# fgcallari/skeres

Hardware: AMD Instinct MI355X
Metric: LM iterations/sec (higher is better)
Workload: dtype f64

## Files before the change

include/skeres_amd.h:

```cpp
#ifndef SKERES_AMD_H
#define SKERES_AMD_H

#include <stddef.h>

#ifdef __cplusplus
extern "C" {
#endif

typedef enum sk_status {
  SK_OK = 0,
  SK_ERR_INVALID_ARGUMENT = 1,
  SK_ERR_NO_DEVICE = 2,
  SK_ERR_HIP = 3,
  SK_ERR_UNSUPPORTED = 4,
  SK_ERR_EVALUATION_FAILED = 5,
  SK_ERR_COMM = 6
} sk_status;

typedef enum sk_linear_solver_type {
  SK_DENSE_NORMAL_CHOLESKY = 0,
  SK_DENSE_QR = 1,
  SK_SPARSE_NORMAL_CHOLESKY = 2,
  SK_DENSE_SCHUR = 3,
  SK_SPARSE_SCHUR = 4,
// ... 237 lines not shown
int sk_options_set_cholesky_envelope(sk_options* o, int on);
enum { SK_DISSECTION_AUTO = 0, SK_DISSECTION_ON = 1, SK_DISSECTION_OFF = 2 };
int sk_options_set_cholesky_dissection(sk_options* o, int mode);
int sk_options_set_resident_kernels(sk_options* o, int on);
int sk_options_set_graph_replay(sk_options* o, int on);
int sk_options_set_max_segments(sk_options* o, int n);
int sk_options_set_trust_region_strategy_type(sk_options* o, int type);
int sk_options_set_dogleg_type(sk_options* o, int type);
int sk_options_get_trust_region_strategy_type(const sk_options* o);
int sk_options_get_dogleg_type(const sk_options* o);
enum { SK_BORDER_AUTO = 0, SK_BORDER_ON = 1, SK_BORDER_OFF = 2 };
int sk_options_set_cholesky_border(sk_options* o, int mode);
enum { SK_RETAINED_AUTO = 0, SK_RETAINED_ON = 1, SK_RETAINED_OFF = 2 };
int sk_options_set_retained_points(sk_options* o, int mode, int max_points);
typedef int (*sk_allreduce_fn)(void* user, double* device_buffer, size_t count, void* hip_stream);
int sk_options_set_distributed(sk_options* o, int rank, int world, sk_allreduce_fn allreduce,
                               void* user);
typedef struct sk_rccl sk_rccl;
int sk_rccl_unique_id(void* id128);
sk_rccl* sk_allreduce_rccl_init(int rank, int world, const void* id128);
sk_rccl* sk_allreduce_rccl_create(void* nccl_comm);
void sk_allreduce_rccl_free(sk_rccl* h);
long sk_allreduce_rccl_calls(const sk_rccl* h);
sk_allreduce_fn sk_allreduce_rccl_fn(void);
enum { SK_DISTRIBUTION_AUTO = 0, SK_DISTRIBUTION_SHARDED = 1, SK_DISTRIBUTION_REPLICATED = 2, SK_DISTRIBUTION_SEGMENTED = 3 };
int sk_options_set_distribution_mode(sk_options* o, int mode);
int sk_options_set_reduce_buffer(sk_options* o, void* device_ptr, size_t bytes);
size_t sk_reduce_buffer_bytes(const sk_options* o, const sk_problem* p);

sk_summary* sk_summary_new(void);
void sk_summary_free(sk_summary* s);
double sk_summary_initial_cost(const sk_summary* s);
double sk_summary_final_cost(const sk_summary* s);
int sk_summary_num_iterations(const sk_summary* s);
int sk_summary_num_successful_steps(const sk_summary* s);
int sk_summary_num_unsuccessful_steps(const sk_summary* s);
int sk_summary_termination_type(const sk_summary* s);
const char* sk_summary_message(const sk_summary* s);
const char* sk_summary_brief_report(const sk_summary* s);
const char* sk_summary_full_report(const sk_summary* s);
int sk_summary_num_logged_iterations(const sk_summary* s);
double sk_summary_iteration_field(const sk_summary* s, int iteration, int field);
double sk_summary_phase_seconds(const sk_summary* s, int phase);
int sk_summary_linear_solver_type_used(const sk_summary* s);
int sk_summary_linear_solver_type_given(const sk_summary* s);

int sk_solve(const sk_options* options, sk_problem* problem, sk_summary* summary);

sk_solver* sk_solver_create(const sk_options* options, sk_problem* problem);
int sk_last_status(void);
void sk_solver_free(sk_solver* s);
int sk_solver_step(sk_solver* s, int* done);
int sk_solver_finish(sk_solver* s, sk_summary* summary);
int sk_solver_set_kernel_timing(sk_solver* s, int on);
double sk_solver_kernel_seconds(const sk_solver* s, const char* name, int* launches);
double sk_solver_syrk_flops_per_solve(const sk_solver* s);
double sk_solver_syrk_c_bytes_per_solve(const sk_solver* s);
int sk_solver_distribution(const sk_solver* s, double* allreduce_seconds, double* saved_seconds);
int sk_solver_stat(const sk_solver* s, const char* name, double* value);
int sk_solver_inner_iteration_blocks(sk_solver* s, int* iterations, int* status);

int sk_problem_point_partition(const sk_problem* p, int world, int* cuts, int* num_cameras,
                               int* num_points, int* point_of_block);
int sk_problem_segment_plan(const sk_problem* p, int max_segments, int forced, int* num_segments, int* camera_part_of_block,
                            int* point_owner_of_block);
int sk_problem_border_plan(const sk_problem* p, int mode, int* num_border_cameras, int* camera_position_of_block, int* gap,
                           double* model_us, double* model_us_plain, double* envelope_fill);
int sk_problem_retained_plan(const sk_problem* p, int mode, int max_points, int border_mode, int* num_retained, int* retained_of_block,
                             double* model_us, double* model_us_without);

int sk_synth_dense_targets(double seed, int m, int n, const double* x_star, double* y_out);

int sk_cholesky_solve(int n, const double* A, const double* b, double* x, double* L, int group);
int sk_cholesky_solve_ex(int n, const double* A, const double* b, double* x, double* L, int group, const int* last,
                         int automatic_plan);
int sk_cholesky_solve_bordered(int n, const double* A, const double* b, double* x, double* L, int group,
                               int border_begin_row, int automatic_plan);

int sk_cholesky_solve_dissected(int n, const double* A, const double* b, double* x, int head, int tail_begin, int group,
                                int automatic_plan);

int sk_cholesky_solve_segments(int n, const double* A, const double* b, double* x, int num_segments, const int* cuts, int group,
                               int automatic_plan);

#ifdef __cplusplus
}
#endif
#endif
```

skeres_amd/api.py:

```python
import ctypes as C
import os

import numpy as np

_HERE = os.path.dirname(os.path.abspath(__file__))
_LIB_PATH = os.path.join(_HERE, "libskeres_amd.so")


class SkeresError(RuntimeError):
    pass


_dp = C.POINTER(C.c_double)
_dpp = C.POINTER(_dp)
_ip = C.POINTER(C.c_int)
EVALUATE_FN = C.CFUNCTYPE(C.c_int, C.c_void_p, _dpp, _dp, _dpp)
ALLREDUCE_FN = C.CFUNCTYPE(C.c_int, C.c_void_p, C.c_void_p, C.c_size_t, C.c_void_p)

_lib = None

_SIGS = {
    "sk_version": (C.c_char_p, []),
    "sk_last_error": (C.c_char_p, []),
    "sk_init_logging": (None, [C.c_char_p]),
# ... 57 lines not shown
    "sk_cost_function_new_tape": (C.c_void_p, [C.c_int, _ip, C.c_int, _ip, C.c_int, _dp, C.c_int, C.c_int, _ip, _dp, C.c_int]),
    "sk_problem_add_dense_rows": (C.c_int, [C.c_void_p, C.c_int, C.c_int, _dp, C.c_void_p, _dp, C.c_int]),
    "sk_problem_num_residual_blocks": (C.c_int, [C.c_void_p]),
    "sk_problem_num_parameter_blocks": (C.c_int, [C.c_void_p]),
    "sk_problem_parameter_block_index": (C.c_int, [C.c_void_p, _dp]),
    "sk_problem_num_parameters": (C.c_int, [C.c_void_p]),
    "sk_problem_num_residuals": (C.c_int, [C.c_void_p]),
    "sk_options_new": (C.c_void_p, []),
    "sk_options_free": (None, [C.c_void_p]),
    "sk_options_set_linear_solver_type": (C.c_int, [C.c_void_p, C.c_int]),
    "sk_options_set_minimizer_type": (C.c_int, [C.c_void_p, C.c_int]),
    "sk_options_set_trust_region_strategy_type": (C.c_int, [C.c_void_p, C.c_int]),
    "sk_options_set_dogleg_type": (C.c_int, [C.c_void_p, C.c_int]),
    "sk_options_get_trust_region_strategy_type": (C.c_int, [C.c_void_p]),
    "sk_options_get_dogleg_type": (C.c_int, [C.c_void_p]),
    "sk_options_set_max_num_iterations": (C.c_int, [C.c_void_p, C.c_int]),
    "sk_options_set_minimizer_progress_to_stdout": (C.c_int, [C.c_void_p, C.c_int]),
    "sk_options_set_function_tolerance": (C.c_int, [C.c_void_p, C.c_double]),
    "sk_options_set_gradient_tolerance": (C.c_int, [C.c_void_p, C.c_double]),
    "sk_options_set_parameter_tolerance": (C.c_int, [C.c_void_p, C.c_double]),
    "sk_options_set_initial_trust_region_radius": (C.c_int, [C.c_void_p, C.c_double]),
    "sk_options_set_max_trust_region_radius": (C.c_int, [C.c_void_p, C.c_double]),
    "sk_options_set_min_trust_region_radius": (C.c_int, [C.c_void_p, C.c_double]),
    "sk_options_set_min_relative_decrease": (C.c_int, [C.c_void_p, C.c_double]),
    "sk_options_set_min_lm_diagonal": (C.c_int, [C.c_void_p, C.c_double]),
    "sk_options_set_max_lm_diagonal": (C.c_int, [C.c_void_p, C.c_double]),
    "sk_options_set_jacobi_scaling": (C.c_int, [C.c_void_p, C.c_int]),
    "sk_options_set_max_num_consecutive_invalid_steps": (C.c_int, [C.c_void_p, C.c_int]),
    "sk_options_set_device": (C.c_int, [C.c_void_p, C.c_int]),
    "sk_options_set_preconditioner_type": (C.c_int, [C.c_void_p, C.c_int]),
    "sk_options_set_eta": (C.c_int, [C.c_void_p, C.c_double]),
    "sk_options_set_max_linear_solver_iterations": (C.c_int, [C.c_void_p, C.c_int]),
    "sk_options_set_min_linear_solver_iterations": (C.c_int, [C.c_void_p, C.c_int]),
    "sk_options_set_cholesky_tuning": (C.c_int, [C.c_void_p, C.c_int, C.c_int]),
    "sk_options_set_schur_elimination": (C.c_int, [C.c_void_p, C.c_int]),
    "sk_cgnr_elimination_plan": (C.c_int, [C.c_void_p, _ip, _ip, _ip, _ip, _ip]),
    "sk_options_set_use_inner_iterations": (C.c_int, [C.c_void_p, C.c_int]),
    "sk_options_get_use_inner_iterations": (C.c_int, [C.c_void_p]),
    "sk_options_set_inner_iteration_tolerance": (C.c_int, [C.c_void_p, C.c_double]),
    "sk_options_get_inner_iteration_tolerance": (C.c_double, [C.c_void_p]),
    "sk_options_set_inner_iteration_ordering": (C.c_int, [C.c_void_p, C.POINTER(_dp), _ip, C.c_int]),
    "sk_inner_iteration_plan": (C.c_int, [C.c_void_p, C.c_void_p, _ip, _ip]),
    "sk_solver_inner_iteration_blocks": (C.c_int, [C.c_void_p, _ip, _ip]),
    "sk_options_set_stream": (C.c_int, [C.c_void_p, C.c_void_p]),
    "sk_options_set_distributed": (C.c_int, [C.c_void_p, C.c_int, C.c_int, ALLREDUCE_FN, C.c_void_p]),
    "sk_options_set_reduce_buffer": (C.c_int, [C.c_void_p, C.c_void_p, C.c_size_t]),
    "sk_reduce_buffer_bytes": (C.c_size_t, [C.c_void_p, C.c_void_p]),
    "sk_summary_new": (C.c_void_p, []),
    "sk_summary_free": (None, [C.c_void_p]),
    "sk_summary_initial_cost": (C.c_double, [C.c_void_p]),
    "sk_summary_final_cost": (C.c_double, [C.c_void_p]),
    "sk_summary_num_iterations": (C.c_int, [C.c_void_p]),
    "sk_summary_num_successful_steps": (C.c_int, [C.c_void_p]),
    "sk_summary_num_unsuccessful_steps": (C.c_int, [C.c_void_p]),
    "sk_summary_termination_type": (C.c_int, [C.c_void_p]),
    "sk_summary_message": (C.c_char_p, [C.c_void_p]),
    "sk_summary_brief_report": (C.c_char_p, [C.c_void_p]),
    "sk_summary_full_report": (C.c_char_p, [C.c_void_p]),
    "sk_summary_num_logged_iterations": (C.c_int, [C.c_void_p]),
    "sk_summary_iteration_field": (C.c_double, [C.c_void_p, C.c_int, C.c_int]),
    "sk_summary_phase_seconds": (C.c_double, [C.c_void_p, C.c_int]),
    "sk_summary_linear_solver_type_used": (C.c_int, [C.c_void_p]),
    "sk_summary_linear_solver_type_given": (C.c_int, [C.c_void_p]),
    "sk_solve": (C.c_int, [C.c_void_p, C.c_void_p, C.c_void_p]),
    "sk_solver_create": (C.c_void_p, [C.c_void_p, C.c_void_p]),
    "sk_solver_free": (None, [C.c_void_p]),
    "sk_solver_step": (C.c_int, [C.c_void_p, _ip]),
    "sk_solver_finish": (C.c_int, [C.c_void_p, C.c_void_p]),
    "sk_solver_set_kernel_timing": (C.c_int, [C.c_void_p, C.c_int]),
    "sk_solver_kernel_seconds": (C.c_double, [C.c_void_p, C.c_char_p, _ip]),
    "sk_solver_syrk_flops_per_solve": (C.c_double, [C.c_void_p]),
    "sk_solver_syrk_c_bytes_per_solve": (C.c_double, [C.c_void_p]),
    "sk_solver_distribution": (C.c_int, [C.c_void_p, _dp, _dp]),
    "sk_solver_stat": (C.c_int, [C.c_void_p, C.c_char_p, _dp]),
    "sk_last_status": (C.c_int, []),
    "sk_cholesky_solve_dissected": (C.c_int, [C.c_int, _dp, _dp, _dp, C.c_int, C.c_int, C.c_int, C.c_int]),
    "sk_rccl_unique_id": (C.c_int, [C.c_void_p]),
    "sk_allreduce_rccl_init": (C.c_void_p, [C.c_int, C.c_int, C.c_void_p]),
    "sk_allreduce_rccl_create": (C.c_void_p, [C.c_void_p]),
    "sk_allreduce_rccl_free": (None, [C.c_void_p]),
    "sk_allreduce_rccl_calls": (C.c_long, [C.c_void_p]),
    "sk_allreduce_rccl_fn": (C.c_void_p, []),
    "sk_cholesky_solve_segments": (C.c_int, [C.c_int, _dp, _dp, _dp, C.c_int, _ip, C.c_int, C.c_int]),
    "sk_cholesky_solve_ex": (C.c_int, [C.c_int, _dp, _dp, _dp, _dp, C.c_int, _ip, C.c_int]),
    "sk_problem_border_plan": (C.c_int, [C.c_void_p, C.c_int, C.POINTER(C.c_int), _ip, C.POINTER(C.c_int), C.POINTER(C.c_double), C.POINTER(C.c_double), C.POINTER(C.c_double)]),
    "sk_cholesky_solve_bordered": (C.c_int, [C.c_int, _dp, _dp, _dp, _dp, C.c_int, C.c_int, C.c_int]),
    "sk_options_set_distribution_mode": (C.c_int, [C.c_void_p, C.c_int]),
    "sk_options_set_cholesky_envelope": (C.c_int, [C.c_void_p, C.c_int]),
    "sk_options_set_cholesky_dissection": (C.c_int, [C.c_void_p, C.c_int]),
    "sk_options_set_cholesky_border": (C.c_int, [C.c_void_p, C.c_int]),
    "sk_options_set_retained_points": (C.c_int, [C.c_void_p, C.c_int, C.c_int]),
    "sk_problem_retained_plan": (C.c_int, [C.c_void_p, C.c_int, C.c_int, C.c_int, C.POINTER(C.c_int), _ip, C.POINTER(C.c_double), C.POINTER(C.c_double)]),
    "sk_options_set_resident_kernels": (C.c_int, [C.c_void_p, C.c_int]),
    "sk_options_set_graph_replay": (C.c_int, [C.c_void_p, C.c_int]),
    "sk_options_set_max_segments": (C.c_int, [C.c_void_p, C.c_int]),
    "sk_cholesky_solve": (C.c_int, [C.c_int, _dp, _dp, _dp, _dp, C.c_int]),
    "sk_synth_dense_targets": (C.c_int, [C.c_double, C.c_int, C.c_int, _dp, _dp]),
    "sk_problem_point_partition": (C.c_int, [C.c_void_p, C.c_int, _ip, _ip, _ip, _ip]),
    "sk_problem_segment_plan": (C.c_int, [C.c_void_p, C.c_int, C.c_int, _ip, _ip, _ip]),
    "sk_evaluate_options_new": (C.c_void_p, []),
    "sk_evaluate_options_free": (None, [C.c_void_p]),
    "sk_evaluate_options_set_apply_loss_function": (C.c_int, [C.c_void_p, C.c_int]),
    "sk_evaluate_options_set_residual_blocks": (C.c_int, [C.c_void_p, _ip, C.c_int]),
    "sk_evaluate_options_set_parameter_blocks": (C.c_int, [C.c_void_p, _dpp, C.c_int]),
    "sk_evaluate_options_set_device": (C.c_int, [C.c_void_p, C.c_int]),
    "sk_evaluate_options_set_launch_timing": (C.c_int, [C.c_void_p, C.c_int]),
    "sk_evaluate_options_launch_seconds": (C.c_double, [C.c_void_p, C.c_int]),
    "sk_problem_evaluate_sizes": (C.c_int, [C.c_void_p, C.c_void_p, _ip, _ip, C.POINTER(C.c_longlong)]),
    "sk_problem_evaluate_structure": (C.c_int, [C.c_void_p, C.c_void_p, _ip, _ip]),
    "sk_problem_evaluate": (C.c_int, [C.c_void_p, C.c_void_p, _dp, _dp, _dp, _dp]),
    "sk_covariance_options_new": (C.c_void_p, []),
    "sk_covariance_options_free": (None, [C.c_void_p]),
    "sk_covariance_options_set_apply_loss_function": (C.c_int, [C.c_void_p, C.c_int]),
    "sk_covariance_options_set_min_reciprocal_condition_number": (C.c_int, [C.c_void_p, C.c_double]),
    "sk_covariance_options_set_device": (C.c_int, [C.c_void_p, C.c_int]),
    "sk_covariance_options_set_schur_elimination": (C.c_int, [C.c_void_p, C.c_int]),
    "sk_covariance_elimination_plan": (C.c_int, [C.c_void_p, _ip, _ip, _ip, C.POINTER(C.c_longlong)]),
    "sk_covariance_new": (C.c_void_p, [C.c_void_p]),
    "sk_covariance_free": (None, [C.c_void_p]),
    "sk_covariance_compute": (C.c_int, [C.c_void_p, C.c_void_p, _dpp, _dpp, C.c_int]),
    "sk_covariance_compute_blocks": (C.c_int, [C.c_void_p, C.c_void_p, _dpp, C.c_int]),
    "sk_covariance_get_block": (C.c_int, [C.c_void_p, _dp, _dp, _dp]),
    "sk_covariance_get_block_in_tangent_space": (C.c_int, [C.c_void_p, _dp, _dp, _dp]),
    "sk_covariance_get_matrix": (C.c_int, [C.c_void_p, _dpp, C.c_int, _dp]),
    "sk_covariance_get_matrix_in_tangent_space": (C.c_int, [C.c_void_p, _dpp, C.c_int, _dp]),
    "sk_covariance_stat": (C.c_int, [C.c_void_p, C.c_char_p, _dp]),
    "sk_covariance_block_sizes": (C.c_int, [C.c_void_p, _dp, _ip, _ip]),
}


def exported_symbols():
    return sorted(_SIGS)


def lib():
    global _lib
    if _lib is None:
        global _LIB_PATH
        _LIB_PATH = os.environ.get("SKERES_AMD_LIBRARY", _LIB_PATH)
        if not os.path.exists(_LIB_PATH):
            raise SkeresError("%s is missing: build it with `python -c 'import __graft_entry__ as g; g.build()'` "
                              "(make -C skeres_amd/csrc). There is no CPU fallback." % _LIB_PATH)
        L = C.CDLL(_LIB_PATH)
        for name, (res, args) in _SIGS.items():
            fn = getattr(L, name)
            fn.restype = res
            fn.argtypes = args
        _lib = L
    return _lib


def _check(rc):
    if rc != 0:
        raise SkeresError("status %d: %s" % (rc, lib().sk_last_error().decode()))


def _check_arg(rc):
    if rc == 1:
        raise ValueError(lib().sk_last_error().decode())
    _check(rc)


def device_count():
    return lib().sk_device_count()


# ... 1273 lines not shown
        mode = lib().sk_solver_distribution(self._h, C.byref(a), C.byref(b))
        return {1: "sharded", 2: "replicated", 3: "segmented"}.get(mode, "sharded"), a.value, b.value


def cholesky_solve(A, b, want_L=False, group=0, last=None, automatic_plan=False):
    A = np.ascontiguousarray(A, dtype=np.float64)
    b = np.ascontiguousarray(b, dtype=np.float64)
    n = A.shape[0]
    x = np.empty(n)
    L = np.empty((n, n)) if want_L else None
    lp = _ip()
    if last is not None:
        last = np.ascontiguousarray(last, dtype=np.int32)
        if last.shape[0] != (n + 1 + 127) // 128:
            raise ValueError("last needs one entry per 128-block column of the padded matrix")
        lp = last.ctypes.data_as(_ip)
    _check(lib().sk_cholesky_solve_ex(n, A.ctypes.data_as(_dp), b.ctypes.data_as(_dp), x.ctypes.data_as(_dp),
                                      L.ctypes.data_as(_dp) if want_L else _dp(), int(group), lp, int(bool(automatic_plan))))
    return (x, L) if want_L else x


def cholesky_solve_bordered(A, b, border_begin, want_L=False, group=0, automatic_plan=False):
    A = np.ascontiguousarray(A, dtype=np.float64)
    b = np.ascontiguousarray(b, dtype=np.float64)
    n = A.shape[0]
    x = np.empty(n)
    L = np.empty((n, n)) if want_L else None
    _check(lib().sk_cholesky_solve_bordered(n, A.ctypes.data_as(_dp), b.ctypes.data_as(_dp), x.ctypes.data_as(_dp),
                                            L.ctypes.data_as(_dp) if want_L else _dp(), int(group), int(border_begin), int(bool(automatic_plan))))
    return (x, L) if want_L else x


def cholesky_solve_dissected(A, b, head, tail_begin, group=0, automatic_plan=False):
    A = np.ascontiguousarray(A, dtype=np.float64)
    b = np.ascontiguousarray(b, dtype=np.float64)
    n = A.shape[0]
    x = np.empty(n)
    _check(lib().sk_cholesky_solve_dissected(n, A.ctypes.data_as(_dp), b.ctypes.data_as(_dp), x.ctypes.data_as(_dp), int(head), int(tail_begin),
                                             int(group), int(bool(automatic_plan))))
    return x


class RcclAllReduce:

    @staticmethod
    def unique_id():
        buf = C.create_string_buffer(128)
        _check(lib().sk_rccl_unique_id(buf))
        return buf.raw

    def __init__(self, rank, world, unique_id):
        self._id = C.create_string_buffer(bytes(unique_id), 128)
        self._h = lib().sk_allreduce_rccl_init(int(rank), int(world), self._id)
        if not self._h:
            raise SkeresError("status 6: %s" % lib().sk_last_error().decode())

    @property
    def calls(self):
        return int(lib().sk_allreduce_rccl_calls(self._h))

    def close(self):
        if self._h:
            lib().sk_allreduce_rccl_free(self._h)
            self._h = None

    def __del__(self):
        try:
            self.close()
        except Exception:
            pass


def cholesky_solve_segments(A, b, cuts, group=0, automatic_plan=False):
    A = np.ascontiguousarray(A, dtype=np.float64)
    b = np.ascontiguousarray(b, dtype=np.float64)
    n = A.shape[0]
    x = np.empty(n)
    c = np.ascontiguousarray(np.asarray(cuts, dtype=np.int32).reshape(-1))
    _check(lib().sk_cholesky_solve_segments(n, A.ctypes.data_as(_dp), b.ctypes.data_as(_dp), x.ctypes.data_as(_dp), len(cuts) + 1,
                                            c.ctypes.data_as(_ip), int(group), int(bool(automatic_plan))))
    return x


def synth_dense_targets(seed, m, n, x_star):
    xs = np.ascontiguousarray(x_star, dtype=np.float64)
    y = np.empty(int(m))
    _check(lib().sk_synth_dense_targets(float(seed), int(m), int(n), xs.ctypes.data_as(_dp), y.ctypes.data_as(_dp)))
    return y
```

skeres_amd/csrc/capi.hip:

```cpp
#include <cmath>
#include <cstdlib>
#include <new>

#include "bal_kernels.hpp"
#include "chol_solve.hpp"
#include "dense_kernels.hpp"
#include "dense_rows_kernels.hpp"
#include "evaluate_kernels.hpp"
#include "cgnr_plan.hpp"
#include "inner_plan.hpp"
#include "covariance.hpp"
#include "covariance_plan.hpp"
#include "evaluate_plan.hpp"
#include "solver.hpp"

using namespace sk;

struct sk_ptrvec { std::vector<double*> v; };
struct sk_loss_function { LossFunction l; };
struct sk_cost_function { CostFunction c; };
struct sk_problem { Problem p; };
struct sk_local_parameterization { LocalParameterization p; };
struct sk_options { Options o; };
struct sk_summary { Summary s; };
// ... 1041 lines not shown
  std::vector<int> part, owner;
  *num_segments = bal_segment_plan(p->p, max_segments, forced != 0, &part, &owner);
  for (size_t b = 0; b < part.size(); ++b) {
    if (camera_part_of_block) camera_part_of_block[b] = part[b];
    if (point_owner_of_block) point_owner_of_block[b] = owner[b];
  }
  return SK_OK;
  SK_GUARD_END(SK_ERR_INVALID_ARGUMENT)
}

int sk_problem_border_plan(const sk_problem* p, int mode, int* num_border_cameras, int* camera_position_of_block, int* gap, double* model_us, double* model_us_plain,
                           double* envelope_fill) {
  SK_GUARD_BEGIN
  if (!p || !num_border_cameras) { set_error("invalid argument"); return SK_ERR_INVALID_ARGUMENT; }
  if (mode != SK_BORDER_AUTO && mode != SK_BORDER_ON && mode != SK_BORDER_OFF) { set_error("invalid border mode %d", mode); return SK_ERR_INVALID_ARGUMENT; }
  std::string why;
  if (!problem_is_bal_shaped(p->p, &why)) { set_error("%s", why.c_str()); return SK_ERR_UNSUPPORTED; }
  std::vector<int> pos;
  *num_border_cameras = bal_border_plan(p->p, mode, &pos, gap, model_us, model_us_plain, envelope_fill);
  if (camera_position_of_block) for (size_t b = 0; b < pos.size(); ++b) camera_position_of_block[b] = pos[b];
  return SK_OK;
  SK_GUARD_END(SK_ERR_INVALID_ARGUMENT)
}

int sk_problem_retained_plan(const sk_problem* p, int mode, int max_points, int border_mode, int* num_retained, int* retained_of_block, double* model_us,
                             double* model_us_without) {
  SK_GUARD_BEGIN
  if (!p || !num_retained) { set_error("invalid argument"); return SK_ERR_INVALID_ARGUMENT; }
  if (mode != SK_RETAINED_AUTO && mode != SK_RETAINED_ON && mode != SK_RETAINED_OFF) { set_error("invalid retained-points mode %d", mode); return SK_ERR_INVALID_ARGUMENT; }
  if (border_mode != SK_BORDER_AUTO && border_mode != SK_BORDER_ON && border_mode != SK_BORDER_OFF) { set_error("invalid border mode %d", border_mode); return SK_ERR_INVALID_ARGUMENT; }
  std::string why;
  if (!problem_is_bal_shaped(p->p, &why)) { set_error("%s", why.c_str()); return SK_ERR_UNSUPPORTED; }
  std::vector<int> flag;
  *num_retained = bal_retained_plan(p->p, mode, max_points, border_mode, &flag, model_us, model_us_without);
  if (retained_of_block) for (size_t b = 0; b < flag.size(); ++b) retained_of_block[b] = flag[b];
  return SK_OK;
  SK_GUARD_END(SK_ERR_INVALID_ARGUMENT)
}

int sk_synth_dense_targets(double seed, int m, int n, const double* x_star, double* y_out) {
  SK_GUARD_BEGIN
  if (m <= 0 || n <= 0 || !x_star || !y_out) { set_error("invalid argument"); return SK_ERR_INVALID_ARGUMENT; }
  if (sk_device_count() <= 0) { set_error("no HIP device available: libskeres_amd has no CPU fallback"); return SK_ERR_NO_DEVICE; }
  std::vector<double> consts(3 * (size_t)m);
  for (int i = 0; i < m; ++i) { consts[3 * (size_t)i] = seed; consts[3 * (size_t)i + 1] = (double)i; consts[3 * (size_t)i + 2] = 0.0; }
  std::vector<double> xs(x_star, x_star + n);
  DevBuf<double> dc, dx, dr;
  hipStream_t s = nullptr;
  SK_HIP_TRY(dc.upload(consts, s)); SK_HIP_TRY(dx.upload(xs, s)); SK_HIP_TRY(dr.alloc(m));
  DenseRowsArgs a{}; a.loss_root = -1; a.m = m; a.n = n; a.m_pad = m; a.consts = dc.p; a.inv_sqrt_n = 1.0 / std::sqrt((double)n);
  launch_rows_residual(a, dx.p, dr.p, nullptr, false, s);
  SK_HIP_TRY(hipMemcpy(y_out, dr.p, (size_t)m * sizeof(double), hipMemcpyDeviceToHost));
  return SK_OK;
  SK_GUARD_END(SK_ERR_INVALID_ARGUMENT)
}

int sk_cholesky_solve(int n, const double* A, const double* b, double* x, double* L, int group) {
  return sk_cholesky_solve_ex(n, A, b, x, L, group, nullptr, 0);
}
int sk_cholesky_solve_ex(int n, const double* A, const double* b, double* x, double* L, int group, const int* last, int automatic_plan) {
  SK_GUARD_BEGIN
  if (n <= 0 || !A || !b || !x) { set_error("invalid argument"); return SK_ERR_INVALID_ARGUMENT; }
  return cholesky_solve_single(n, A, b, x, L, group, last, automatic_plan, -1);
  SK_GUARD_END(SK_ERR_INVALID_ARGUMENT)
}
int sk_cholesky_solve_bordered(int n, const double* A, const double* b, double* x, double* L, int group, int border_begin_row, int automatic_plan) {
  SK_GUARD_BEGIN
  if (n <= 0 || !A || !b || !x || border_begin_row < 0 || border_begin_row > n) { set_error("invalid argument"); return SK_ERR_INVALID_ARGUMENT; }
  return cholesky_solve_single(n, A, b, x, L, group, nullptr, automatic_plan, border_begin_row);
  SK_GUARD_END(SK_ERR_INVALID_ARGUMENT)
}
int sk_cholesky_solve_dissected(int n, const double* A, const double* b, double* x, int head, int tail_begin, int group, int automatic_plan) {
  SK_GUARD_BEGIN
  if (n <= 0 || !A || !b || !x || head < 0 || tail_begin < head || tail_begin > n) { set_error("invalid argument"); return SK_ERR_INVALID_ARGUMENT; }
  return cholesky_solve_two_way(n, A, b, x, head, tail_begin, group, automatic_plan);
  SK_GUARD_END(SK_ERR_INVALID_ARGUMENT)
}
int sk_cholesky_solve_segments(int n, const double* A, const double* b, double* x, int num_segments, const int* cuts, int group, int automatic_plan) {
  SK_GUARD_BEGIN
  if (n <= 0 || !A || !b || !x || num_segments < 2 || !cuts) { set_error("invalid argument"); return SK_ERR_INVALID_ARGUMENT; }
  return cholesky_solve_multi_way(n, A, b, x, num_segments, cuts, group, automatic_plan);
  SK_GUARD_END(SK_ERR_INVALID_ARGUMENT)
}

}
```

skeres_amd/csrc/chol_fronts.cpp:

```cpp
#include "chol_fronts.hpp"

#include <cstdio>
#include <cstring>

namespace sk {

std::vector<int> host_block_first_cols(const std::vector<double>& M, size_t ld, int nblk) {
  std::vector<int> first_col(nblk);
  for (int i = 0; i < nblk; ++i) {
    first_col[i] = i;
    for (int j = 0; j < i && first_col[i] == i; ++j) {
      bool nz = false;
      for (int r = 0; r < 128 && !nz; ++r) {
        const double* row = &M[((size_t)i * 128 + r) * ld + (size_t)j * 128];
        for (int c = 0; c < 128; ++c) if (row[c] != 0.0) { nz = true; break; }
      }
      if (nz) first_col[i] = j;
    }
  }
  return first_col;
}
std::vector<int> host_block_envelope(const std::vector<double>& M, size_t ld, int nblk, int tail_rows) {
  return cholesky_envelope_last(host_block_first_cols(M, ld, nblk), tail_rows);
}
// ... 85 lines not shown
std::string segment_cuts(int n, const double* A, int R, const int* cuts, SegmentCuts* out) {
  SegmentCuts& c = *out;
  c.R = R; c.n = n;
  c.sb.assign(R + 1, 0); c.se.assign(R + 1, 0);
  std::vector<int>& sb = c.sb; std::vector<int>& se = c.se;
  sb[R] = n;
  for (int k = 1; k < R; ++k) { sb[k] = cuts[2 * (k - 1)]; se[k] = cuts[2 * (k - 1) + 1]; }
  for (int k = 1; k <= R; ++k)
    if (sb[k] < se[k - 1] || (k < R && (se[k] < sb[k] || se[k] > n))) return "invalid cuts";
  for (int k = 1; k < R; ++k)
    for (int i = se[k]; i < n; ++i)
      for (int j = 0; j < sb[k]; ++j)
        if (A[(size_t)i * n + j] != 0.0) return format("rows behind separator %d couple with rows before it at (%d, %d): not a separator", k, i, j);
  c.sep_off.assign(R, 0);
  for (int k = 1; k < R; ++k) c.sep_off[k] = c.sep_off[k - 1] + (se[k] - sb[k]);
  c.nroot = c.sep_off[R - 1];
  return std::string();
}

static inline double sym(const double* A, int n, int i, int j) { return i >= j ? A[(size_t)i * n + j] : A[(size_t)j * n + i]; }

HostFront segments_root(const SegmentCuts& c, const double* A, const double* b) {
  HostFront r;
  const int R = c.R, nroot = c.nroot, E = (nroot + 1 + 127) / 128;
  const size_t dR = (size_t)E * 128;
  r.dim = dR; r.nblk = E; r.ncols = E; r.rhs_row = nroot;
  std::vector<double>& FR = r.F;
  FR.assign(dR * dR, 0.0);
  for (int k = 1; k < R; ++k)
    for (int i = c.sb[k]; i < c.se[k]; ++i) {
      const int ri = c.root_index(i);
      for (int k2 = 1; k2 <= k; ++k2)
        for (int j = c.sb[k2]; j < c.se[k2] && j <= i; ++j) FR[(size_t)ri * dR + c.root_index(j)] = sym(A, c.n, i, j);
      FR[(size_t)nroot * dR + ri] = b[i];
    }
  FR[(size_t)nroot * dR + nroot] = 1e300;
  for (size_t j = (size_t)nroot + 1; j < dR; ++j) FR[j * dR + j] = 1.0;
  r.last = root_envelope(c.sep_off);
  return r;
}

LeafFront segment_leaf(const SegmentCuts& c, const double* A, const double* b, int k) {
  LeafFront f;
  const int R = c.R;
  const std::vector<int>& sb = c.sb; const std::vector<int>& se = c.se;
  const int lo = se[k], hi = sb[k + 1], ni = hi - lo;
  const int left_n = k > 0 ? se[k] - sb[k] : 0, right_n = k + 1 < R ? se[k + 1] - sb[k + 1] : 0;
  f.L = segment_layout(ni, left_n, right_n);
  f.interior_n = ni;
  const SegmentLayout& L = f.L;
  f.dim = (size_t)L.nblk * 128;
  const size_t d = f.dim;
  f.order.assign(d, -1);
  for (int t = 0; t < ni; ++t) f.order[t] = L.reversed ? hi - 1 - t : lo + t;
  const int bo = L.ncols * 128;
  if (L.right_off >= 0) for (int t = 0; t < right_n; ++t) f.order[bo + L.right_off + t] = sb[k + 1] + t;
  if (L.left_off >= 0) for (int t = 0; t < left_n; ++t) f.order[bo + L.left_off + t] = L.reversed ? se[k] - 1 - t : sb[k] + t;
  std::vector<double>& F = f.F;
  F.assign(d * d, 0.0);
  for (size_t i = 0; i < d; ++i) {
    const int gi = f.order[i];
    if (gi < 0) continue;
    for (size_t j = 0; j <= i && j < (size_t)ni; ++j) F[i * d + j] = sym(A, c.n, gi, f.order[j]);
  }
  for (int t = 0; t < ni; ++t) F[(size_t)L.rhs_row * d + t] = b[f.order[t]];
  for (int i = ni; i < bo; ++i) F[(size_t)i * d + i] = 1.0;
  f.last = host_block_envelope(F, d, L.nblk, L.tail_rows);
  f.map.assign(d - bo, -1);
  for (size_t i = bo; i < d; ++i) if (f.order[i] >= 0) f.map[i - bo] = c.root_index(f.order[i]);
  f.map[L.rhs_row - bo] = c.nroot;
  f.gmap = f.map;
  f.gmap[L.rhs_row - bo] = -1;
  return f;
}

void segments_scatter_root(const SegmentCuts& c, const double* yR, double* x) {
  for (int k = 1; k < c.R; ++k) for (int i = c.sb[k]; i < c.se[k]; ++i) x[i] = yR[c.root_index(i)];
}

void segments_scatter_leaf(const LeafFront& f, const double* y, double* x) {
  for (int t = 0; t < f.L.ncols * 128; ++t) if (f.order[t] >= 0) x[f.order[t]] = y[t];
}

}
```

skeres_amd/csrc/chol_fronts.hpp:

```cpp
#pragma once
#include <cstddef>
#include <string>
#include <vector>

#include "chol_envelope.hpp"

namespace sk {

std::vector<int> host_block_first_cols(const std::vector<double>& M, size_t ld, int nblk);
std::vector<int> host_block_envelope(const std::vector<double>& M, size_t ld, int nblk, int tail_rows = 1);

struct HostFront {
  size_t dim = 0;
  int nblk = 0, ncols = 0, rhs_row = 0;
  std::vector<double> F;
  std::vector<int> last;
};

struct SingleFront {
  int n = 0, npad = 0, nblk = 0, rhs_row = 0;
  std::vector<double> S;
  std::vector<int> last, tail;
};
inline int single_front_blocks(int n) { return (n + 1 + 127) / 128; }
int invalid_envelope_column(int n, const int* last);
SingleFront single_front(int n, const double* A, const double* b, int border_begin_row);
void single_front_solution(const SingleFront& f, const std::vector<double>& y, double* x);
void single_front_factor(const SingleFront& f, const std::vector<double>& S, double* L);

struct TwoWayFronts {
  int n = 0, head = 0, tail_n = 0, sep_n = 0, border_blocks = 0;
  HostFront A, B, R;
  std::vector<int> mapB;
};
std::string two_way_check(int n, const double* A, int head, int tail_begin);
TwoWayFronts two_way_fronts(int n, const double* A, const double* b, int head, int tail_begin);
void two_way_scatter(const TwoWayFronts& f, const double* y, double* x);

struct SegmentCuts {
  int R = 0, n = 0, nroot = 0;
  std::vector<int> sb, se;
  std::vector<int> sep_off;
  int root_index(int row) const;
};
std::string segment_cuts(int n, const double* A, int R, const int* cuts, SegmentCuts* out);
HostFront segments_root(const SegmentCuts& c, const double* A, const double* b);
struct LeafFront {
  SegmentLayout L;
  size_t dim = 0;
  int interior_n = 0;
  std::vector<int> order;
  std::vector<int> map;
  std::vector<int> gmap;
  std::vector<int> last;
  std::vector<double> F;
};
LeafFront segment_leaf(const SegmentCuts& c, const double* A, const double* b, int k);
void segments_scatter_root(const SegmentCuts& c, const double* yR, double* x);
void segments_scatter_leaf(const LeafFront& f, const double* y, double* x);

}
```

skeres_amd/csrc/chol_kernels.hip:

```cpp
#include <hip/hip_runtime.h>
#include <algorithm>
#include <atomic>
#include <chrono>
#include <hip/hip_ext.h>
#include <math.h>
#include <stdlib.h>
#include <string.h>
#include <memory>
#include "chol_kernels.hpp"
#include "device_table.hpp"

namespace sk {

typedef double d4 __attribute__((ext_vector_type(4)));

constexpr int gemm_lds_doubles(int kBKT, int kTM, int kTN) { return 2 * (kTM + kTN) * (kBKT + 2); }
#define SK_GEMM_LDS(kBKT, kTM, kTN) __shared__ __attribute__((aligned(16))) double sh[gemm_lds_doubles(kBKT, kTM, kTN)];
template <int kMode, int kShape, int kBKT, int kPF, int kTM, int kTN>
__device__ __forceinline__ void gemm_nt_f64_body(double* shp, double* C, long ldc, const double* A, long lda, const double* B, long ldb, int K,
                                                 int tiles_m, int skip, int main_t = 0x7fffffff, int jump_t = 0, int main_n = 0x7fffffff,
                                                 int jump_n = 0, int block_id = -1, int* first_column_done = nullptr, int count_cols = 1,
                                                 int* diag_done = nullptr) {
  constexpr int mode = kMode;
  constexpr int kLdT = kBKT + 2;
// ... 75 lines not shown
  _Pragma("unroll") for (int i = 0; i < kChB; ++i) {                                                       \
    const double2 v_ = *reinterpret_cast<const double2*>(Bg + (long)(i * kRowStep + srow) * ldb + (kbase) + sc); rb##set[2 * i] = v_.x; rb##set[2 * i + 1] = v_.y; \
  }
#define SK_STORE_STAGE(set, buf)                                                                   \
  _Pragma("unroll") for (int i = 0; i < kChA; ++i)                                                  \
    *reinterpret_cast<double2*>(&shp[(buf) * kShBuf + (i * kRowStep + srow) * kLdT + sc]) = make_double2(ra##set[2 * i], ra##set[2 * i + 1]); \
  _Pragma("unroll") for (int i = 0; i < kChB; ++i)                                                  \
    *reinterpret_cast<double2*>(&shp[(buf) * kShBuf + (kTM + i * kRowStep + srow) * kLdT + sc]) = make_double2(rb##set[2 * i], rb##set[2 * i + 1]);
  const int nk = K / kBKT;
  SK_LOAD_STAGE(0, 0)
  if (kPF == 2) { SK_LOAD_STAGE(1, (nk > 1 ? 1 : 0) * kBKT) }
  SK_STORE_STAGE(0, 0)
  __syncthreads();
#define SK_LOAD_STAGE_X(set, kbase) SK_LOAD_STAGE(set, kbase)
#define SK_STORE_STAGE_X(set, buf) SK_STORE_STAGE(set, buf)
#define SK_KSTEP(kt, SETL, SETS)                                                                   \
  {                                                                                                \
    const int buf = (kt) & 1;                                                                      \
    const int knext = ((kt) + kPF < nk ? (kt) + kPF : nk - 1) * kBKT;                              \
    SK_LOAD_STAGE_X(SETL, knext)                                                                   \
    const double* sa = &shp[buf * kShBuf + (wr * (kTM / 2) + l15) * kLdT + l4];                               \
    const double* sb = &shp[buf * kShBuf + (kTM + wc * (kTN / 2) + l15) * kLdT + l4];                         \
    _Pragma("unroll") for (int kk = 0; kk < kBKT / 4; ++kk) {                                      \
      double a[kMT], b[kNT];                                                                       \
      _Pragma("unroll") for (int m = 0; m < kMT; ++m) a[m] = sa[m * 16 * kLdT + kk * 4];           \
      _Pragma("unroll") for (int m = 0; m < kNT; ++m) b[m] = sb[m * 16 * kLdT + kk * 4];           \
      _Pragma("unroll") for (int mt = 0; mt < kMT; ++mt)                                           \
        _Pragma("unroll") for (int nt = 0; nt < kNT; ++nt)                                         \
          acc[mt][nt] = __builtin_amdgcn_mfma_f64_16x16x4f64(a[mt], b[nt], acc[mt][nt], 0, 0, 0);  \
    }                                                                                              \
    SK_STORE_STAGE_X(SETS, buf ^ 1)                                                                \
    __syncthreads();                                                                               \
  }
  if (kPF == 1) {
    for (int kt = 0; kt < nk; ++kt) SK_KSTEP(kt, 0, 0)
  } else {
    for (int kt = 0; kt < nk; kt += 2) {
      SK_KSTEP(kt, 0, 1)
      SK_KSTEP(kt + 1, 1, 0)
    }
  }
#undef SK_KSTEP
#undef SK_LOAD_STAGE_X
#undef SK_STORE_STAGE_X
  (void)ra1; (void)rb1;
#undef SK_LOAD_STAGE
#undef SK_STORE_STAGE
  const double sgn = mode == 0 ? -1.0 : 1.0;
  if (kShape == 2 && first_column_done && first_column) {
#pragma unroll
    for (int mt = 0; mt < kMT; ++mt)
#pragma unroll
      for (int nt = 0; nt < kNT; ++nt)
#pragma unroll
        for (int i = 0; i < 4; ++i)
          __hip_atomic_store(&Cg[(long)(crow + mt * 16 + 4 * i) * ldc + ccol + nt * 16], sgn * acc[mt][nt][i], __ATOMIC_RELAXED, __HIP_MEMORY_SCOPE_AGENT);
    asm volatile("s_waitcnt vmcnt(0) lgkmcnt(0)" ::: "memory");
    __syncthreads();
    if (threadIdx.x == 0) {
      __hip_atomic_fetch_add(first_column_done, 1, __ATOMIC_RELAXED, __HIP_MEMORY_SCOPE_AGENT);
      if (diag_done && diag_tile) __hip_atomic_fetch_add(diag_done, 16 / (128 / kTM), __ATOMIC_RELAXED, __HIP_MEMORY_SCOPE_AGENT);
    }
    return;
  }
#pragma unroll
  for (int mt = 0; mt < kMT; ++mt)
#pragma unroll
    for (int nt = 0; nt < kNT; ++nt)
#pragma unroll
      for (int i = 0; i < 4; ++i)
        Cg[(long)(crow + mt * 16 + 4 * i) * ldc + ccol + nt * 16] = sgn * acc[mt][nt][i];
}

__global__ __launch_bounds__(256, 2) void syrk_trailing_f64_kernel(double* C, long ldc, const double* A, long lda, int K, int tile_off, int main_t,
                                                                   int jump_t) {
  SK_GEMM_LDS(16, 128, 128)
  gemm_nt_f64_body<0, 1, 16, 1, 128, 128>(sh, C, ldc, A, lda, A, lda, K, 0, tile_off, main_t, jump_t);
}
__global__ __launch_bounds__(256, 2) void syrk_trailing_thin_f64_kernel(double* C, long ldc, const double* A, long lda, int K, int tiles_m, int main_t,
                                                                        int jump_t, int main_n, int jump_n, int* first_column_done, int count_cols, int* diag_done) {
  SK_GEMM_LDS(16, 32, 128)
  gemm_nt_f64_body<0, 2, 16, 2, 32, 128>(sh, C, ldc, A, lda, A, lda, K, tiles_m, 0, main_t, jump_t, main_n, jump_n, -1, first_column_done, count_cols, diag_done);
}
struct ThinSyrkArgs { double* C; long ldc; const double* A; long lda; int K, tiles_m, main_t, jump_t, main_n, jump_n; int* first_column_done; int grid; };
struct ThinSyrkPair { ThinSyrkArgs f[2]; };
__global__ __launch_bounds__(256, 2) void syrk_trailing_thin_pair_f64_kernel(ThinSyrkPair pair) {
  const ThinSyrkArgs& p = pair.f[blockIdx.y];
  if ((int)blockIdx.x >= p.grid) return;
  SK_GEMM_LDS(16, 32, 128)
  gemm_nt_f64_body<0, 2, 16, 2, 32, 128>(sh, p.C, p.ldc, p.A, p.lda, p.A, p.lda, p.K, p.tiles_m, 0, p.main_t, p.jump_t, p.main_n, p.jump_n, -1, p.first_column_done, 1, nullptr);
}
__global__ __launch_bounds__(256, 2) void syrk_gram_f64_kernel(double* C, long ldc, size_t slab_stride, const double* A, long lda, int K) {
  SK_GEMM_LDS(16, 128, 128)
  gemm_nt_f64_body<1, 1, 16, 1, 128, 128>(sh, C + (size_t)blockIdx.y * slab_stride, ldc, A + (size_t)blockIdx.y * K, lda, A + (size_t)blockIdx.y * K, lda, K, 0, 0);
}
__global__ __launch_bounds__(256) void gram_reduce_kernel(double* __restrict__ H, const double* __restrict__ slabs, size_t slab_stride, long ld,
                                                          int nslabs) {
  const int b = blockIdx.x;
  int r = (int)((sqrt(8.0 * (double)b + 1.0) - 1.0) * 0.5);
  while ((r + 1) * (r + 2) / 2 <= b) ++r;
  while (r * (r + 1) / 2 > b) --r;
  const int ti = r, tj = b - r * (r + 1) / 2;
  for (int e = threadIdx.x; e < 128 * 128; e += 256) {
    const size_t off = (size_t)(ti * 128 + (e >> 7)) * ld + tj * 128 + (e & 127);
    double s = 0.0;
    for (int c = 0; c < nslabs; ++c) s += slabs[(size_t)c * slab_stride + off];
    H[off] = s;
  }
}
__global__ __launch_bounds__(256, 2) void gemm_update_f64_kernel(double* C, long ldc, const double* A, long lda, const double* B,
                                                                 long ldb, int K, int tiles_m, int skip, int main_t, int jump_t) {
  __builtin_amdgcn_s_setprio(2);
  SK_GEMM_LDS(16, 64, 128)
  gemm_nt_f64_body<0, 0, 16, 2, 64, 128>(sh, C, ldc, A, lda, B, ldb, K, tiles_m, skip, main_t, jump_t);
}
__global__ __launch_bounds__(256, 2) void gemm_update_thin_f64_kernel(double* C, long ldc, const double* A, long lda, const double* B,
                                                                      long ldb, int K, int tiles_m, int skip, int main_t, int jump_t) {
  __builtin_amdgcn_s_setprio(2);
  SK_GEMM_LDS(16, 32, 128)
  gemm_nt_f64_body<0, 0, 16, 2, 32, 128>(sh, C, ldc, A, lda, B, ldb, K, tiles_m, skip, main_t, jump_t);
}
__global__ __launch_bounds__(256, 2) void trsm_gemm_thin_f64_kernel(double* C, long ldc, const double* A, long lda, const double* Linv,
                                                                    int tiles_m, int main_t, int jump_t) {
  __builtin_amdgcn_s_setprio(2);
  SK_GEMM_LDS(16, 32, 128)
  gemm_nt_f64_body<1, 0, 16, 2, 32, 128>(sh, C, ldc, A, lda, Linv, 128, 128, tiles_m, 0, main_t, jump_t);
}
__global__ __launch_bounds__(256, 1) void gemm_diag_f64_kernel(double* C, long ldc, const double* A, long lda, int K) {
  __builtin_amdgcn_s_setprio(3);
  SK_GEMM_LDS(32, 64, 64)
  gemm_nt_f64_body<0, 0, 32, 2, 64, 64>(sh, C, ldc, A, lda, A, lda, K, 2, 4);
}
__global__ __launch_bounds__(256, 2) void trsm_gemm_f64_kernel(double* C, long ldc, const double* A, long lda, const double* Linv,
                                                               int tiles_m, int main_t, int jump_t) {
  __builtin_amdgcn_s_setprio(2);
  SK_GEMM_LDS(16, 64, 128)
  gemm_nt_f64_body<1, 0, 16, 2, 64, 128>(sh, C, ldc, A, lda, Linv, 128, 128, tiles_m, 0, main_t, jump_t);
}

static constexpr int kB = 32, kBs = 33;
static constexpr int kBlk = kB * kBs;
__device__ __forceinline__ int blk_off(int bi, int bj) { return (bi * (bi + 1) / 2 + bj) * kBlk; }
__device__ __forceinline__ int inv_off(int bi, int bj) { return (10 + bi * (bi - 1) / 2 + bj) * kBlk; }

__device__ __forceinline__ double fast_rsqrt(double x) {
  double y = __builtin_amdgcn_rsq(x);
  double h = 0.5 * x;
  y = y * (1.5 - h * y * y);
  y = y * (1.5 - h * y * y);
  return y;
}
__device__ __forceinline__ double fast_rcp(double x) {
  const double y = __builtin_amdgcn_rcp(x);
  const double e = __builtin_fma(-x, y, 1.0);
  const double q = __builtin_fma(e, e, e);
  return __builtin_fma(y, q, y);
}
__device__ __forceinline__ double lane_bcast(double x, int src) {
  const int lo = __builtin_amdgcn_readlane(__double2loint(x), src);
  const int hi = __builtin_amdgcn_readlane(__double2hiint(x), src);
  return __hiloint2double(hi, lo);
}

__device__ __forceinline__ bool wave_potrf32(const double* D, double* colbuf, double (&a)[32], int lane) {
  const int row = lane & 31;
  const bool unit = lane >= 32;
#pragma unroll
  for (int c = 0; c < 32; ++c) {
    const double d = D[row * kBs + c];
// ... 506 lines not shown
      }
      if (sync_load(abort_flag) != 0) return false;
      if (wall_clock64() - t0 > kChainTimeoutTicks) { __hip_atomic_store(abort_flag, 1, __ATOMIC_RELAXED, __HIP_MEMORY_SCOPE_AGENT); return false; }
    }
    __builtin_amdgcn_s_sleep(2);
  }
}

struct ChainRanges { int n; int begin[8], end[8]; };

__device__ __forceinline__ void chain_end_signal(int* counter) {
  __syncthreads();
  if (threadIdx.x == 0) {
    __builtin_amdgcn_fence(__ATOMIC_RELEASE, "agent");
    __hip_atomic_fetch_add(counter, 1, __ATOMIC_RELAXED, __HIP_MEMORY_SCOPE_AGENT);
  }
}
__global__ void chain_end_marker_kernel(int* counter) { chain_end_signal(counter); }
__global__ void chain_gate_kernel(const int* counter, int expected, int* info) {
  if (threadIdx.x != 0) return;
  if (sync_load(counter) < expected) {
    const long long t0 = wall_clock64();
    int spins = 0;
    do {
      __builtin_amdgcn_s_sleep(4);
      if ((++spins & 63) == 0 && wall_clock64() - t0 > 4 * kChainTimeoutTicks) { info_raise(info, 2); break; }
    } while (sync_load(counter) < expected);
  }
  __builtin_amdgcn_fence(__ATOMIC_ACQUIRE, "agent");
}
__global__ void chain_start_gate_kernel(const int* p, int value, int* info) {
  if (threadIdx.x != 0) return;
  if (!chain_wait_start(p, value)) info_raise(info, 2);
}
__device__ __forceinline__ void potrf_server_body(double* lds, double* S, long ld, const ChainRanges& ranges, double* Linv, int* info, int* sync, int maxblk, int local, int start) {
  __shared__ int ok_s;
  const int stamp_front = gridDim.x == 2 ? (int)blockIdx.x : 0;
  int done = 0;
  if (start != 0) {
    if (threadIdx.x == 0) ok_s = chain_wait_start(sync + kSyncStart, start) ? 1 : 0;
    __syncthreads();
    if (!ok_s) {
      if (threadIdx.x == 0) info_raise(info, 2);
      return;
    }
    SK_CHAIN_ACQUIRE_ALL
    __syncthreads();
  }
  if (local && threadIdx.x == 0) __hip_atomic_store(sync + kSyncServerXcc, 1 + xcc_id(), __ATOMIC_RELAXED, __HIP_MEMORY_SCOPE_AGENT);
  for (int r = 0; r < ranges.n; ++r)
    for (int j = ranges.begin[r]; j < ranges.end[r]; ++j) {
      if (j > 0) {
        if (threadIdx.x == 0) ok_s = server_wait_diag(sync, j, local) ? 1 : 0;
        __syncthreads();
        if (!ok_s) {
          if (threadIdx.x == 0) info_raise(info, 2);
          return;
        }
        SK_CHAIN_ACQUIRE_ALL
      }
      SK_CHAIN_STAMP(j, 0)
      potrf128_body(lds, S + (long)j * 128 * ld + (long)j * 128, ld, Linv + (long)j * 128 * 128, info);
      if (local) {
        asm volatile("s_waitcnt vmcnt(0) lgkmcnt(0)" ::: "memory");
        __syncthreads();
        if (threadIdx.x == 0) {
          store_l2(sync + kSyncPotrfFast, j + 1);
          SK_CHAIN_STAMP(j, 1)
          __builtin_amdgcn_fence(__ATOMIC_RELEASE, "agent");
          __hip_atomic_fetch_add(sync + kSyncPotrfDone, j + 1 - done, __ATOMIC_RELAXED, __HIP_MEMORY_SCOPE_AGENT);
        }
      } else {
        chain_publish(sync + kSyncPotrfDone, j + 1 - done);
        SK_CHAIN_STAMP(j, 1)
      }
      done = j + 1;
    }
}
__global__ __launch_bounds__(256, 1) void potrf_server_kernel(double* S, long ld, ChainRanges ranges, double* Linv, int* info, int* sync, int maxblk, int local, int start) {
  extern __shared__ __attribute__((aligned(16))) double lds[];
  potrf_server_body(lds, S, ld, ranges, Linv, info, sync, maxblk, local, start);
  if (start != 0) chain_end_signal(sync + kSyncEnd);
}
__global__ __launch_bounds__(256) void chain_start_kernel(int* sync_a, int n_a, int* sync_b, int n_b, int value) {
  for (int i = threadIdx.x; i < n_a; i += 256) sync_a[i] = 0;
  if (sync_b) for (int i = threadIdx.x; i < n_b; i += 256) sync_b[i] = 0;
  __syncthreads();
  if (threadIdx.x != 0) return;
  __builtin_amdgcn_fence(__ATOMIC_RELEASE, "agent");
  __hip_atomic_store(sync_a + kSyncStart, value, __ATOMIC_RELAXED, __HIP_MEMORY_SCOPE_AGENT);
  if (sync_b) __hip_atomic_store(sync_b + kSyncStart, value, __ATOMIC_RELAXED, __HIP_MEMORY_SCOPE_AGENT);
}
struct ServerArgs { double* S; long ld; ChainRanges ranges; double* Linv; int* sync; int maxblk; };
struct ServerPair { ServerArgs f[2]; };
__global__ __launch_bounds__(256, 1) void potrf_server_pair_kernel(ServerPair pair, int* info, int local, int start) {
  extern __shared__ __attribute__((aligned(16))) double lds[];
  const ServerArgs& p = pair.f[blockIdx.x];
  potrf_server_body(lds, p.S, p.ld, p.ranges, p.Linv, info, p.sync, p.maxblk, local, start);
  if (start != 0) chain_end_signal(pair.f[0].sync + kSyncEnd);
}

constexpr int kCritLd = 130;
__device__ __forceinline__ void crit_tile_load(double* shp, const double* A, long lda, const double* B, long ldb) {
  const int t = threadIdx.x, row = t >> 3, c0 = (t & 7) * 16;
  double2 va[8], vb[8];
#pragma unroll
  for (int i = 0; i < 8; ++i) va[i] = *reinterpret_cast<const double2*>(A + (long)row * lda + c0 + 2 * i);
#pragma unroll
  for (int i = 0; i < 8; ++i) vb[i] = *reinterpret_cast<const double2*>(B + (long)row * ldb + c0 + 2 * i);
#pragma unroll
  for (int i = 0; i < 8; ++i) *reinterpret_cast<double2*>(shp + row * kCritLd + c0 + 2 * i) = va[i];
#pragma unroll
  for (int i = 0; i < 8; ++i) *reinterpret_cast<double2*>(shp + (32 + row) * kCritLd + c0 + 2 * i) = vb[i];
}
__device__ __forceinline__ d4 crit_tile_mma(const double* shp, d4 acc) {
  const int lane = threadIdx.x & 63, wave = threadIdx.x >> 6;
  const int l15 = lane & 15, l4 = lane >> 4;
  const double* sa = shp + ((wave >> 1) * 16 + l15) * kCritLd + l4;
  const double* sb = shp + (32 + (wave & 1) * 16 + l15) * kCritLd + l4;
  d4 acc1 = {0.0, 0.0, 0.0, 0.0};
#pragma unroll
  for (int kk = 0; kk < 32; kk += 2) {
    acc = __builtin_amdgcn_mfma_f64_16x16x4f64(sa[kk * 4], sb[kk * 4], acc, 0, 0, 0);
    acc1 = __builtin_amdgcn_mfma_f64_16x16x4f64(sa[kk * 4 + 4], sb[kk * 4 + 4], acc1, 0, 0, 0);
  }
  return acc + acc1;
}
__device__ __forceinline__ long crit_tile_off(long ldc, int i) {
  const int lane = threadIdx.x & 63, wave = threadIdx.x >> 6;
  return (long)((wave >> 1) * 16 + (lane >> 4) + 4 * i) * ldc + (wave & 1) * 16 + (lane & 15);
}

__device__ __forceinline__ void chain_column_body(int b, double* S, long ld, int j, const double* Linv_j, int tiles_m, int main_t, int jump_t,
                                                  int ncrit, double* Xs, int* sync, int maxblk, int syrk_need, int column_need, int* info, int do_next, int wait_first,
                                                  int ncand) {
  __shared__ __attribute__((aligned(16))) double sh[2 * 32 * kCritLd];
  static_assert(2 * 32 * kCritLd >= gemm_lds_doubles(16, 32, 128), "LDS of the thin tiles");
  __shared__ int ok_s;
  const int stamp_front = gridDim.y == 2 ? (int)blockIdx.y : 0;
  __builtin_amdgcn_s_setprio(2);
  double* A21 = S + (long)(j + 1) * 128 * ld + (long)j * 128;
  int* x_ready = sync + kSyncHeader + maxblk + j;
  int* diag_ready = sync + kSyncHeader + j + 1;
  int* abort_flag = sync + kSyncAbort;
  const bool local = ncand > ncrit;
  bool crit = b < ncand;
  if (crit && local) {
    if (threadIdx.x == 0) {
      int t = -1;
      if (chain_wait(sync + kSyncServerXcc, 1, abort_flag) && sync_load(sync + kSyncServerXcc) == 1 + xcc_id())
        t = __hip_atomic_fetch_add(sync + kSyncHeader + 2 * maxblk + j, 1, __ATOMIC_RELAXED, __HIP_MEMORY_SCOPE_AGENT);
      ok_s = t >= 0 && t < 16 ? t : -1;
    }
    __syncthreads();
    const int tile = ok_s;
    __syncthreads();
    if (tile < 0) return;
    b = tile;
  }
  const int ri = b >> 2, q = b & 3;
  const int thin_id = 4 + (b - ncand);
  const int thin_bid = ncrit ? thin_id : b;
  const bool stamp = b == 0 && crit == (ncrit > 0);
  if (stamp) SK_CHAIN_STAMP(j, 2)
  if (crit && local) {
    double* Xj = Xs + (size_t)j * 128 * 128;
    const bool lower = q <= ri;
    double* Ct = A21 + 128 + (long)(ri * 32) * ld + q * 32;
    {
      const int t = threadIdx.x, row = t >> 3, c0 = (t & 7) * 16;
      double2 va[8];
#pragma unroll
      for (int i = 0; i < 8; ++i) va[i] = *reinterpret_cast<const double2*>(A21 + (long)(ri * 32 + row) * ld + c0 + 2 * i);
#pragma unroll
      for (int i = 0; i < 8; ++i) *reinterpret_cast<double2*>(sh + row * kCritLd + c0 + 2 * i) = va[i];
    }
    if (threadIdx.x == 0) ok_s = chain_wait_l2(sync + kSyncPotrfFast, j + 1, abort_flag) ? 1 : 0;
    __syncthreads();
// ... 52 lines not shown
      if (b == 1 && threadIdx.x == 0) {
        __builtin_amdgcn_fence(__ATOMIC_RELEASE, "agent");
        __hip_atomic_fetch_add(x_ready, 16, __ATOMIC_RELAXED, __HIP_MEMORY_SCOPE_AGENT);
      }
      asm volatile("s_waitcnt vmcnt(0) lgkmcnt(0)" ::: "memory");
      if (lower) {
#pragma unroll
        for (int i = 0; i < 8; ++i) *reinterpret_cast<double2*>(sh + row * kCritLd + c0 + 2 * i) = va[i];
#pragma unroll
        for (int i = 0; i < 8; ++i) *reinterpret_cast<double2*>(sh + (32 + row) * kCritLd + c0 + 2 * i) = vb[i];
      }
    }
    __syncthreads();
    if (lower) {
      cacc = crit_tile_mma(sh, cacc);
#pragma unroll
      for (int i = 0; i < 4; ++i) Ct[crit_tile_off(ld, i)] = -cacc[i];
    }
    asm volatile("s_waitcnt vmcnt(0) lgkmcnt(0)" ::: "memory");
    __syncthreads();
    if (threadIdx.x == 0) store_l2(sync + kSyncDSlot + b, j + 1);
    if (stamp) SK_CHAIN_STAMP(j, 6)
    return;
  }
  if (threadIdx.x == 0)
    ok_s = (chain_wait(sync + kSyncPotrfDone, j + 1, abort_flag) &&
            (!wait_first || (chain_wait(sync + kSyncSyrkSeq, syrk_need, abort_flag) && chain_wait(sync + kSyncSyrkColumn, column_need, abort_flag)))) ? 1 : 0;
  __syncthreads();
  if (!ok_s) { if (threadIdx.x == 0) info_raise(info, 2); return; }
  SK_CHAIN_ACQUIRE_ALL
  if (stamp) SK_CHAIN_STAMP(j, 3)
  d4 xacc = {0.0, 0.0, 0.0, 0.0};
  if (crit) {
    crit_tile_load(sh, A21 + (long)ri * 32 * ld, ld, Linv_j + (long)q * 32 * 128, 128);
    __syncthreads();
    xacc = crit_tile_mma(sh, xacc);
#pragma unroll
    for (int i = 0; i < 4; ++i) store_through(Xs + (long)(ri * 32) * 128 + q * 32 + crit_tile_off(128, i), xacc[i]);
    chain_publish_through(x_ready, 1);
  } else {
    gemm_nt_f64_body<1, 0, 16, 2, 32, 128>(sh, A21, ld, A21, ld, Linv_j, 128, 128, tiles_m, 0, main_t, jump_t, 0x7fffffff, 0, thin_bid);
    asm volatile("s_waitcnt vmcnt(0) lgkmcnt(0)" ::: "memory");
    __syncthreads();
  }
  if (stamp) SK_CHAIN_STAMP(j, 4)
  if (!do_next && !crit) return;
  if (threadIdx.x == 0)
    ok_s = (chain_wait(x_ready, ncrit, abort_flag) && (!do_next || (chain_wait(sync + kSyncSyrkSeq, syrk_need, abort_flag) &&
            chain_wait(sync + kSyncSyrkColumn, column_need, abort_flag)))) ? 1 : 0;
  __syncthreads();
  if (!ok_s) { if (threadIdx.x == 0) info_raise(info, 2); return; }
  SK_CHAIN_ACQUIRE_ALL
  if (stamp) SK_CHAIN_STAMP(j, 5)
  const double* Xsrc = local ? (const double*)(Xs + (size_t)j * 128 * 128) : (const double*)Xs;
  if (crit) {
#pragma unroll
    for (int i = 0; i < 4; ++i) A21[(long)(ri * 32) * ld + q * 32 + crit_tile_off(ld, i)] = xacc[i];
    if (!do_next) return;
    if (q <= ri) {
      double* Ct = A21 + 128 + (long)(ri * 32) * ld + q * 32;
      d4 acc;
#pragma unroll
      for (int i = 0; i < 4; ++i) acc[i] = -Ct[crit_tile_off(ld, i)];
      crit_tile_load(sh, Xs + (long)ri * 32 * 128, 128, Xs + (long)q * 32 * 128, 128);
      __syncthreads();
      acc = crit_tile_mma(sh, acc);
#pragma unroll
      for (int i = 0; i < 4; ++i) store_through(Ct + crit_tile_off(ld, i), -acc[i]);
    }
    chain_publish_through(diag_ready, 1);
  } else {
    const double* Bx = ncrit ? Xsrc : (const double*)A21;
    gemm_nt_f64_body<0, 0, 16, 2, 32, 128>(sh, A21 + 128, ld, A21, ld, Bx, ncrit ? 128 : ld, 128, tiles_m, 1, main_t, jump_t, 0x7fffffff, 0, thin_bid);
    if (ncrit == 0 && b == 0) chain_publish(diag_ready, 16);
  }
  if (stamp) SK_CHAIN_STAMP(j, 6)
}
__global__ __launch_bounds__(256, 2) void chain_column_kernel(double* S, long ld, int j, const double* Linv_j, int tiles_m, int main_t, int jump_t,
                                                              int ncrit, double* Xs, int* sync, int maxblk, int syrk_need, int column_need, int* info, int do_next, int wait_first,
                                                              int ncand) {
  chain_column_body((int)blockIdx.x, S, ld, j, Linv_j, tiles_m, main_t, jump_t, ncrit, Xs, sync, maxblk, syrk_need, column_need, info, do_next, wait_first, ncand);
}
struct ColumnArgs { double* S; long ld; int j; const double* Linv_j; int tiles_m, main_t, jump_t, ncrit; double* Xs; int* sync; int maxblk, syrk_need, column_need, grid, ncand; };
struct ColumnPair { ColumnArgs f[2]; };
__global__ __launch_bounds__(256, 2) void chain_column_pair_kernel(ColumnPair pair, int* info) {
  const ColumnArgs& p = pair.f[blockIdx.y];
  if ((int)blockIdx.x >= p.grid) return;
  chain_column_body((int)blockIdx.x, p.S, p.ld, p.j, p.Linv_j, p.tiles_m, p.main_t, p.jump_t, p.ncrit, p.Xs, p.sync, p.maxblk, p.syrk_need, p.column_need, info, 1, 0, p.ncand);
}

__global__ void chain_marker_kernel(int* flag, int seq) {
  __hip_atomic_store(flag, seq, __ATOMIC_RELAXED, __HIP_MEMORY_SCOPE_AGENT);
}

__global__ __launch_bounds__(1024) void bs_step_kernel(const double* __restrict__ Linv, const double* __restrict__ Lrow, long ld,
                                                        double* __restrict__ w, double* __restrict__ yout, int kb, int col0, int ncols) {
  __shared__ double wk[128], ykb[128], part[8][128];
  const int t = threadIdx.x;
  const int c = t & 127, g = t >> 7;
  const int cl = t & 63, rg = t >> 6;
  const int col = col0 + blockIdx.x * 64 + cl;
  double wv = 0.0, li[16], lr[8];
  if (t < 128) wv = w[kb * 128 + t];
#pragma unroll
  for (int i = 0; i < 16; ++i) li[i] = Linv[(long)(g * 16 + i) * 128 + c];
  if (col < ncols) {
    const double* p = Lrow + (long)(rg * 8) * ld + col;
#pragma unroll
    for (int i = 0; i < 8; ++i) lr[i] = p[(long)i * ld];
  } else {
#pragma unroll
    for (int i = 0; i < 8; ++i) lr[i] = 0.0;
  }
  if (t < 128) wk[t] = wv;
  __syncthreads();
  {
    double s = 0.0;
#pragma unroll
    for (int i = 0; i < 16; ++i) s += li[i] * wk[g * 16 + i];
    part[g][c] = s;
  }
  __syncthreads();
  if (t < 128) {
    double s = 0.0;
#pragma unroll
    for (int q = 0; q < 8; ++q) s += part[q][t];
    ykb[t] = s;
    if (blockIdx.x == 0) yout[kb * 128 + t] = s;
  }
  __syncthreads();
  double s = 0.0;
#pragma unroll
  for (int i = 0; i < 8; ++i) s += lr[i] * ykb[rg * 8 + i];
  double* red = &part[0][0];
  red[rg * 64 + cl] = s;
  __syncthreads();
  if (t < 64 && col < ncols) {
    double u = 0.0;
#pragma unroll
    for (int g = 0; g < 16; ++g) u += red[g * 64 + t];
    w[col] -= u;
  }
}

#ifdef SK_TESTING
__device__ int g_bs_test_janitor_giveup;
#endif
__device__ long long g_bs_stamps[1024][4];
__device__ int g_bs_stamps_on;
constexpr int kBsMaxBlocks = 960;
struct BsTop { unsigned short top[kBsMaxBlocks]; unsigned short tail[kBsMaxBlocks]; };
constexpr unsigned long long kBsSentinel = ~0ull;
struct BsArgs {
  const double* Linv; double* S; long ld; const double* rhs; int n; double* y; int nblk; int* info; int nown; const double* yb;
  int janitors;
  const int* yb_map;
  int jan_parts;
  int l2_poll;
};
__device__ __forceinline__ unsigned long long load_sc0_u64(const unsigned long long* p) {
  unsigned long long v;
  asm volatile("global_load_dwordx2 %0, %1, off sc0\n\ts_waitcnt vmcnt(0)" : "=v"(v) : "v"(p) : "memory");
  return v;
}
template <typename Env>
__device__ __forceinline__ void bs_resident_body(const BsArgs& a, const Env& env, const int block) {
  const double* __restrict__ Linv = a.Linv; double* S = a.S; const long ld = a.ld; const double* rhs = a.rhs; const int n = a.n; double* y = a.y;
  const int nblk = a.nblk; int* info = a.info; const int nown = a.nown; const double* __restrict__ yb = a.yb; const int zero_after = a.janitors;
// ... 76 lines not shown
          } else {
            v = __hip_atomic_load(src, __ATOMIC_RELAXED, __HIP_MEMORY_SCOPE_AGENT);
          }
          if (v == kBsSentinel && wall_clock64() - t0 > kChainTimeoutTicks) { abort_s = 1; v = 0ull; }
        } while (v == kBsSentinel);
      }
      ysh[t] = __longlong_as_double((long long)v);
    }
    __syncthreads();
    if (g_bs_stamps_on && t == 0 && cur == kb + 1) g_bs_stamps[kb][1] = wall_clock64();
#pragma unroll
    for (int g = 0; g < 2; ++g) {
      double sacc = 0.0;
#pragma unroll
      for (int i = 0; i < 8; ++i) sacc += lr[g * 8 + i] * ysh[rg * 16 + g * 8 + i];
      part[rg * 2 + g][c] = sacc;
    }
    const int nxt = (cur > top && cur - 1 < tlo) ? top : cur - 1;
    if (nxt > kb) {
      const double* p = Lcol + (long)nxt * 128 * ld;
#pragma unroll
      for (int i = 0; i < 16; ++i) lr[i] = p[(long)i * ld];
    }

    __syncthreads();
    if (t < 128) {
      double u = 0.0;
#pragma unroll
      for (int g = 0; g < 16; ++g) u += part[g][t];
      wsh[t] -= u;
    }
    cur = nxt;
  }
  __syncthreads();
  {
    double sacc = 0.0;
#pragma unroll
    for (int i = 0; i < 16; ++i) sacc += li[i] * wsh[rg * 16 + i];
    part[rg][c] = sacc;
  }
  __syncthreads();
  if (t < 128) {
    double sacc = 0.0;
#pragma unroll
    for (int q = 0; q < 8; ++q) sacc += part[q][t];
    unsigned long long bits = (unsigned long long)__double_as_longlong(sacc);
    if (bits == kBsSentinel) bits ^= 1ull;
    if (a.l2_poll) *reinterpret_cast<volatile unsigned long long*>(y + (long)kb * 128 + t) = bits;
    __hip_atomic_store(reinterpret_cast<unsigned long long*>(y + (long)kb * 128 + t), bits, __ATOMIC_RELAXED, __HIP_MEMORY_SCOPE_AGENT);
    if (g_bs_stamps_on && t == 0) { asm volatile("s_waitcnt vmcnt(0)" ::: "memory"); g_bs_stamps[kb][2] = wall_clock64(); }
  }
  if (t == 0 && abort_s && info) info_raise(info, 2);
}

__global__ __launch_bounds__(1024, 1) void bs_resident_kernel(const double* __restrict__ Linv, double* S, long ld, const double* rhs,
                                                               int n, double* y, int nblk, BsTop env, int* info, int nown, const double* __restrict__ yb, int zero_after ,
                                                               const int* __restrict__ yb_map) {
  const int spread = zero_after < 0 ? 1 : 0;
  const BsArgs a{Linv, S, ld, rhs, n, y, nblk, info, nown, yb, spread ? 7 * nown : zero_after, yb_map, spread ? 7 : 0, spread};
  const int b = (int)blockIdx.x;
  bs_resident_body(a, env, spread ? ((b & 7) == 0 ? b >> 3 : nown + (b >> 3) * 7 + (b & 7) - 1) : b);
}
constexpr int kBsPairMaxBlocks = 448;
struct BsTopHalf { unsigned short top[kBsPairMaxBlocks]; unsigned short tail[kBsPairMaxBlocks]; };
struct BsPair { BsArgs f[2]; BsTopHalf env[2]; };
__global__ __launch_bounds__(1024, 1) void bs_resident_pair_kernel(BsPair p) {
  const int b = (int)blockIdx.x, nA = p.f[0].nown, nB = p.f[1].nown, own = nA + nB;
  int front, blk;
  if (p.f[0].jan_parts > 0) {
    const int g = b >> 3, slot = b & 7;
    front = slot >> 2;
    const int nown = front ? nB : nA;
    if (g >= nown) return;
    blk = (slot & 3) == 0 ? g : nown + g * 3 + (slot & 3) - 1;
    bs_resident_body(p.f[front], p.env[front], blk);
    return;
  }
  if (b < own) {
    const int m = nA < nB ? nA : nB;
    if (b < 2 * m) { front = b & 1; blk = b >> 1; } else { front = nA > nB ? 0 : 1; blk = b - m; }
  } else {
    const int j = b - own;
    if (j < p.f[0].janitors) { front = 0; blk = nA + j; } else { front = 1; blk = nB + (j - p.f[0].janitors); }
  }
  bs_resident_body(p.f[front], p.env[front], blk);
}

__global__ void copy_row_kernel(const double* __restrict__ src, double* __restrict__ dst, int n, int npad) {
  const int j = blockIdx.x * blockDim.x + threadIdx.x;
  if (j < npad) dst[j] = j < n ? src[j] : 0.0;
}

static const size_t g_potrf_lds = (size_t)(18 * kBlk + 192 + 4) * sizeof(double);
size_t potrf128_lds_bytes() { return g_potrf_lds; }

static std::vector<hipStream_t> g_orphan_streams;
constexpr int g_early_column = 1;
constexpr int g_thin_grid = 512;
constexpr int g_ext_events = 1;
constexpr unsigned g_event_flags = hipEventDisableTiming | hipEventDisableSystemFence;
static int g_chain_server = 1;
constexpr int g_chain_max_trailing = 24, g_chain_prefix_group = 2;
static int g_pair_max_trailing = 0;
constexpr int g_thin_syrk_tiles = 48;
constexpr int g_tail_tiles = 48, g_tail_group = 1;
static int g_chain_local = 0;
static std::atomic<int> g_bs_resident{1};
#ifdef SK_TESTING
static std::atomic<int> g_test_withhold{-1};
static std::atomic<int> g_test_janitor_giveup{0};
#endif
hipError_t cholesky_init() {
  static std::once_flag once;
  std::call_once(once, [] {
#ifdef SK_TESTING
    if (const char* e = getenv("SK_CHAIN_TEST_WITHHOLD_MARKER")) g_test_withhold.store(atoi(e));
    if (const char* e = getenv("SK_BS_TEST_JANITOR_GIVEUP")) g_test_janitor_giveup.store(atoi(e) > 0 ? 1 : 0);
#endif
    const DevKnobs& k = dev_knobs();
    g_bs_resident.store(k.bs_resident);
    g_chain_server = k.chain_server;
    g_pair_max_trailing = k.pair_max_trailing;
    g_chain_local = k.chain_xcd_local;
  });
  hipError_t rc = hipFuncSetAttribute(reinterpret_cast<const void*>(potrf_server_kernel), hipFuncAttributeMaxDynamicSharedMemorySize, (int)g_potrf_lds);
  if (rc != hipSuccess) return rc;
  rc = hipFuncSetAttribute(reinterpret_cast<const void*>(potrf_server_pair_kernel), hipFuncAttributeMaxDynamicSharedMemorySize, (int)g_potrf_lds);
  if (rc != hipSuccess) return rc;
  return hipFuncSetAttribute(reinterpret_cast<const void*>(potrf128_kernel), hipFuncAttributeMaxDynamicSharedMemorySize, 160 * 1024);
}

CholeskyContext::~CholeskyContext() {
  for (hipEvent_t e : events) (void)hipEventDestroy(e);
  if (fork_ev) (void)hipEventDestroy(fork_ev);
  if (join_ev) (void)hipEventDestroy(join_ev);
  if (sync) (void)hipFree(sync);
  if (xs) (void)hipFree(xs);
}

int* CholeskyContext::sync_for(int nblk) {
  if (nblk > sync_blk) {
    if (sync) (void)hipFree(sync);
    if (xs) (void)hipFree(xs);
    sync = nullptr; xs = nullptr;
    sync_blk = 0;
    const int cap = (nblk + 63) / 64 * 64;
    if (hipMalloc(reinterpret_cast<void**>(&xs), sizeof(double) * 128 * 128 * (size_t)cap) != hipSuccess) { (void)hipGetLastError(); xs = nullptr; return nullptr; }
    if (hipMalloc(reinterpret_cast<void**>(&sync), sizeof(int) * (size_t)(kSyncHeader + kSyncArrays * cap)) != hipSuccess) { (void)hipGetLastError(); sync = nullptr; return nullptr; }
    sync_blk = cap;
  }
  return sync;
}

constexpr int kBulkCand = 2, kPanelCand = 4, kServerCand = 3;
struct DeviceQueues {
  int device = -1;
  hipStream_t panel = nullptr, bulk = nullptr, bulk_early = nullptr, server = nullptr;
  int reserved_cus = 0, early_tiles = 0;
  hipStream_t bulk_candidates[kBulkCand] = {}, bulk_early_candidates[kBulkCand] = {}, panel_candidates[kPanelCand] = {},
              server_candidates[kServerCand] = {};
  std::vector<hipStream_t> all_streams;
  int queue_choice = -1;
  std::atomic<bool> tuning{false};
  std::atomic<int> chain_server{1};
  std::atomic<int> pair_users{0};
  hipStream_t fork = nullptr;
  hipStream_t plain[2] = {nullptr, nullptr};
  std::mutex enqueue_mutex[2];
};
static PerDeviceTable<DeviceQueues> g_device_queues;

static hipError_t create_bulk_stream(hipStream_t* out, int per_xcd, int ncu, int* reserved) {
  *reserved = 0;
  if (per_xcd > 0 && ncu >= 64 && ncu % 8 == 0 && per_xcd < ncu / 8) {
    std::vector<uint32_t> mask((size_t)(ncu + 31) / 32, 0u);
    for (int i = per_xcd * 8; i < ncu; ++i) mask[(size_t)i / 32] |= 1u << (i % 32);
    if (hipExtStreamCreateWithCUMask(out, (uint32_t)mask.size(), mask.data()) == hipSuccess) { *reserved = per_xcd * 8; return hipSuccess; }
    (void)hipGetLastError();
  }
  return hipStreamCreateWithFlags(out, hipStreamNonBlocking);
}

static DeviceQueues* create_device_queues(int dev) {
  std::unique_ptr<DeviceQueues> q(new DeviceQueues());
  q->device = dev;
  q->chain_server.store(g_chain_server);
  int ncu = 0, reserved = 0, reserved_early = 0;
  (void)hipDeviceGetAttribute(&ncu, hipDeviceAttributeMultiprocessorCount, dev);
  const int per_xcd = dev_knobs().bulk_reserve >= 0 ? dev_knobs().bulk_reserve : 4, per_xcd_early = dev_knobs().bulk_reserve_early >= 0 ? dev_knobs().bulk_reserve_early : 2, early_tiles = 72;
  if (dev_knobs().queue_shift > 0) {
    std::vector<uint32_t> all((size_t)(ncu + 31) / 32, 0xffffffffu);
    for (int k = 0; k < dev_knobs().queue_shift; ++k) {
      hipStream_t d = nullptr;
      if (hipExtStreamCreateWithCUMask(&d, (uint32_t)all.size(), all.data()) != hipSuccess) (void)hipGetLastError();
      else q->all_streams.push_back(d);
    }
  }
  auto fail = [&]() -> DeviceQueues* {
    for (hipStream_t st : q->all_streams) g_orphan_streams.push_back(st);
    return nullptr;
  };
  hipStream_t b = nullptr, be = nullptr;
  if (create_bulk_stream(&b, per_xcd, ncu, &reserved) != hipSuccess) { (void)hipGetLastError(); return fail(); }
  q->all_streams.push_back(b);
  if (create_bulk_stream(&be, per_xcd_early, ncu, &reserved_early) != hipSuccess) { (void)hipGetLastError(); return fail(); }
  q->all_streams.push_back(be);
  q->bulk_candidates[0] = b; q->bulk_early_candidates[0] = be;
  hipStream_t p = nullptr, sv = nullptr;
  if (reserved > 0) {
    const size_t words = (size_t)(ncu + 31) / 32;
    std::vector<uint32_t> cu0(words, 0u), rest(words, 0u);
    cu0[0] = 0xffu;
    for (int i = 8; i < ncu; ++i) rest[(size_t)i / 32] |= 1u << (i % 32);
    bool ok = true;
    auto masked = [&](hipStream_t* out, const std::vector<uint32_t>& m) {
      if (!ok) return;
      if (hipExtStreamCreateWithCUMask(out, (uint32_t)words, m.data()) != hipSuccess) { (void)hipGetLastError(); *out = nullptr; ok = false; return; }
      q->all_streams.push_back(*out);
    };
    for (int k = 1; k < kBulkCand && ok; ++k) {
      int r = 0;
      if (create_bulk_stream(&q->bulk_candidates[k], per_xcd, ncu, &r) != hipSuccess || create_bulk_stream(&q->bulk_early_candidates[k], per_xcd_early, ncu, &r) != hipSuccess) {
        (void)hipGetLastError();
        ok = false;
      }
      if (q->bulk_candidates[k]) q->all_streams.push_back(q->bulk_candidates[k]);
      if (q->bulk_early_candidates[k]) q->all_streams.push_back(q->bulk_early_candidates[k]);
    }
    for (int k = 0; k < kPanelCand; ++k) masked(&q->panel_candidates[k], rest);
    for (int k = 0; k < kServerCand; ++k) masked(&q->server_candidates[k], cu0);
    p = q->panel_candidates[0];
    sv = p ? q->server_candidates[0] : nullptr;
    if (!ok) q->queue_choice = 0;
    if (dev_knobs().chain_queues >= 0) q->queue_choice = dev_knobs().chain_queues % (kBulkCand * kPanelCand * kServerCand);
    if (ok && q->queue_choice >= 0) {
      b = q->bulk_candidates[q->queue_choice / (kPanelCand * kServerCand)];
      be = q->bulk_early_candidates[q->queue_choice / (kPanelCand * kServerCand)];
      p = q->panel_candidates[q->queue_choice / kServerCand % kPanelCand];
      sv = q->server_candidates[q->queue_choice % kServerCand];
    }
  }
  if (!p) {
    if (hipStreamCreateWithFlags(&p, hipStreamNonBlocking) != hipSuccess) { (void)hipGetLastError(); return fail(); }
    q->all_streams.push_back(p);
  }
  q->server = sv; q->panel = p; q->bulk = b; q->bulk_early = be; q->reserved_cus = reserved; q->early_tiles = early_tiles;
  static bool registered = false;
  if (!registered) {
// ... 218 lines not shown
  }
  if (serialised) {
    q.tuning = false;
    ctx->in_trial = false;
    q.chain_server = 0;
    std::fprintf(stderr, "[skeres_amd] the resident panel chain timed out in its trial run (are kernels being serialised, e.g. by counter "
                         "collection?): block columns are factored launch by launch in this process\n");
    select(0);
    q.queue_choice = 0;
    (void)hipFree(A); (void)hipFree(Linv); (void)hipFree(info);
    return;
  }
  double best = ms[0];
  for (int c = 1; c < ncomb; ++c) best = std::min(best, ms[c]);
  if (best > 8.0) {
    q.chain_server = 0;
    std::fprintf(stderr, "[skeres_amd] the resident panel chain ran %.0f times slower than it should in its trial run (is the device shared with "
                         "another process?): block columns are factored launch by launch in this process\n", best / 1.1);
  }
  std::vector<double> ms2((size_t)ncomb, 1e30);
  double best2 = 1e30;
  for (int c = 0; c < ncomb; ++c) {
    if (ms[c] > 1.08 * best) continue;
    select(c);
    ctx->early_tiles = 0;
    double sum = 0.0;
    for (int rep = 0; rep < 4; ++rep) {
      (void)hipStreamSynchronize(s);
      const auto t0 = std::chrono::steady_clock::now();
      cholesky_factor(A, n, n, Linv, info, 2, s, ctx, nullptr, nullptr, false);
      (void)hipStreamSynchronize(s);
      if (rep > 0) sum += std::chrono::duration<double, std::milli>(std::chrono::steady_clock::now() - t0).count();
    }
    ms2[c] = sum / 3.0;
    best2 = std::min(best2, ms2[c]);
  }
  for (int c = ncomb - 1; c >= 0; --c) if (ms2[c] <= 1.04 * best2) q.queue_choice = c;
  if (dev_knobs().debug_queues) {
    std::fprintf(stderr, "[skeres_amd] synthetic factorisations (ms: banded under the resident chain / dense on the early-group queue) per (bulk, panel, server) queue candidates:");
    for (int c = 0; c < ncomb; ++c) {
      std::fprintf(stderr, "%s%.2f", c % kServerCand == 0 ? "  " : " ", ms[c]);
      if (ms2[c] < 1e29) std::fprintf(stderr, "/%.2f", ms2[c]);
    }
    std::fprintf(stderr, ": combination %d (device %d)\n", q.queue_choice, q.device);
  }
  q.tuning = false;
  ctx->in_trial = false;
  select(q.queue_choice);
  (void)hipFree(A);
  (void)hipFree(Linv);
  (void)hipFree(info);
}

bool cholesky_note_info(CholeskyContext* ctx, int info) {
  if (info == 2) g_bs_resident.store(0);
  if (info == 2 && ctx && ctx->sync && dev_knobs().debug_chain_abort) {
    std::vector<int> h((size_t)kSyncHeader + kSyncArrays * ctx->sync_blk);
    (void)hipMemcpy(h.data(), ctx->sync, h.size() * sizeof(int), hipMemcpyDeviceToHost);
    std::fprintf(stderr, "[skeres_amd] chain abort: potrf_done %d abort %d syrk_seq %d syrk_column %d | diag_ready:", h[kSyncPotrfDone], h[kSyncAbort], h[kSyncSyrkSeq], h[kSyncSyrkColumn]);
    for (int j = 0; j < 40 && j < ctx->sync_blk; ++j) std::fprintf(stderr, " %d", h[kSyncHeader + j]);
    std::fprintf(stderr, " | x_ready:");
    for (int j = 0; j < 40 && j < ctx->sync_blk; ++j) std::fprintf(stderr, " %d", h[kSyncHeader + ctx->sync_blk + j]);
    std::fprintf(stderr, "\n");
  }
  if (info != 2) return false;
  if (!ctx || !ctx->dq) {
    std::fprintf(stderr, "[skeres_amd] the resident back-substitution timed out: one launch per block step from now on\n");
    return true;
  }
  std::lock_guard<std::mutex> lock(g_device_queues.operation_mutex());
  if (ctx->dq->chain_server) {
    ctx->dq->chain_server = 0;
    std::fprintf(stderr, "[skeres_amd] the resident panel chain timed out on device %d (is the device shared with another process, or are "
                         "kernels being serialised?): block columns are factored launch by launch on it from now on\n", ctx->dq->device);
  }
  return true;
}
void cholesky_disable_chain(CholeskyContext* ctx) {
  if (!ctx || !ctx->dq) return;
  std::lock_guard<std::mutex> lock(g_device_queues.operation_mutex());
  ctx->dq->chain_server = 0;
}
bool cholesky_chain_enabled(const CholeskyContext* ctx) { return ctx && ctx->dq && ctx->server && ctx->resident && ctx->dq->chain_server; }
bool cholesky_claim_pair_servers(CholeskyContext* ctx) {
  if (!ctx || !ctx->dq) return false;
  if (ctx->dq->pair_users.fetch_add(1) < 4) return true;
  ctx->dq->pair_users.fetch_sub(1);
  return false;
}
void cholesky_release_pair_servers(CholeskyContext* ctx) { if (ctx && ctx->dq) ctx->dq->pair_users.fetch_sub(1); }

void cholesky_prepare(CholeskyContext* ctx, hipStream_t s) {
  if (!ctx || !ctx->dq || !ctx->server || ctx->prepared) return;
  std::lock_guard<std::mutex> lock(g_device_queues.operation_mutex());
  DeviceQueues& q = *ctx->dq;
  if (!q.chain_server || !ctx->resident) { if (q.queue_choice >= 0) { ctx->use(&q); ctx->prepared = true; } return; }
  if (q.queue_choice < 0) tune_chain_queues(ctx, s);
  ctx->use(&q);
  ctx->prepared = q.queue_choice >= 0;
}

void cholesky_factor(double* S, long ld, int npad, double* Linv, int* info, int group, hipStream_t s, CholeskyContext* ctx,
                     KernelTimer* kt, const int* last, bool allow_chain, int ncols, int tail_rows, const CholeskyPartner* partner, const int* tail) {
  const int nblk = npad / 128;
  if (ncols < 0 || ncols > nblk) ncols = nblk;
  if (tail_rows < 1 || ncols > nblk - tail_rows) tail_rows = 1;
  const int tail_uniform = nblk - tail_rows;
  auto tail0_of = [&](int c) { return tail ? tail[c < nblk ? c : nblk - 1] : tail_uniform; };
  if (ctx && ctx->dq && !ctx->prepared && !(ctx->dq->tuning && ctx->in_trial)) cholesky_prepare(ctx, s);
  const bool la = ctx != nullptr && ctx->panel != nullptr && ctx->bulk != nullptr;
  std::unique_lock<std::mutex> enqueue_lock;
  const auto t_wait0 = std::chrono::steady_clock::now();
  if (la && ctx->dq) enqueue_lock = std::unique_lock<std::mutex>(ctx->dq->enqueue_mutex[ctx->fork ? 1 : 0]);
  struct EnqueueClock {
    std::chrono::steady_clock::time_point t0, t1 = std::chrono::steady_clock::now();
    ~EnqueueClock() {
      const bool on = dev_knobs().debug_chain_abort;
      const double held = std::chrono::duration<double, std::milli>(std::chrono::steady_clock::now() - t1).count();
      const double waited = std::chrono::duration<double, std::milli>(t1 - t0).count();
      if (on && (held > 50.0 || waited > 500.0)) std::fprintf(stderr, "[skeres_amd] cholesky_factor: waited %.1f ms for the device's enqueue lock, enqueued for %.1f ms\n", waited, held);
    }
  } enqueue_clock;
  enqueue_clock.t0 = t_wait0;
  hipStream_t sp = la ? ctx->panel : s;
  hipStream_t sb = la ? ctx->bulk : s;
  hipStream_t sb_prev = sb;
  size_t ev = 0;
  auto order = [&](hipStream_t from, hipStream_t to) {
    if (from == to) return;
    hipEvent_t e = ctx->event(ev++);
    (void)hipEventRecord(e, from);
    (void)hipStreamWaitEvent(to, e, 0);
  };
  auto last_main = [&](int c) { return last ? (last[c] < nblk - 1 ? last[c] : nblk - 1) : nblk - 1; };
  struct Rows { int main, extra, jump; };
  auto rows_from = [&](int first_row, int col) {
    Rows r;
    const int last_row = last_main(col);
    r.main = last_row >= first_row ? last_row - first_row + 1 : 0;
    const int t0 = std::max(tail0_of(col), first_row + r.main);
    r.extra = std::max(0, nblk - t0);
    r.jump = r.extra ? t0 - (first_row + r.main) : 0;
    return r;
  };
  auto update = [&](hipStream_t st, const char* name, double* C, const double* A, const double* B, int K, Rows r, int tiles_n, int flags) {
    const int tiles_m = r.main + r.extra;
    if (tiles_m <= 0 || tiles_n <= 0) return;
    if (kt) kt->begin(name, st);
    if (4 * tiles_m * tiles_n <= g_thin_grid)
      hipLaunchKernelGGL(gemm_update_thin_f64_kernel, dim3(4 * tiles_m * tiles_n), dim3(256), 0, st, C, ld, A, ld, B, ld, K, 4 * tiles_m, flags, 4 * r.main,
                         4 * r.jump);
    else
      hipLaunchKernelGGL(gemm_update_f64_kernel, dim3(2 * tiles_m * tiles_n), dim3(256), 0, st, C, ld, A, ld, B, ld, K, 2 * tiles_m, flags, 2 * r.main,
                         2 * r.jump);
    if (kt) kt->end(name, st);
  };
  auto update_diag = [&](hipStream_t st, const char* name, double* C, const double* A, int K) {
    if (kt) kt->begin(name, st);
    hipLaunchKernelGGL(gemm_diag_f64_kernel, dim3(4), dim3(256), 0, st, C, ld, A, ld, K);
    if (kt) kt->end(name, st);
  };
  hipEvent_t panel_done = nullptr;
  auto panel = [&](int k0, int k1) {
    panel_done = nullptr;
    for (int kb = k0; kb < k1; ++kb) {
      double* Akk = S + (long)kb * 128 * ld + (long)kb * 128;
      const Rows below = rows_from(kb + 1, kb);
      const double* P = S + (long)kb * 128 * ld + (long)k0 * 128;
      const int K = (kb - k0) * 128;
      if (kb > k0) update_diag(sp, "gemm_diag_update", Akk, P, K);
      if (kt) kt->begin("potrf128", sp);
      hipLaunchKernelGGL(potrf128_kernel, dim3(1), dim3(256), potrf128_lds_bytes(), sp, Akk, ld, Linv + (long)kb * 128 * 128, info);
      if (kt) kt->end("potrf128", sp);
      if (below.main + below.extra > 0) {
        double* A21 = Akk + 128 * ld;
        if (kb > k0) update(sp, "gemm_panel_update", A21, P + 128 * ld, P, K, below, 1, 0);
        hipEvent_t stop = nullptr;
        if (la && g_ext_events && kb == k1 - 1) stop = panel_done = ctx->event(ev++);
        if (kt) kt->begin("gemm_trsm", sp);
        if (4 * (below.main + below.extra) <= g_thin_grid)
          hipExtLaunchKernelGGL(trsm_gemm_thin_f64_kernel, dim3(4 * (below.main + below.extra)), dim3(256), 0, sp, nullptr, stop, 0, A21, ld,
                                (const double*)A21, ld, (const double*)(Linv + (long)kb * 128 * 128), 4 * (below.main + below.extra), 4 * below.main,
                                4 * below.jump);
        else
          hipExtLaunchKernelGGL(trsm_gemm_f64_kernel, dim3(2 * (below.main + below.extra)), dim3(256), 0, sp, nullptr, stop, 0, A21, ld,
                                (const double*)A21, ld, (const double*)(Linv + (long)kb * 128 * 128), 2 * (below.main + below.extra), 2 * below.main,
                                2 * below.jump);
        if (kt) kt->end("gemm_trsm", sp);
      }
    }
  };
  const CholeskyPlan plan = cholesky_plan(nblk, group, last, la && allow_chain && ctx->server != nullptr, ncols, tail_rows, tail);
  const std::vector<int>& gb = plan.bounds;
  const int ngroups = (int)gb.size() - 1;
  ChainRanges ranges;
  ranges.n = 0;
  for (int j = 0; j < nblk; ++j)
    if (plan.resident[j] && (j == 0 || !plan.resident[j - 1])) {
      if (ranges.n == 8) { ranges.n = 0; break; }
      int e = j;
      while (e < nblk && plan.resident[e]) ++e;
      ranges.begin[ranges.n] = j; ranges.end[ranges.n] = e; ++ranges.n;
    }
  bool chain = ranges.n > 0 && ctx->dq && ctx->dq->chain_server && ctx->resident && !(kt && kt->times_all());
  int* sync = chain ? ctx->sync_for(nblk) : nullptr;
  if (!sync) chain = false;
  auto is_resident = [&](int k) { return chain && k < nblk && plan.resident[k]; };
  const int local = chain && (g_chain_local == 1 || (g_chain_local == 2 && !(partner && partner->ncols > 0))) ? 1 : 0;
  auto column_grid = [&](int ncrit, int T, int ncand) { return ncrit ? ncand + 4 * T - 4 : 4 * T; };
  const int maxblk = chain ? ctx->sync_blk : 0;
  const char* stamps_file = chain ? dev_knobs().chain_stamps : nullptr;
  hipStream_t srv = nullptr;
  hipEvent_t start_ev = nullptr;
  int start_value = 0;
  struct PartnerState {
    bool on = false; CholeskyPlan plan; int nblk = 0, ncols = 0, tail0 = 0, start_at = 0, maxblk = 0; const int* last = nullptr; const int* tail = nullptr;
    double* S = nullptr; long ld = 0; double* Linv = nullptr; int* sync = nullptr; double* xs = nullptr;
    int next = 0, seq = 0, col_seq = 0;
  } pb;
  struct PartnerStep { ColumnArgs col; ThinSyrkArgs syrk; int Tb; bool next_resident, by_column; };
  auto partner_step = [&](int kB) {
    PartnerStep st;
    auto lm = [&](int c) { return pb.last ? (pb.last[c] < pb.nblk - 1 ? pb.last[c] : pb.nblk - 1) : pb.nblk - 1; };
    auto rf = [&](int first_row, int last_row) {
      Rows r;
      r.main = last_row >= first_row ? last_row - first_row + 1 : 0;
      const int t0 = std::max(pb.tail ? pb.tail[kB] : pb.tail0, first_row + r.main);
      r.extra = std::max(0, pb.nblk - t0);
      r.jump = r.extra ? t0 - (first_row + r.main) : 0;
      return r;
    };
    const int k1 = kB + 1, Lg = lm(kB);
    const Rows rn = rf(k1, Lg), rs = rf(k1 + 1, Lg);
    const int T = rn.main + rn.extra, ncrit = (rn.main > 0 || rn.jump == 0) ? 16 : 0;
    st.Tb = rs.main + rs.extra;
    st.next_resident = k1 < pb.ncols;
    st.by_column = st.next_resident && g_early_column;
    const int ncand = ncrit && local ? kCritCandidates : ncrit;
    st.col = ColumnArgs{pb.S, pb.ld, kB, pb.Linv + (long)kB * 128 * 128, 4 * T, 4 * rn.main, 4 * rn.jump, ncrit, pb.xs, pb.sync, pb.maxblk, pb.seq, pb.col_seq,
                        column_grid(ncrit, T, ncand), ncand};
    st.syrk = ThinSyrkArgs{pb.S + (long)(k1 + 1) * 128 * pb.ld + (long)(k1 + 1) * 128, pb.ld, pb.S + (long)(k1 + 1) * 128 * pb.ld + (long)kB * 128, pb.ld, 128, 4 * st.Tb,
                           4 * rs.main, 4 * rs.jump, rs.main, rs.jump, st.by_column ? pb.sync + kSyncSyrkColumn : (int*)nullptr, st.Tb > 0 ? 2 * st.Tb * (st.Tb + 1) : 0};
    return st;
  };
  auto partner_advance = [&](const PartnerStep& st, hipStream_t bulk_stream) {
    if (st.Tb > 0) {
      if (st.by_column) pb.col_seq += 4 * st.Tb;
      else if (st.next_resident) { ++pb.seq; hipLaunchKernelGGL(chain_marker_kernel, dim3(1), dim3(1), 0, bulk_stream, pb.sync + kSyncSyrkSeq, pb.seq); }
    }
    ++pb.next;
  };
  if (chain) {
    const int stamps_on = stamps_file ? 1 : 0;
    static int stamps_state = 0;
    if (stamps_on != stamps_state) { (void)hipMemcpyToSymbol(HIP_SYMBOL(g_chain_stamps_on), &stamps_on, sizeof(int)); stamps_state = stamps_on; }
    srv = ctx->server;
    hipStreamCaptureStatus capturing = hipStreamCaptureStatusNone;
    if (hipStreamIsCapturing(s, &capturing) != hipSuccess) { (void)hipGetLastError(); capturing = hipStreamCaptureStatusActive; }
    const bool early = dev_knobs().chain_early_server != 0 && capturing == hipStreamCaptureStatusNone;
    if (!early) (void)hipMemsetAsync(sync, 0, sizeof(int) * (size_t)(kSyncHeader + kSyncArrays * maxblk), s);
    if (partner && partner->ncols > 0 && partner->ctx && !(kt && kt->times_all())) {
      pb.plan = cholesky_plan(partner->nblk, group, partner->last, true, partner->ncols, partner->tail_rows, partner->tail);
      bool all = (int)pb.plan.resident.size() >= partner->ncols;
      for (int j = 0; all && j < partner->ncols; ++j) all = pb.plan.resident[j] && !pb.plan.paired[j];
      int start = 0;
      while (start < ncols && !(plan.resident[start] && !plan.paired[start])) ++start;
      int* sb_sync = all && start < ncols ? partner->ctx->sync_for(partner->nblk) : nullptr;
      if (sb_sync && partner->ctx->xs) {
        pb.on = true; pb.start_at = start; pb.sync = sb_sync; pb.maxblk = partner->ctx->sync_blk; pb.xs = partner->ctx->xs;
        pb.nblk = partner->nblk; pb.ncols = partner->ncols; pb.tail0 = partner->nblk - std::max(1, std::min(partner->tail_rows, partner->nblk - partner->ncols));
        pb.last = partner->last; pb.tail = partner->tail; pb.S = partner->S; pb.ld = partner->ld; pb.Linv = partner->Linv;
        if (!early) (void)hipMemsetAsync(pb.sync, 0, sizeof(int) * (size_t)(kSyncHeader + kSyncArrays * pb.maxblk), s);
        partner->taken = true;
      }
    }
    start_ev = ctx->event(ev++);
    (void)hipEventRecord(start_ev, s);
    if (early) {
      static std::atomic<int> epoch{0};
      start_value = 1 + (epoch.fetch_add(1) & 0x3fffffff);
      hipLaunchKernelGGL(chain_start_kernel, dim3(1), dim3(256), 0, s, sync, kSyncHeader + kSyncArrays * maxblk, pb.on ? pb.sync : (int*)nullptr,
                         pb.on ? kSyncHeader + kSyncArrays * pb.maxblk : 0, start_value);
    } else {
      (void)hipStreamWaitEvent(srv, start_ev, 0);
    }
    if (pb.on) {
      ServerPair sp2;
      sp2.f[0] = ServerArgs{S, ld, ranges, Linv, sync, maxblk};
      ChainRanges rb; rb.n = 1; rb.begin[0] = 0; rb.end[0] = pb.ncols;
      sp2.f[1] = ServerArgs{pb.S, pb.ld, rb, pb.Linv, pb.sync, pb.maxblk};
      hipLaunchKernelGGL(potrf_server_pair_kernel, dim3(2), dim3(256), potrf128_lds_bytes(), srv, sp2, info, local, start_value);
    } else {
      hipLaunchKernelGGL(potrf_server_kernel, dim3(1), dim3(256), potrf128_lds_bytes(), srv, S, ld, ranges, Linv, info, sync, maxblk, local, start_value);
    }
  }
  if (la && chain && start_value != 0 && sp != s) {
    hipLaunchKernelGGL(chain_start_gate_kernel, dim3(1), dim3(64), 0, sp, (const int*)(sync + kSyncStart), start_value, info);
  } else if (la) {
    if (!start_ev) { start_ev = ctx->event(ev++); (void)hipEventRecord(start_ev, s); }
    for (hipStream_t q : {sp, ctx->bulk, ctx->bulk_early}) if (q != s) (void)hipStreamWaitEvent(q, start_ev, 0);
  }
  if (!is_resident(0) && ncols > 0) panel(gb[0], gb[1]);
  bool used_bulk_early = false;
  hipEvent_t syrk_done = nullptr;
  hipEvent_t syrk_any = nullptr, syrk_done2 = nullptr;
  int seq = 0;
  int col_seq = 0;
  for (int g = 0; g + 1 < ngroups; ++g) {
    const int k0 = gb[g], k1 = gb[g + 1];
    if (k0 >= ncols) break;
    const int K = (k1 - k0) * 128;
    bool with_partner = false;
    PartnerStep pst{};
    const bool resident = is_resident(k0);
    const bool next_resident = is_resident(k1);
    const bool pair = plan.paired[k0] == 1 && k1 - k0 == 2;
    const bool after_pair = k0 > 0 && plan.paired[k0 - 1] == 2 && is_resident(k0 - 1);
    const int na = pair ? 0 : (resident ? 1 : gb[g + 2] - k1);
    const Rows rn = rows_from(k1, k1 - 1);
    const Rows rs = rows_from(k1 + na, k1 - 1);
    double* A22 = S + (long)k1 * 128 * ld + (long)k1 * 128;
    const double* P = S + (long)k1 * 128 * ld + (long)k0 * 128;
    const int Tb = rs.main + rs.extra;
    if (la) sb = Tb >= ctx->early_tiles ? ctx->bulk_early : ctx->bulk;
    if (la && Tb > 0 && sb == ctx->bulk_early) used_bulk_early = true;
    if (sb != sb_prev && syrk_done) (void)hipStreamWaitEvent(sb, syrk_done, 0);
    sb_prev = sb;
    if (resident && pair) {
      if (syrk_done2) (void)hipStreamWaitEvent(sp, syrk_done2, 0);
      hipEvent_t col_done = ctx->event(ev++);
      for (int c = 0; c < 2; ++c) {
        const Rows rc = rows_from(k0 + c + 1, k0 + c);
        const int T = rc.main + rc.extra;
        const int ncrit = (rc.main > 0 || rc.jump == 0) ? 16 : 0;
        hipExtLaunchKernelGGL(chain_column_kernel, dim3(ncrit ? 16 + 4 * T - 4 : 4 * T), dim3(256), 0, sp, nullptr, c == 1 ? col_done : (hipEvent_t) nullptr, 0, S, ld,
                              k0 + c, (const double*)(Linv + (long)(k0 + c) * 128 * 128), 4 * T, 4 * rc.main, 4 * rc.jump, ncrit, ctx->xs, sync, maxblk, seq, col_seq, info,
                              c == 0 ? 1 : 0, c == 0 && after_pair ? 1 : 0, ncrit);
      }
      (void)hipStreamWaitEvent(sb, col_done, 0);
    } else if (resident) {
      const int T = rn.main + rn.extra;
      const int ncrit = (rn.main > 0 || rn.jump == 0) ? 16 : 0;
      const int ncand = ncrit && local && !after_pair ? kCritCandidates : ncrit;
      with_partner = pb.on && k0 >= pb.start_at && pb.next < pb.ncols && !after_pair && Tb <= g_thin_syrk_tiles && ctx->early_tiles > g_thin_syrk_tiles;
      if (with_partner) pst = partner_step(pb.next);
      hipEvent_t col_done = (Tb > 0 || (with_partner && pst.Tb > 0)) ? ctx->event(ev++) : nullptr;
      if (with_partner) {
        ColumnPair cp;
        cp.f[0] = ColumnArgs{S, ld, k0, Linv + (long)k0 * 128 * 128, 4 * T, 4 * rn.main, 4 * rn.jump, ncrit, ctx->xs, sync, maxblk, seq, col_seq, column_grid(ncrit, T, ncand), ncand};
        cp.f[1] = pst.col;
        hipExtLaunchKernelGGL(chain_column_pair_kernel, dim3(std::max(cp.f[0].grid, cp.f[1].grid), 2), dim3(256), 0, sp, nullptr, col_done, 0, cp, info);
      } else {
        hipExtLaunchKernelGGL(chain_column_kernel, dim3(column_grid(ncrit, T, ncand)), dim3(256), 0, sp, nullptr, col_done, 0, S, ld, k0,
                              (const double*)(Linv + (long)k0 * 128 * 128), 4 * T, 4 * rn.main, 4 * rn.jump, ncrit, ctx->xs, sync, maxblk, seq, col_seq, info, 1, after_pair ? 1 : 0, ncand);
      }
      if (col_done) (void)hipStreamWaitEvent(sb, col_done, 0);
    } else {
      if (panel_done) (void)hipStreamWaitEvent(sb, panel_done, 0);
      else order(sp, sb);
      if (la && syrk_done) (void)hipStreamWaitEvent(sp, syrk_done, 0);
      update(sp, "gemm_syrk_next", A22, P, P, K, rn, na, 1);
    }
    syrk_done = nullptr;
    if (with_partner) {
      const bool by_col = next_resident && g_early_column;
      bool withheld = false;
#ifdef SK_TESTING
      if (next_resident && Tb > 0 && !ctx->dq->tuning) { int want = k1; withheld = want >= 0 && g_test_withhold.compare_exchange_strong(want, -1); }
#endif
      ThinSyrkPair tp;
      tp.f[0] = ThinSyrkArgs{S + (long)(k1 + 1) * 128 * ld + (long)(k1 + 1) * 128, ld, S + (long)(k1 + 1) * 128 * ld + (long)k0 * 128, ld, 128, 4 * Tb, 4 * rs.main, 4 * rs.jump,
                             rs.main, rs.jump, by_col && !withheld ? sync + kSyncSyrkColumn : (int*)nullptr, Tb > 0 ? 2 * Tb * (Tb + 1) : 0};
      tp.f[1] = pst.syrk;
      const int gx = std::max(tp.f[0].grid, tp.f[1].grid);
      hipEvent_t t_start = nullptr, t_stop = nullptr;
      if (kt && gx > 0) kt->pair("gemm_syrk", &t_start, &t_stop);
      hipEvent_t stop_ev = t_stop ? t_stop : ctx->event(ev++);
      if (gx > 0) hipExtLaunchKernelGGL(syrk_trailing_thin_pair_f64_kernel, dim3(gx, 2), dim3(256), 0, sb, t_start, stop_ev, 0, tp);
      if (Tb > 0) {
        if (by_col) col_seq += 4 * Tb;
        else if (next_resident) { ++seq; if (!withheld) hipLaunchKernelGGL(chain_marker_kernel, dim3(1), dim3(1), 0, sb, sync + kSyncSyrkSeq, seq); }
      }
      partner_advance(pst, sb);
      if (gx > 0 && !next_resident) syrk_done = stop_ev;
      syrk_done2 = syrk_any;
      syrk_any = gx > 0 ? stop_ev : nullptr;
    } else if (Tb > 0) {
      double* Cb = S + (long)(k1 + na) * 128 * ld + (long)(k1 + na) * 128;
      const double* Pb = S + (long)(k1 + na) * 128 * ld + (long)k0 * 128;
      bool record = la && (!next_resident || (pair && !resident));
      if (la && !record && g + 3 < (int)gb.size()) {
        const int k2 = gb[g + 2], na1 = (plan.paired[k1] == 1 && k2 - k1 == 2) ? 0 : (is_resident(k1) ? 1 : gb[g + 3] - k2);
        const Rows rs1 = rows_from(k2 + na1, k2 - 1);
        record = (rs1.main + rs1.extra >= ctx->early_tiles) != (sb == ctx->bulk_early);
      }
      hipEvent_t t_start = nullptr, t_stop = nullptr;
      if (kt) kt->pair("gemm_syrk", &t_start, &t_stop);
      hipEvent_t stop_ev = t_stop ? t_stop : ((record || (la && chain)) ? ctx->event(ev++) : nullptr);
      bool withheld = false;
#ifdef SK_TESTING
      if (next_resident && !ctx->dq->tuning) { int want = k1; withheld = want >= 0 && g_test_withhold.compare_exchange_strong(want, -1); }
#endif
      const bool pair_chain = pair && resident;
      const bool thin = Tb <= g_thin_syrk_tiles || pair_chain, by_column = next_resident && thin && (g_early_column || pair_chain);
      const int count_cols = pair_chain ? 2 : 1;
      if (thin)
        hipExtLaunchKernelGGL(syrk_trailing_thin_f64_kernel, dim3(2 * Tb * (Tb + 1)), dim3(256), 0, sb, t_start, stop_ev, 0, Cb, ld, Pb, ld, K, 4 * Tb, 4 * rs.main,
                              4 * rs.jump, rs.main, rs.jump, by_column && !withheld ? sync + kSyncSyrkColumn : (int*)nullptr, count_cols,
                              pair_chain && next_resident && !withheld ? sync + kSyncHeader + k1 : (int*)nullptr);
      else
        hipExtLaunchKernelGGL(syrk_trailing_f64_kernel, dim3(Tb * (Tb + 1) / 2), dim3(256), 0, sb, t_start, stop_ev, 0, Cb, ld, Pb, ld, K, 0, rs.main, rs.jump);
      if (by_column) {
        col_seq += 4 * Tb + (count_cols > 1 && Tb > 1 ? 4 * (Tb - 1) : 0);
      } else if (next_resident) {
        ++seq;
        if (!withheld) hipLaunchKernelGGL(chain_marker_kernel, dim3(1), dim3(1), 0, sb, sync + kSyncSyrkSeq, seq);
      }
      if (record) syrk_done = stop_ev;
      syrk_done2 = syrk_any;
      syrk_any = stop_ev;
    } else {
      syrk_done2 = syrk_any;
      syrk_any = nullptr;
    }
    if (next_resident) {
      if (!resident) hipLaunchKernelGGL(chain_marker_kernel, dim3(1), dim3(1), 0, sp, sync + kSyncHeader + k1, 16);
    } else {
      const int k2 = gb[g + 2];
      if (k1 < ncols) {
        if ((pair || (resident && k2 - k1 > 1)) && la && syrk_done) (void)hipStreamWaitEvent(sp, syrk_done, 0);
        panel(k1, k2);
      }
    }
  }
  while (pb.on && pb.next < pb.ncols) {
    const PartnerStep st = partner_step(pb.next);
    hipEvent_t col_done = st.Tb > 0 ? ctx->event(ev++) : nullptr;
    ColumnPair cp;
    cp.f[0] = st.col; cp.f[1] = st.col; cp.f[1].grid = 0;
    hipExtLaunchKernelGGL(chain_column_pair_kernel, dim3(st.col.grid, 1), dim3(256), 0, sp, nullptr, col_done, 0, cp, info);
    if (st.Tb > 0) {
      (void)hipStreamWaitEvent(ctx->bulk, col_done, 0);
      ThinSyrkPair tp;
      tp.f[0] = st.syrk; tp.f[1] = st.syrk; tp.f[1].grid = 0;
      hipEvent_t t_start = nullptr, t_stop = nullptr;
      if (kt) kt->pair("gemm_syrk", &t_start, &t_stop);
      hipExtLaunchKernelGGL(syrk_trailing_thin_pair_f64_kernel, dim3(st.syrk.grid, 1), dim3(256), 0, ctx->bulk, t_start, t_stop, 0, tp);
    }
    partner_advance(st, ctx->bulk);
  }
  if (chain && start_value != 0) {
    int expected = pb.on ? 2 : 1;
    for (hipStream_t q : {sp, ctx->bulk, used_bulk_early ? ctx->bulk_early : (hipStream_t) nullptr})
      if (q && q != s) { hipLaunchKernelGGL(chain_end_marker_kernel, dim3(1), dim3(64), 0, q, sync + kSyncEnd); ++expected; }
    hipLaunchKernelGGL(chain_gate_kernel, dim3(1), dim3(64), 0, s, (const int*)(sync + kSyncEnd), expected, info);
  } else {
  order(sp, s);
  if (la) { order(ctx->bulk, s); if (used_bulk_early) order(ctx->bulk_early, s); }
  if (chain) order(srv, s);
  }
  if (stamps_file) {
    (void)hipStreamSynchronize(s);
    std::vector<long long> st((size_t)1024 * 8);
    (void)hipMemcpyFromSymbol(st.data(), HIP_SYMBOL(g_chain_stamps), st.size() * sizeof(long long));
    const std::string stamps_name = std::string(stamps_file) + (partner && partner->ncols > 0 ? ".pair" : "");
    if (FILE* f = fopen(stamps_name.c_str(), "w")) {
      for (int j = 0; j < nblk && j < 512; ++j) {
        if (!plan.resident[j]) continue;
        fprintf(f, "%d ", j);
        for (int i = 0; i < 7; ++i) fprintf(f, "%lld ", st[(size_t)j * 8 + i]);
        const Rows rs = rows_from(j + 2, j);
        fprintf(f, "%d\n", rs.main + rs.extra);
      }
      for (int j = 0; partner && j < partner->ncols && j < 512; ++j) {
        fprintf(f, "%d ", 512 + j);
        for (int i = 0; i < 7; ++i) fprintf(f, "%lld ", st[(size_t)(512 + j) * 8 + i]);
        fprintf(f, "0\n");
      }
      fclose(f);
    }
  }
}

bool cholesky_backsolve_resident(int nblk) { return g_bs_resident.load() != 0 && nblk <= kBsMaxBlocks; }
static int bs_janitors(int owners) { return std::max(1, std::min(owners, 96)); }
void cholesky_backsolve(double* S, long ld, int n, int npad, int rhs_row, const double* Linv, double* w, double* y,
                        hipStream_t s, KernelTimer* kt, const int* last, int* info, const int* tail, bool zero_after, int resident, bool prefilled) {
  const int nblk = npad / 128;
  if (info && (resident < 0 ? g_bs_resident.load() != 0 : resident != 0) && nblk <= kBsMaxBlocks) {
    BsTop env;
    for (int c = 0; c < nblk; ++c) {
      env.top[c] = (unsigned short)(last ? std::min(std::max(last[c], c), nblk - 1) : nblk - 1);
      env.tail[c] = (unsigned short)(tail ? std::min(std::max(tail[c], 0), nblk - 1) : nblk - 1);
    }
    if (kt) kt->begin("backsolve", s);
    if (!prefilled) (void)hipMemsetAsync(y, 0xff, sizeof(double) * (size_t)npad, s);
    const char* bs_stamps = dev_knobs().bs_stamps;
    if (bs_stamps) { static bool on = false; if (!on) { const int one = 1; (void)hipMemcpyToSymbol(HIP_SYMBOL(g_bs_stamps_on), &one, sizeof(int)); on = true; } }
    const bool spread = zero_after && dev_knobs().bs_spread != 0;
    const int janitors = zero_after ? bs_janitors(nblk) : 0;
#ifdef SK_TESTING
    if (janitors > 0) { int want = 1; if (g_test_janitor_giveup.compare_exchange_strong(want, 0)) { const int one = 1; (void)hipMemcpyToSymbolAsync(HIP_SYMBOL(g_bs_test_janitor_giveup), &one, sizeof(int), 0, hipMemcpyHostToDevice, s); (void)hipStreamSynchronize(s); } }
#endif
    hipLaunchKernelGGL(bs_resident_kernel, dim3(spread ? 8 * nblk : nblk + janitors), dim3(1024), 0, s, Linv, S, ld, (const double*)(S + (long)rhs_row * ld), n, y, nblk, env, info, nblk,
                       (const double*)nullptr, spread ? -1 : janitors, (const int*)nullptr);
    if (kt) kt->end("backsolve", s);
    if (bs_stamps) {
      (void)hipStreamSynchronize(s);
      std::vector<long long> st((size_t)1024 * 4);
      (void)hipMemcpyFromSymbol(st.data(), HIP_SYMBOL(g_bs_stamps), st.size() * sizeof(long long));
      if (FILE* f = fopen(bs_stamps, "w")) {
        for (int kb = nblk - 1; kb >= 0; --kb) fprintf(f, "%d %lld %lld %lld\n", kb, st[(size_t)kb * 4], st[(size_t)kb * 4 + 1], st[(size_t)kb * 4 + 2]);
        fclose(f);
      }
    }
    return;
  }
  hipLaunchKernelGGL(copy_row_kernel, dim3((npad + 255) / 256), dim3(256), 0, s, S + (long)rhs_row * ld, w, n, npad);
  if (kt) kt->begin("backsolve", s);
  const std::vector<int> first = cholesky_row_first_cols(nblk, last, tail);
  for (int kb = nblk - 1; kb >= 0; --kb) {
    const int ncols = kb * 128, col0 = first[kb] * 128;
    const int grid = ncols > col0 ? (ncols - col0 + 63) / 64 : 1;
    hipLaunchKernelGGL(bs_step_kernel, dim3(grid), dim3(1024), 0, s, Linv + (long)kb * 128 * 128, S + (long)kb * 128 * ld, ld, w, y, kb, col0, ncols);
  }
  if (kt) kt->end("backsolve", s);
}

__global__ __launch_bounds__(256) void border_add_kernel(double* __restrict__ root, long ld_r, const double* __restrict__ border, long ld_f, int m,
                                                         const int* __restrict__ map) {
  const long e = (long)blockIdx.x * 256 + threadIdx.x;
  if (e >= (long)m * m) return;
  const int i = (int)(e / m), j = (int)(e % m);
  if (j > i) return;
  int ri = i, rj = j;
  if (map) { ri = map[i]; rj = map[j]; }
  if (ri < 0 || rj < 0) return;
  const double v = border[(long)i * ld_f + j];
  if (v == 0.0) return;
  if (ri >= rj) root[(long)ri * ld_r + rj] += v;
  else root[(long)rj * ld_r + ri] += v;
}

__global__ __launch_bounds__(1024) void bs_border_kernel(const double* __restrict__ Lb, long ld, int m, const double* __restrict__ yb, double* __restrict__ w,
                                                          int col0, int ncols) {
  __shared__ double red[16 * 64];
  const int t = threadIdx.x, cl = t & 63, rg = t >> 6;
  const int col = col0 + blockIdx.x * 64 + cl;
  double acc = 0.0;
  if (col < ncols)
    for (int r = rg; r < m; r += 16) acc += Lb[(long)r * ld + col] * yb[r];
  red[rg * 64 + cl] = acc;
  __syncthreads();
  if (t < 64 && col < ncols) {
    double u = 0.0;
#pragma unroll
    for (int g = 0; g < 16; ++g) u += red[g * 64 + t];
    w[col] -= u;
  }
}

__global__ void gather_map_kernel(const double* __restrict__ src, const int* __restrict__ map, double* __restrict__ dst, int m) {
  const int i = blockIdx.x * blockDim.x + threadIdx.x;
  if (i < m) dst[i] = map ? (map[i] >= 0 ? src[map[i]] : 0.0) : src[i];
}

__global__ __launch_bounds__(256) void border_add2_kernel(double* __restrict__ root, long ld_r, const double* __restrict__ a, long ld_a, const double* __restrict__ b, long ld_b,
                                                          int m, const int* __restrict__ map) {
  const long e = (long)blockIdx.x * 256 + threadIdx.x;
  if (e >= (long)m * m) return;
  const int i = (int)(e / m), j = (int)(e % m);
  if (j > i) return;
  double v = root[(long)i * ld_r + j];
  bool touched = false;
  const double va = a[(long)i * ld_a + j];
  if (va != 0.0) { v += va; touched = true; }
  const int bi = map[i], bj = map[j];
  if (bi >= 0 && bj >= 0) {
    const double vb = bi >= bj ? b[(long)bi * ld_b + bj] : b[(long)bj * ld_b + bi];
    if (vb != 0.0) { v += vb; touched = true; }
  }
  if (touched) root[(long)i * ld_r + j] = v;
}
void cholesky_border_add(double* root, long ld_r, const double* front, long ld_f, int ncols, int border_blocks, const int* map, hipStream_t s) {
  const int m = border_blocks * 128;
  const long total = (long)m * m;
  hipLaunchKernelGGL(border_add_kernel, dim3((unsigned)((total + 255) / 256)), dim3(256), 0, s, root, ld_r, front + (long)ncols * 128 * ld_f + (long)ncols * 128, ld_f, m, map);
}

void cholesky_backsolve_front(double* S, long ld, int nblk, int ncols, int rhs_row, const double* Linv, const double* yb, double* w, double* y,
                              hipStream_t s, const int* last, bool spike, int tail_rows, int* info, bool zero_after, const int* tail, const int* yb_map, int resident,
                              bool prefilled) {
  const int ni = ncols * 128, m = (nblk - ncols) * 128;
  if (ncols <= 0) return;
  const bool res = info && (resident < 0 ? g_bs_resident.load() != 0 : resident != 0) && nblk <= kBsMaxBlocks;
  if (yb_map && !res) {
    std::fprintf(stderr, "[skeres_amd] internal: cholesky_backsolve_front got a border map without the resident launch\n");
    if (info) (void)hipMemsetAsync(info, 0x7f, sizeof(int), s);
    return;
  }
  if (res) {
    if (tail_rows < 1 || tail_rows > nblk - ncols) tail_rows = 1;
    BsTop env;
    for (int c = 0; c < nblk; ++c) {
      env.top[c] = (unsigned short)(last ? std::min(std::max(last[c], c), nblk - 1) : nblk - 1);
      env.tail[c] = (unsigned short)(tail ? std::min(std::max(tail[c], 0), nblk - 1) : nblk - tail_rows);
    }
    if (!prefilled) (void)hipMemsetAsync(y, 0xff, sizeof(double) * (size_t)ni, s);
    const bool spread = zero_after && dev_knobs().bs_spread != 0;
    const int janitors = zero_after ? bs_janitors(ncols) : 0;
    hipLaunchKernelGGL(bs_resident_kernel, dim3(spread ? 8 * ncols : ncols + janitors), dim3(1024), 0, s, Linv, S, ld, (const double*)(S + (long)rhs_row * ld), ni, y, nblk, env, info, ncols, yb,
                       spread ? -1 : janitors, yb_map);
    return;
  }
  hipLaunchKernelGGL(copy_row_kernel, dim3((ni + 255) / 256), dim3(256), 0, s, S + (long)rhs_row * ld, w, ni, ni);
  std::vector<int> first(nblk, 0);
  int c0 = 0;
  if (last)
    for (int kb = 0; kb < nblk - 1; ++kb) {
      while (c0 < kb && last[c0] < kb) ++c0;
      first[kb] = c0;
    }
  const int bfirst = first[ncols < nblk - 1 ? ncols : nblk - 1];
  const int bcol0 = (spike || tail) ? 0 : std::min(bfirst, ncols) * 128;
  if (ni > bcol0)
    hipLaunchKernelGGL(bs_border_kernel, dim3((ni - bcol0 + 63) / 64), dim3(1024), 0, s, S + (long)ncols * 128 * ld, ld, m, yb, w, bcol0, ni);
  for (int kb = ncols - 1; kb >= 0; --kb) {
    const int nc = kb * 128, col0 = first[kb] * 128;
    const int grid = nc > col0 ? (nc - col0 + 63) / 64 : 1;
    hipLaunchKernelGGL(bs_step_kernel, dim3(grid), dim3(1024), 0, s, Linv + (long)kb * 128 * 128, S + (long)kb * 128 * ld, ld, w, y, kb, col0, nc);
  }
}

static void fork_join_events(CholeskyContext* c) {
  if (!c->fork_ev) (void)hipEventCreateWithFlags(&c->fork_ev, g_event_flags);
  if (!c->join_ev) (void)hipEventCreateWithFlags(&c->join_ev, g_event_flags);
}

void cholesky_dissected_factor(const DissectedSystem& d, int* info, int group, hipStream_t s, CholeskyContext* ctxA, CholeskyContext* ctxB,
                               KernelTimer* kt, KernelTimer* ktB, bool allow_chain) {
  if (d.A.ncols > 0 && d.B.ncols > 0 && ctxA && ctxB && allow_chain) {
    CholeskyPartner pt{d.B.S, d.B.ld, d.B.nblk, d.B.ncols, 1, d.B.last, d.B.Linv, ctxB, d.B.tail};
    cholesky_factor(d.A.S, d.A.ld, d.A.nblk * 128, d.A.Linv, info, group, s, ctxA, kt, d.A.last, allow_chain, d.A.ncols, 1, &pt, d.A.tail);
    if (!pt.taken)
      cholesky_factor(d.B.S, d.B.ld, d.B.nblk * 128, d.B.Linv, info, group, s, ctxA, kt, d.B.last, allow_chain, d.B.ncols, 1, nullptr, d.B.tail);
    cholesky_border_add(d.R.S, d.R.ld, d.A.S, d.A.ld, d.A.ncols, d.border_blocks, nullptr, s);
    cholesky_border_add(d.R.S, d.R.ld, d.B.S, d.B.ld, d.B.ncols, d.border_blocks, d.mapB, s);
    cholesky_factor(d.R.S, d.R.ld, d.R.nblk * 128, d.R.Linv, info, group, s, ctxA, kt, d.R.last, allow_chain);
    return;
  }
  const bool side = d.B.ncols > 0 && ctxB && ctxB->fork;
  if (d.B.ncols > 0 && !side) {
    cholesky_factor(d.B.S, d.B.ld, d.B.nblk * 128, d.B.Linv, info, group, s, ctxA, kt, d.B.last, allow_chain && ctxB && ctxB->server, d.B.ncols, 1, nullptr, d.B.tail);
  } else if (side) {
    fork_join_events(ctxB);
    hipStream_t sB = ctxB->fork;
    (void)hipEventRecord(ctxB->fork_ev, s);
    (void)hipStreamWaitEvent(sB, ctxB->fork_ev, 0);
    const bool chainB = allow_chain && ctxB->server != nullptr;
    if (!ctxB->runner) ctxB->runner.reset(new AsyncRunner(ctxB->device));
    ctxB->runner->run([&d, info, group, ctxB, ktB, sB, chainB] {
      cholesky_factor(d.B.S, d.B.ld, d.B.nblk * 128, d.B.Linv, info, group, sB, ctxB, ktB, d.B.last, chainB, d.B.ncols, 1, nullptr, d.B.tail);
      (void)hipEventRecord(ctxB->join_ev, sB);
    });
  }
  if (d.A.ncols > 0) cholesky_factor(d.A.S, d.A.ld, d.A.nblk * 128, d.A.Linv, info, group, s, ctxA, kt, d.A.last, allow_chain, d.A.ncols, 1, nullptr, d.A.tail);
  if (side) {
    ctxB->runner->wait();
    (void)hipStreamWaitEvent(s, ctxB->join_ev, 0);
  }
  if (d.A.ncols > 0 && d.B.ncols > 0 && d.mapB && d.mapB_involution) {
    const int m = d.border_blocks * 128;
    hipLaunchKernelGGL(border_add2_kernel, dim3((unsigned)(((long)m * m + 255) / 256)), dim3(256), 0, s, d.R.S, d.R.ld,
                       (const double*)(d.A.S + (long)d.A.ncols * 128 * d.A.ld + (long)d.A.ncols * 128), d.A.ld,
                       (const double*)(d.B.S + (long)d.B.ncols * 128 * d.B.ld + (long)d.B.ncols * 128), d.B.ld, m, d.mapB);
  } else {
    if (d.A.ncols > 0) cholesky_border_add(d.R.S, d.R.ld, d.A.S, d.A.ld, d.A.ncols, d.border_blocks, nullptr, s);
    if (d.B.ncols > 0) cholesky_border_add(d.R.S, d.R.ld, d.B.S, d.B.ld, d.B.ncols, d.border_blocks, d.mapB, s);
  }
  cholesky_factor(d.R.S, d.R.ld, d.R.nblk * 128, d.R.Linv, info, group, s, ctxA, kt, d.R.last, allow_chain);
}

void cholesky_dissected_backsolve(const DissectedSystem& d, int n_root, double* wR, double* yR, double* wA, double* yA, double* wB, double* yB, double* ybB,
                                  hipStream_t s, CholeskyContext* ctxB, KernelTimer* kt, int* info, bool zero_after, int resident, bool prefilled) {
  if (resident < 0) resident = g_bs_resident.load() != 0 ? 1 : 0;
  cholesky_backsolve(d.R.S, d.R.ld, n_root, d.R.nblk * 128, d.R.rhs_row, d.R.Linv, wR, yR, s, nullptr, d.R.last, info, nullptr, zero_after, resident, prefilled);
  if (kt) kt->begin("backsolve", s);
  const int m = d.border_blocks * 128;
  const bool paired = dev_knobs().bs_pair != 0 && d.A.ncols > 0 && d.B.ncols > 0 && info && resident != 0 && d.A.nblk <= kBsPairMaxBlocks && d.B.nblk <= kBsPairMaxBlocks;
  const bool side = !paired && d.B.ncols > 0 && d.A.ncols > 0 && ctxB && ctxB->fork;
  hipStream_t sB = s;
  if (paired) {
    BsPair p;
    const bool spread = zero_after && dev_knobs().bs_spread != 0;
    const FrontView* fv[2] = {&d.A, &d.B};
    double* ys[2] = {yA, yB};
    int grid = 0, jan = 0;
    for (int f = 0; f < 2; ++f) {
      const FrontView& F = *fv[f];
      for (int c = 0; c < F.nblk; ++c) {
        p.env[f].top[c] = (unsigned short)(F.last ? std::min(std::max(F.last[c], c), F.nblk - 1) : F.nblk - 1);
        p.env[f].tail[c] = (unsigned short)(F.tail ? std::min(std::max(F.tail[c], 0), F.nblk - 1) : F.nblk - 1);
      }
      const int janitors = spread ? 3 * F.ncols : (zero_after ? bs_janitors(F.ncols) : 0);
      p.f[f] = BsArgs{F.Linv, F.S, F.ld, (const double*)(F.S + (long)F.rhs_row * F.ld), F.ncols * 128, ys[f], F.nblk, info, F.ncols, yR, janitors, f == 1 ? d.mapB : nullptr,
                      spread ? 3 : 0, spread ? 1 : 0};
      grid += F.ncols; jan += janitors;
    }
    if (spread) { grid = 8 * std::max(d.A.ncols, d.B.ncols); jan = 0; }
    const size_t nA = (size_t)d.A.ncols * 128, nB = (size_t)d.B.ncols * 128;
    if (prefilled) {}
    else if (yB >= yA + nA && (size_t)(yB - yA) <= nA + 4096) (void)hipMemsetAsync(yA, 0xff, sizeof(double) * ((size_t)(yB - yA) + nB), s);
    else { (void)hipMemsetAsync(yA, 0xff, sizeof(double) * nA, s); (void)hipMemsetAsync(yB, 0xff, sizeof(double) * nB, s); }
    hipLaunchKernelGGL(bs_resident_pair_kernel, dim3(grid + jan), dim3(1024), 0, s, p);
  } else {
  if (d.B.ncols > 0) {
    if (side) {
      fork_join_events(ctxB);
      (void)hipEventRecord(ctxB->fork_ev, s);
      (void)hipStreamWaitEvent(ctxB->fork, ctxB->fork_ev, 0);
      sB = ctxB->fork;
    }
    const bool mapped = info && resident != 0 && d.B.nblk <= kBsMaxBlocks;
    if (!mapped) cholesky_gather_map(yR, d.mapB, ybB, m, sB);
    cholesky_backsolve_front(d.B.S, d.B.ld, d.B.nblk, d.B.ncols, d.B.rhs_row, d.B.Linv, mapped ? yR : ybB, wB, yB, sB, d.B.last, false, 1, info, zero_after, d.B.tail,
                             mapped ? d.mapB : nullptr, resident, prefilled);
  }
  }
  if (!paired && d.A.ncols > 0) cholesky_backsolve_front(d.A.S, d.A.ld, d.A.nblk, d.A.ncols, d.A.rhs_row, d.A.Linv, yR, wA, yA, s, d.A.last, false, 1, info, zero_after, d.A.tail, nullptr, resident, prefilled);
  if (side) {
    (void)hipEventRecord(ctxB->join_ev, ctxB->fork);
    (void)hipStreamWaitEvent(s, ctxB->join_ev, 0);
  }
  if (kt) kt->end("backsolve", s);
}

void cholesky_gather_map(const double* src, const int* map, double* dst, int m, hipStream_t s) {
  hipLaunchKernelGGL(gather_map_kernel, dim3((m + 255) / 256), dim3(256), 0, s, src, map, dst, m);
}

void launch_syrk_gram(double* H, long ldh, const double* A, long lda, int Kc, int nslabs, double* slabs, int tiles, hipStream_t s,
                      KernelTimer* kt) {
  if (tiles <= 0) return;
  const size_t slab_stride = (size_t)tiles * 128 * ldh;
  if (kt) kt->begin("syrk_gram", s);
  hipLaunchKernelGGL(syrk_gram_f64_kernel, dim3(tiles * (tiles + 1) / 2, nslabs), dim3(256), 0, s, nslabs > 1 ? slabs : H, ldh, slab_stride, A, lda, Kc);
  if (kt) kt->end("syrk_gram", s);
  if (nslabs > 1) hipLaunchKernelGGL(gram_reduce_kernel, dim3(tiles * (tiles + 1) / 2), dim3(256), 0, s, H, slabs, slab_stride, ldh, nslabs);
}

double cholesky_syrk_flops(int npad, int group, const int* last, bool chain, double* c_tiles, int ncols, int tail_rows, const int* tail) {
  const int nblk = npad / 128;
  const BlockEnvelope env(nblk, last, tail, ncols, tail_rows);
  ncols = env.ncols;
  const CholeskyPlan plan = cholesky_plan(nblk, group, last, chain, ncols, env.tail_rows, tail);
  const std::vector<int>& gb = plan.bounds;
  double f = 0.0, tiles = 0.0;
  for (size_t g = 0; g + 2 < gb.size(); ++g) {
    if (gb[g] >= ncols) break;
    const int k0 = gb[g], k1 = gb[g + 1];
    const int na = (plan.paired[k0] == 1 && k1 - k0 == 2) ? 0 : (plan.resident[k0] ? 1 : gb[g + 2] - k1);
    const int Tb = env.active_rows(k1 - 1, k1 + na);
    f += 0.5 * Tb * (Tb + 1.0) * 2.0 * 128.0 * 128.0 * (double)((k1 - k0) * 128);
    tiles += 0.5 * Tb * (Tb + 1.0);
  }
  if (c_tiles) *c_tiles = tiles;
  return f;
}

}
```

skeres_amd/csrc/chol_kernels.hpp:

```cpp
#pragma once
#include <hip/hip_runtime.h>
#include <condition_variable>
#include <cstdint>
#include <functional>
#include <map>
#include <memory>
#include <mutex>
#include <thread>
#include <string>
#include <vector>

#include "chol_envelope.hpp"
#include "dev_knobs.hpp"

namespace sk {

class KernelTimer {
 public:
  struct Stat { double seconds = 0.0; int launches = 0; };
  void enable(bool on) { enabled_ = on; }
  void only(const std::string& name) { only_ = name; }
  bool enabled() const { return enabled_; }
  bool times_all() const { return enabled_ && only_.empty(); }
  void begin(const char* name, hipStream_t s) {
// ... 56 lines not shown
  std::map<std::string, Stat> stats_;
};

class AsyncRunner {
 public:
  explicit AsyncRunner(int device) : device_(device) {}
  ~AsyncRunner() {
    { std::lock_guard<std::mutex> l(m_); stop_ = true; }
    cv_.notify_all();
    if (th_.joinable()) th_.join();
  }
  void run(std::function<void()> job) {
    wait();
    { std::lock_guard<std::mutex> l(m_); job_ = std::move(job); busy_ = true; }
    if (!th_.joinable()) th_ = std::thread([this] { loop(); });
    cv_.notify_all();
  }
  void wait() {
    std::unique_lock<std::mutex> l(m_);
    cv_.wait(l, [this] { return !busy_; });
  }

 private:
  void loop() {
    (void)hipSetDevice(device_);
    for (;;) {
      std::function<void()> job;
      {
        std::unique_lock<std::mutex> l(m_);
        cv_.wait(l, [this] { return stop_ || (busy_ && job_); });
        if (stop_) return;
        job = std::move(job_); job_ = nullptr;
      }
      job();
      { std::lock_guard<std::mutex> l(m_); busy_ = false; }
      cv_.notify_all();
    }
  }
  int device_;
  std::thread th_;
  std::mutex m_;
  std::condition_variable cv_;
  std::function<void()> job_;
  bool busy_ = false, stop_ = false;
};

struct DeviceQueues;
struct CholeskyContext {
  DeviceQueues* dq = nullptr;
  bool prepared = false;
  bool in_trial = false;
  bool resident = true;
  int device = -1;
  void use(DeviceQueues* q);
  hipStream_t panel = nullptr;
  hipStream_t bulk = nullptr;
  hipStream_t bulk_early = nullptr;
  int early_tiles = 0;
  int reserved_cus = 0;
  hipStream_t server = nullptr;
  int* sync = nullptr;
  int sync_blk = 0;
  double* xs = nullptr;
  int* sync_for(int nblk);
  std::vector<hipEvent_t> events;
  hipError_t init();
  hipError_t init_secondary(const CholeskyContext& primary);
  hipStream_t fork = nullptr;
  hipEvent_t fork_ev = nullptr, join_ev = nullptr;
  std::unique_ptr<AsyncRunner> runner;
  hipEvent_t event(size_t i);
  ~CholeskyContext();
};

hipError_t cholesky_init();
size_t potrf128_lds_bytes();
struct CholeskyPartner {
  double* S; long ld; int nblk, ncols, tail_rows; const int* last; double* Linv; CholeskyContext* ctx;
  const int* tail = nullptr;
  mutable bool taken = false;
};
void cholesky_factor(double* S, long ld, int npad, double* Linv, int* info, int group, hipStream_t s, CholeskyContext* ctx,
                     KernelTimer* kt, const int* last = nullptr, bool allow_chain = false, int ncols = -1, int tail_rows = 1,
                     const CholeskyPartner* partner = nullptr, const int* tail = nullptr);
void cholesky_prepare(CholeskyContext* ctx, hipStream_t s);
bool cholesky_note_info(CholeskyContext* ctx, int info);
bool cholesky_chain_enabled(const CholeskyContext* ctx);
bool cholesky_claim_pair_servers(CholeskyContext* ctx);
void cholesky_release_pair_servers(CholeskyContext* ctx);
void cholesky_disable_chain(CholeskyContext* ctx);
void cholesky_backsolve(double* S, long ld, int n, int npad, int rhs_row, const double* Linv, double* w, double* y,
                        hipStream_t s, KernelTimer* kt, const int* last = nullptr, int* info = nullptr, const int* tail = nullptr, bool zero_after = false, int resident = -1,
                        bool prefilled = false);
bool cholesky_backsolve_resident(int nblk);
struct FrontView {
  double* S = nullptr; long ld = 0;
  int nblk = 0, ncols = 0;
  const int* last = nullptr;
  double* Linv = nullptr;
  int rhs_row = 0;
  int tail_rows = 1;
  bool spike = false;
  const int* tail = nullptr;
};
struct DissectedSystem {
  FrontView A, B, R;
  int border_blocks = 0;
  const int* mapB = nullptr;
  bool mapB_involution = false;
};
void cholesky_dissected_factor(const DissectedSystem& d, int* info, int group, hipStream_t s, CholeskyContext* ctxA, CholeskyContext* ctxB,
                               KernelTimer* kt, KernelTimer* ktB, bool allow_chain);
void cholesky_dissected_backsolve(const DissectedSystem& d, int n_root, double* wR, double* yR, double* wA, double* yA, double* wB, double* yB, double* ybB,
                                  hipStream_t s, CholeskyContext* ctxB, KernelTimer* kt, int* info = nullptr, bool zero_after = false, int resident = -1, bool prefilled = false);
void cholesky_border_add(double* root, long ld_r, const double* front, long ld_f, int ncols, int border_blocks, const int* map, hipStream_t s);
void cholesky_backsolve_front(double* S, long ld, int nblk, int ncols, int rhs_row, const double* Linv, const double* yb, double* w, double* y,
                              hipStream_t s, const int* last, bool spike = false, int tail_rows = 1, int* info = nullptr, bool zero_after = false, const int* tail = nullptr,
                              const int* yb_map = nullptr,
                              int resident = -1, bool prefilled = false);
void cholesky_gather_map(const double* src, const int* map, double* dst, int m, hipStream_t s);
void launch_syrk_gram(double* H, long ldh, const double* A, long lda, int Kc, int nslabs, double* slabs, int tiles, hipStream_t s,
                      KernelTimer* kt);

}
```

skeres_amd/csrc/chol_solve.hip:

```cpp
#include "chol_solve.hpp"

#include <memory>

#include "chol_fronts.hpp"
#include "chol_kernels.hpp"
#include "common.hpp"

namespace sk {
namespace {

struct SolveDevice {
  CholeskyContext ctx;
  StreamGuard stream;
  bool la = false;
  int open(bool prepare) {
    if (sk_device_count() <= 0) { set_error("no HIP device available: libskeres_amd has no CPU fallback"); return SK_ERR_NO_DEVICE; }
    SK_HIP_TRY(cholesky_init());
    la = ctx.init() == hipSuccess;
    if (!la) (void)hipGetLastError();
    SK_HIP_TRY(hipStreamCreateWithFlags(&stream.s, hipStreamNonBlocking));
    if (prepare && la) cholesky_prepare(&ctx, stream.s);
    return SK_OK;
  }
  CholeskyContext* context() { return la ? &ctx : nullptr; }
  bool chain(int automatic_plan) const { return automatic_plan != 0 && la && ctx.server != nullptr; }
  int close(const int* dinfo) {
    int info = 0;
    SK_HIP_TRY(hipMemcpyAsync(&info, dinfo, sizeof(int), hipMemcpyDeviceToHost, stream.s));
    SK_HIP_TRY(hipStreamSynchronize(stream.s));
    if (info == 2) { (void)cholesky_note_info(&ctx, info); set_error("the resident panel chain timed out"); return SK_ERR_HIP; }
    if (info) { set_error("matrix is not positive definite"); return SK_ERR_EVALUATION_FAILED; }
    return SK_OK;
  }
};

int group_or_automatic(int group, int automatic_plan) { return group > 0 ? group : automatic_plan ? 1 : 3; }

hipError_t download(std::vector<double>& h, const double* d, hipStream_t s) { return hipMemcpyAsync(h.data(), d, h.size() * sizeof(double), hipMemcpyDeviceToHost, s); }

const int* envelope_of(const std::vector<int>& last) { return last.empty() ? nullptr : last.data(); }

}

int cholesky_solve_single(int n, const double* A, const double* b, double* x, double* L, int group, const int* last, int automatic_plan, int border_begin_row) {
  if (last) {
    const int c = invalid_envelope_column(n, last);
    if (c >= 0) { set_error("invalid block envelope at block column %d", c); return SK_ERR_INVALID_ARGUMENT; }
  }
  SolveDevice dev;
  if (const int rc = dev.open(false)) return rc;
  hipStream_t s = dev.stream.s;
  group = group_or_automatic(group, automatic_plan);
  SingleFront f = single_front(n, A, b, border_begin_row);
  const int npad = f.npad;
  const int* tail = nullptr;
  if (border_begin_row >= 0) { last = f.last.data(); tail = f.tail.data(); }
  DevBuf<double> dS, dLinv, dw, dy; DevBuf<int> dinfo;
  SK_HIP_TRY(dS.upload(f.S, s)); SK_HIP_TRY(dLinv.alloc((size_t)npad * 128)); SK_HIP_TRY(dLinv.zero(s));
  SK_HIP_TRY(dy.alloc(npad)); SK_HIP_TRY(dw.alloc(npad)); SK_HIP_TRY(dinfo.alloc(1)); SK_HIP_TRY(dinfo.zero(s));
  cholesky_factor(dS.p, npad, npad, dLinv.p, dinfo.p, group, s, dev.context(), nullptr, last, dev.chain(automatic_plan), -1, 1, nullptr, tail);
  cholesky_backsolve(dS.p, npad, n, npad, f.rhs_row, dLinv.p, dw.p, dy.p, s, nullptr, last, dinfo.p, tail);
  if (const int rc = dev.close(dinfo.p)) return rc;
  std::vector<double> y(npad);
  SK_HIP_TRY(download(y, dy.p, s));
  if (L) SK_HIP_TRY(download(f.S, dS.p, s));
  SK_HIP_TRY(hipStreamSynchronize(s));
  single_front_solution(f, y, x);
  if (L) single_front_factor(f, f.S, L);
  return SK_OK;
}

int cholesky_solve_two_way(int n, const double* A, const double* b, double* x, int head, int tail_begin, int group, int automatic_plan) {
  const std::string why = two_way_check(n, A, head, tail_begin);
  if (!why.empty()) { set_error("%s", why.c_str()); return SK_ERR_INVALID_ARGUMENT; }
  SolveDevice dev;
  if (const int rc = dev.open(true)) return rc;
  hipStream_t s = dev.stream.s;
  CholeskyContext ctxB;
  const bool side = dev.la && ctxB.init_secondary(dev.ctx) == hipSuccess;
  if (dev.la && !side) (void)hipGetLastError();
  group = group_or_automatic(group, automatic_plan);
  const TwoWayFronts f = two_way_fronts(n, A, b, head, tail_begin);
  const size_t dA = f.A.dim, dB = f.B.dim, dR = f.R.dim;
  DevBuf<double> dFA, dFB, dFR, dLinv, dw, dy; DevBuf<int> dinfo, dmap;
  SK_HIP_TRY(dFA.upload(f.A.F, s)); SK_HIP_TRY(dFB.upload(f.B.F, s)); SK_HIP_TRY(dFR.upload(f.R.F, s)); SK_HIP_TRY(dmap.upload(f.mapB, s));
  SK_HIP_TRY(dLinv.alloc((size_t)(f.A.ncols + f.B.ncols + f.R.ncols) * 128 * 128)); SK_HIP_TRY(dLinv.zero(s));
  SK_HIP_TRY(dw.alloc(dA + dB + 2 * dR)); SK_HIP_TRY(dy.alloc(dA + dB + dR)); SK_HIP_TRY(dy.zero(s)); SK_HIP_TRY(dinfo.alloc(1)); SK_HIP_TRY(dinfo.zero(s));
  auto view = [](const HostFront& h, double* S, double* Linv) {
    FrontView v;
    v.S = S; v.ld = (long)h.dim; v.nblk = h.nblk; v.ncols = h.ncols; v.last = envelope_of(h.last); v.Linv = Linv; v.rhs_row = h.rhs_row;
    return v;
  };
  DissectedSystem d;
  d.A = view(f.A, dFA.p, dLinv.p);
  d.B = view(f.B, dFB.p, dLinv.p + (size_t)f.A.ncols * 128 * 128);
  d.R = view(f.R, dFR.p, dLinv.p + (size_t)(f.A.ncols + f.B.ncols) * 128 * 128);
  d.border_blocks = f.border_blocks; d.mapB = dmap.p;
  cholesky_dissected_factor(d, dinfo.p, group, s, dev.context(), side ? &ctxB : nullptr, nullptr, nullptr, dev.chain(automatic_plan));
  double *wA = dw.p, *wB = dw.p + dA, *wR = dw.p + dA + dB, *ybB = dw.p + dA + dB + dR;
  double *yA = dy.p, *yB = dy.p + dA, *yR = dy.p + dA + dB;
  cholesky_dissected_backsolve(d, f.sep_n, wR, yR, wA, yA, wB, yB, ybB, s, side ? &ctxB : nullptr, nullptr, dinfo.p);
  if (const int rc = dev.close(dinfo.p)) return rc;
  std::vector<double> y(dA + dB + dR);
  SK_HIP_TRY(download(y, dy.p, s));
  SK_HIP_TRY(hipStreamSynchronize(s));
  two_way_scatter(f, y.data(), x);
  return SK_OK;
}

int cholesky_solve_multi_way(int n, const double* A, const double* b, double* x, int num_segments, const int* cuts, int group, int automatic_plan) {
  const int R = num_segments;
  SegmentCuts c;
  const std::string why = segment_cuts(n, A, R, cuts, &c);
  if (!why.empty()) { set_error("%s", why.c_str()); return SK_ERR_INVALID_ARGUMENT; }
  SolveDevice dev;
  if (const int rc = dev.open(true)) return rc;
  hipStream_t s = dev.stream.s;
  group = group_or_automatic(group, automatic_plan);
  const bool chain = dev.chain(automatic_plan);
  const HostFront root = segments_root(c, A, b);
  const size_t dR = root.dim;
  const int* lastR = envelope_of(root.last);
  DevBuf<double> dFR; DevBuf<int> dinfo;
  SK_HIP_TRY(dFR.upload(root.F, s)); SK_HIP_TRY(dinfo.alloc(1)); SK_HIP_TRY(dinfo.zero(s));
  struct Leaf { LeafFront f; std::vector<double> yh; DevBuf<double> F, Linv, w, y, yb; DevBuf<int> dmap; };
  std::vector<std::unique_ptr<Leaf>> leaves;
  for (int k = 0; k < R; ++k) {
    std::unique_ptr<Leaf> lf(new Leaf());
    lf->f = segment_leaf(c, A, b, k);
    const SegmentLayout& L = lf->f.L;
    const size_t d = lf->f.dim, border = d - (size_t)L.ncols * 128;
    SK_HIP_TRY(lf->F.upload(lf->f.F, s)); SK_HIP_TRY(lf->dmap.upload(lf->f.map, s));
    SK_HIP_TRY(lf->Linv.alloc((size_t)L.ncols * 128 * 128)); SK_HIP_TRY(lf->Linv.zero(s));
    SK_HIP_TRY(lf->w.alloc(d)); SK_HIP_TRY(lf->y.alloc(d)); SK_HIP_TRY(lf->y.zero(s)); SK_HIP_TRY(lf->yb.alloc(border));
    if (lf->f.interior_n > 0) {
      cholesky_factor(lf->F.p, (long)d, (int)d, lf->Linv.p, dinfo.p, group, s, dev.context(), nullptr, lf->f.last.data(), chain, L.ncols, L.tail_rows);
      cholesky_border_add(dFR.p, (long)dR, lf->F.p, (long)d, L.ncols, L.nblk - L.ncols, lf->dmap.p, s);
    }
    SK_HIP_TRY(hipStreamSynchronize(s));
    std::vector<double>().swap(lf->f.F);
    leaves.push_back(std::move(lf));
  }
  DevBuf<double> dLinvR, dwR, dyR;
  SK_HIP_TRY(dLinvR.alloc(dR * 128)); SK_HIP_TRY(dLinvR.zero(s)); SK_HIP_TRY(dwR.alloc(dR)); SK_HIP_TRY(dyR.alloc(dR));
  cholesky_factor(dFR.p, (long)dR, (int)dR, dLinvR.p, dinfo.p, group, s, dev.context(), nullptr, lastR, chain);
  cholesky_backsolve(dFR.p, (long)dR, c.nroot, (int)dR, c.nroot, dLinvR.p, dwR.p, dyR.p, s, nullptr, lastR, dinfo.p);
  for (auto& lf : leaves) {
    const SegmentLayout& L = lf->f.L;
    if (L.ncols == 0) continue;
    const int m = (L.nblk - L.ncols) * 128;
    DevBuf<int> dg;
    SK_HIP_TRY(dg.upload(lf->f.gmap, s));
    cholesky_gather_map(dyR.p, dg.p, lf->yb.p, m, s);
    cholesky_backsolve_front(lf->F.p, (long)lf->f.dim, L.nblk, L.ncols, L.rhs_row, lf->Linv.p, lf->yb.p, lf->w.p, lf->y.p, s, lf->f.last.data(), L.spike, L.tail_rows, dinfo.p);
    SK_HIP_TRY(hipStreamSynchronize(s));
  }
  if (const int rc = dev.close(dinfo.p)) return rc;
  std::vector<double> yR(dR);
  SK_HIP_TRY(download(yR, dyR.p, s));
  for (auto& lf : leaves) { lf->yh.resize(lf->f.dim); SK_HIP_TRY(download(lf->yh, lf->y.p, s)); }
  SK_HIP_TRY(hipStreamSynchronize(s));
  segments_scatter_root(c, yR.data(), x);
  for (auto& lf : leaves) segments_scatter_leaf(lf->f, lf->yh.data(), x);
  return SK_OK;
}

}
```

skeres_amd/csrc/chol_solve.hpp:

```cpp
#pragma once

namespace sk {

int cholesky_solve_single(int n, const double* A, const double* b, double* x, double* L, int group, const int* last, int automatic_plan, int border_begin_row);
int cholesky_solve_two_way(int n, const double* A, const double* b, double* x, int head, int tail_begin, int group, int automatic_plan);
int cholesky_solve_multi_way(int n, const double* A, const double* b, double* x, int num_segments, const int* cuts, int group, int automatic_plan);

}
```

Before: 263.6.

## Add nested-dissection tree Cholesky solve with lock-step group kernels for up to four fronts

Adds a dissection-tree Cholesky solver (two to four leaves, optional middle separators and a bordered root). Sibling fronts at each level are factored and back-solved together by widening the former pair kernels (server, column, thin syrk, chain start, resident backsolve) to groups of up to four fronts. The goal is to run independent fronts concurrently in single launches and cut per-front launch and serialization cost. It adds a new API entry point, and it is unclear whether the default LM iteration path uses it.

New measurement: 260.9. -1.0%, worse.

```diff
diff --git a/include/skeres_amd.h b/include/skeres_amd.h
--- a/include/skeres_amd.h
+++ b/include/skeres_amd.h
@@ -343,6 +343,10 @@
 
 int sk_cholesky_solve_segments(int n, const double* A, const double* b, double* x, int num_segments, const int* cuts, int group,
                                int automatic_plan);
+int sk_cholesky_solve_tree(int n, const double* A, const double* b, double* x, int num_segments, const int* cuts, int border_begin,
+                           int group, int automatic_plan, int lock_step, double* factors, long factor_doubles);
+long sk_cholesky_tree_factor_doubles(int n, int num_segments, const int* cuts, int border_begin);
+int sk_cholesky_tree_fronts_in_lock_step(void);
 
 #ifdef __cplusplus
 }
diff --git a/skeres_amd/api.py b/skeres_amd/api.py
--- a/skeres_amd/api.py
+++ b/skeres_amd/api.py
@@ -163,6 +163,9 @@
     "sk_allreduce_rccl_calls": (C.c_long, [C.c_void_p]),
     "sk_allreduce_rccl_fn": (C.c_void_p, []),
     "sk_cholesky_solve_segments": (C.c_int, [C.c_int, _dp, _dp, _dp, C.c_int, _ip, C.c_int, C.c_int]),
+    "sk_cholesky_solve_tree": (C.c_int, [C.c_int, _dp, _dp, _dp, C.c_int, _ip, C.c_int, C.c_int, C.c_int, C.c_int, _dp, C.c_long]),
+    "sk_cholesky_tree_factor_doubles": (C.c_long, [C.c_int, C.c_int, _ip, C.c_int]),
+    "sk_cholesky_tree_fronts_in_lock_step": (C.c_int, []),
     "sk_cholesky_solve_ex": (C.c_int, [C.c_int, _dp, _dp, _dp, _dp, C.c_int, _ip, C.c_int]),
     "sk_problem_border_plan": (C.c_int, [C.c_void_p, C.c_int, C.POINTER(C.c_int), _ip, C.POINTER(C.c_int), C.POINTER(C.c_double), C.POINTER(C.c_double), C.POINTER(C.c_double)]),
     "sk_cholesky_solve_bordered": (C.c_int, [C.c_int, _dp, _dp, _dp, _dp, C.c_int, C.c_int, C.c_int]),
@@ -1602,6 +1605,25 @@
     return x
 
 
+def cholesky_solve_tree(A, b, cuts, border_begin=-1, group=0, automatic_plan=True, lock_step=True, want_factors=False):
+    A = np.ascontiguousarray(A, dtype=np.float64)
+    b = np.ascontiguousarray(b, dtype=np.float64)
+    n = A.shape[0]
+    x = np.empty(n)
+    c = np.ascontiguousarray(np.asarray(cuts, dtype=np.int32).reshape(-1))
+    cp = c.ctypes.data_as(_ip)
+    factors, fp, count = None, _dp(), 0
+    if want_factors:
+        count = lib().sk_cholesky_tree_factor_doubles(n, len(cuts) + 1, cp, int(border_begin))
+        if count < 0:
+            raise ValueError(lib().sk_last_error().decode())
+        factors = np.empty(count)
+        fp = factors.ctypes.data_as(_dp)
+    _check(lib().sk_cholesky_solve_tree(n, A.ctypes.data_as(_dp), b.ctypes.data_as(_dp), x.ctypes.data_as(_dp), len(cuts) + 1, cp, int(border_begin),
+                                        int(group), int(bool(automatic_plan)), int(bool(lock_step)), fp, count))
+    return (x, factors) if want_factors else x
+
+
 def synth_dense_targets(seed, m, n, x_star):
     xs = np.ascontiguousarray(x_star, dtype=np.float64)
     y = np.empty(int(m))
diff --git a/skeres_amd/csrc/capi.hip b/skeres_amd/csrc/capi.hip
--- a/skeres_amd/csrc/capi.hip
+++ b/skeres_amd/csrc/capi.hip
@@ -1147,5 +1147,19 @@
   return cholesky_solve_multi_way(n, A, b, x, num_segments, cuts, group, automatic_plan);
   SK_GUARD_END(SK_ERR_INVALID_ARGUMENT)
 }
-
-}
+int sk_cholesky_solve_tree(int n, const double* A, const double* b, double* x, int num_segments, const int* cuts, int border_begin, int group, int automatic_plan,
+                           int lock_step, double* factors, long factor_doubles) {
+  SK_GUARD_BEGIN
+  if (n <= 0 || !A || !b || !x || num_segments < 2 || num_segments > 4 || !cuts || border_begin > n || (factors && factor_doubles <= 0)) { set_error("invalid argument"); return SK_ERR_INVALID_ARGUMENT; }
+  return cholesky_solve_tree(n, A, b, x, num_segments, cuts, border_begin, group, automatic_plan, lock_step, factors, factor_doubles);
+  SK_GUARD_END(SK_ERR_INVALID_ARGUMENT)
+}
+int sk_cholesky_tree_fronts_in_lock_step(void) { return cholesky_tree_fronts_in_lock_step(); }
+long sk_cholesky_tree_factor_doubles(int n, int num_segments, const int* cuts, int border_begin) {
+  SK_GUARD_BEGIN
+  if (n <= 0 || num_segments < 2 || num_segments > 4 || !cuts || border_begin > n) { set_error("invalid argument"); return -1; }
+  return cholesky_tree_factor_doubles(n, num_segments, cuts, border_begin);
+  SK_GUARD_END(-1)
+}
+
+}
diff --git a/skeres_amd/csrc/chol_fronts.cpp b/skeres_amd/csrc/chol_fronts.cpp
--- a/skeres_amd/csrc/chol_fronts.cpp
+++ b/skeres_amd/csrc/chol_fronts.cpp
@@ -191,4 +191,137 @@
   for (int t = 0; t < f.L.ncols * 128; ++t) if (f.order[t] >= 0) x[f.order[t]] = y[t];
 }
 
-}
+namespace {
+struct TreeShape {
+  int R = 0, n = 0, border_begin = 0;
+  std::vector<int> sb, se;
+  int root_sep() const { return R >= 3 ? 2 : 1; }
+  int nmid() const { return R >= 4 ? 2 : R == 3 ? 1 : 0; }
+  int mid_sep(int m) const { return m == 0 ? 1 : 3; }
+  int leaf_parent(int k) const { return R == 2 ? -1 : k < 2 ? 0 : R == 4 ? 1 : -1; }
+  int parent_front(int f) const { return f < 4 ? (leaf_parent(f) >= 0 ? 4 + leaf_parent(f) : 6) : f < 6 ? 6 : -1; }
+  int front_of(int row) const {
+    if (row >= border_begin) return 6;
+    for (int k = 1; k < R; ++k)
+      if (row >= sb[k] && row < se[k]) return k == root_sep() ? 6 : k == 1 ? 4 : 5;
+    for (int k = 0; k < R; ++k) if (row >= se[k] && row < sb[k + 1]) return k;
+    return -1;
+  }
+  std::vector<int> rows_of(int f) const {
+    std::vector<int> r;
+    auto range = [&r](int lo, int hi) { for (int i = lo; i < hi; ++i) r.push_back(i); };
+    if (f < 4) range(se[f], sb[f + 1]);
+    else if (f < 6) range(sb[mid_sep(f - 4)], se[mid_sep(f - 4)]);
+    else { range(sb[root_sep()], se[root_sep()]); range(border_begin, n); }
+    return r;
+  }
+};
+std::string tree_shape(int n, int R, const int* cuts, int border_begin, TreeShape* out) {
+  TreeShape& t = *out;
+  if (R < 2 || R > 4) return "a dissection tree has two to four segments";
+  t.R = R; t.n = n; t.border_begin = border_begin < 0 ? n : border_begin;
+  if (t.border_begin > n) return "invalid cuts";
+  t.sb.assign(R + 1, 0); t.se.assign(R + 1, 0);
+  t.sb[R] = t.border_begin;
+  for (int k = 1; k < R; ++k) { t.sb[k] = cuts[2 * (k - 1)]; t.se[k] = cuts[2 * (k - 1) + 1]; }
+  for (int k = 1; k <= R; ++k)
+    if (t.sb[k] < t.se[k - 1] || (k < R && (t.se[k] < t.sb[k] || t.se[k] > t.border_begin))) return "invalid cuts";
+  return std::string();
+}
+}
+
+std::string tree_check(int n, const double* A, int R, const int* cuts, int border_begin) {
+  TreeShape t;
+  const std::string why = tree_shape(n, R, cuts, border_begin, &t);
+  if (!why.empty()) return why;
+  std::vector<int> front(n);
+  for (int i = 0; i < n; ++i) front[i] = t.front_of(i);
+  auto under = [&t](int f, int g) { for (f = t.parent_front(f); f >= 0; f = t.parent_front(f)) if (f == g) return true; return false; };
+  for (int i = 0; i < n; ++i)
+    for (int j = 0; j < i; ++j) {
+      if (A[(size_t)i * n + j] == 0.0) continue;
+      const int fi = front[i], fj = front[j];
+      if (fi != fj && !under(fi, fj) && !under(fj, fi)) return format("rows %d and %d couple across the tree: not a separator", i, j);
+    }
+  return std::string();
+}
+
+TreeFronts tree_fronts(int n, const double* A, const double* b, int R, const int* cuts, int border_begin) {
+  TreeFronts out;
+  TreeShape t;
+  if (!tree_shape(n, R, cuts, border_begin, &t).empty()) return out;
+  out.n = n; out.nleaves = R; out.nmid = t.nmid();
+  auto front = [&out](int f) -> TreeFrontHost& { return f < 4 ? out.leaf[f] : f < 6 ? out.mid[f - 4] : out.root; };
+  const int sequence[7] = {6, 4, 5, 0, 1, 2, 3};
+  for (int f : sequence) {
+    if ((f < 4 && f >= R) || (f >= 4 && f < 6 && f - 4 >= out.nmid)) continue;
+    TreeFrontHost& F = front(f);
+    const std::vector<int> own = t.rows_of(f);
+    const int ni = (int)own.size();
+    F.interior_n = ni;
+    HostFront& h = F.h;
+    if (f == 6) {
+      h.nblk = h.ncols = (ni + 1 + 127) / 128; h.rhs_row = ni; F.border_n = 0;
+    } else {
+      const TreeFrontHost& P = front(t.parent_front(f));
+      F.parent = f < 4 ? t.leaf_parent(f) : -1;
+      F.border_n = P.interior_n + P.border_n;
+      h.ncols = (ni + 127) / 128;
+      F.tail_rows = (F.border_n + 1 + 127) / 128;
+      h.nblk = h.ncols + F.tail_rows;
+      h.rhs_row = h.ncols * 128 + F.border_n;
+    }
+    h.dim = (size_t)h.nblk * 128;
+    const size_t d = h.dim;
+    const int bo = f == 6 ? 0 : h.ncols * 128;
+    F.order.assign(d, -1);
+    for (int k = 0; k < ni; ++k) F.order[k] = own[k];
+    if (f != 6) {
+      const TreeFrontHost& P = front(t.parent_front(f));
+      const int pbo = &P == &out.root ? 0 : P.h.ncols * 128;
+      F.map.assign(d - bo, -1);
+      int k = 0;
+      for (int q = 0; q < P.interior_n; ++q, ++k) { F.order[bo + k] = P.order[q]; F.map[k] = q; }
+      for (int q = 0; q < P.border_n; ++q, ++k) { F.order[bo + k] = P.order[pbo + q]; F.map[k] = pbo + q; }
+      F.ymap = F.map;
+      F.map[F.border_n] = P.h.rhs_row;
+    }
+    h.F.assign(d * d, 0.0);
+    for (size_t i = 0; i < d; ++i) {
+      const int gi = F.order[i];
+      if (gi < 0) continue;
+      for (size_t j = 0; j <= i && j < (size_t)ni; ++j) h.F[i * d + j] = sym(A, n, gi, F.order[j]);
+    }
+    for (int k = 0; k < ni; ++k) h.F[(size_t)h.rhs_row * d + k] = b[own[k]];
+    if (f == 6) {
+      h.F[(size_t)ni * d + ni] = 1e300;
+      for (size_t j = (size_t)ni + 1; j < d; ++j) h.F[j * d + j] = 1.0;
+    } else {
+      for (int i = ni; i < bo; ++i) h.F[(size_t)i * d + i] = 1.0;
+      if (f < 4) h.last = host_block_envelope(h.F, d, h.nblk, F.tail_rows);
+    }
+  }
+  return out;
+}
+
+long tree_factor_doubles(int n, int R, const int* cuts, int border_begin) {
+  TreeShape t;
+  if (!tree_shape(n, R, cuts, border_begin, &t).empty()) return -1;
+  long rows[7] = {0, 0, 0, 0, 0, 0, 0}, total = 0;
+  const int sequence[7] = {6, 4, 5, 0, 1, 2, 3};
+  for (int f : sequence) {
+    if ((f < 4 && f >= R) || (f >= 4 && f < 6 && f - 4 >= t.nmid())) continue;
+    const long ni = (long)t.rows_of(f).size();
+    long dim;
+    if (f == 6) { rows[f] = ni; dim = (ni + 1 + 127) / 128 * 128; }
+    else { const long border = rows[t.parent_front(f)]; rows[f] = ni + border; dim = ((ni + 127) / 128 + (border + 1 + 127) / 128) * 128; }
+    total += dim * dim;
+  }
+  return total;
+}
+
+void tree_scatter(const TreeFrontHost& f, const double* y, double* x) {
+  for (int k = 0; k < f.interior_n; ++k) x[f.order[k]] = y[k];
+}
+
+}
diff --git a/skeres_amd/csrc/chol_fronts.hpp b/skeres_amd/csrc/chol_fronts.hpp
--- a/skeres_amd/csrc/chol_fronts.hpp
+++ b/skeres_amd/csrc/chol_fronts.hpp
@@ -59,4 +59,22 @@
 void segments_scatter_root(const SegmentCuts& c, const double* yR, double* x);
 void segments_scatter_leaf(const LeafFront& f, const double* y, double* x);
 
+struct TreeFrontHost {
+  HostFront h;
+  int tail_rows = 1;
+  int parent = -1;
+  int interior_n = 0, border_n = 0;
+  std::vector<int> order;
+  std::vector<int> map;
+  std::vector<int> ymap;
+};
+struct TreeFronts {
+  int n = 0, nleaves = 0, nmid = 0;
+  TreeFrontHost leaf[4], mid[2], root;
+};
+std::string tree_check(int n, const double* A, int R, const int* cuts, int border_begin);
+TreeFronts tree_fronts(int n, const double* A, const double* b, int R, const int* cuts, int border_begin);
+void tree_scatter(const TreeFrontHost& f, const double* y, double* x);
+long tree_factor_doubles(int n, int R, const int* cuts, int border_begin);
+
 }
diff --git a/skeres_amd/csrc/chol_kernels.hip b/skeres_amd/csrc/chol_kernels.hip
--- a/skeres_amd/csrc/chol_kernels.hip
+++ b/skeres_amd/csrc/chol_kernels.hip
@@ -181,9 +181,10 @@
   SK_GEMM_LDS(16, 32, 128)
   gemm_nt_f64_body<0, 2, 16, 2, 32, 128>(sh, C, ldc, A, lda, A, lda, K, tiles_m, 0, main_t, jump_t, main_n, jump_n, -1, first_column_done, count_cols, diag_done);
 }
+constexpr int kMaxGroupFronts = 4;
 struct ThinSyrkArgs { double* C; long ldc; const double* A; long lda; int K, tiles_m, main_t, jump_t, main_n, jump_n; int* first_column_done; int grid; };
-struct ThinSyrkPair { ThinSyrkArgs f[2]; };
-__global__ __launch_bounds__(256, 2) void syrk_trailing_thin_pair_f64_kernel(ThinSyrkPair pair) {
+struct ThinSyrkGroup { ThinSyrkArgs f[kMaxGroupFronts]; };
+__global__ __launch_bounds__(256, 2) void syrk_trailing_thin_pair_f64_kernel(ThinSyrkGroup pair) {
   const ThinSyrkArgs& p = pair.f[blockIdx.y];
   if ((int)blockIdx.x >= p.grid) return;
   SK_GEMM_LDS(16, 32, 128)
@@ -856,18 +857,19 @@
   potrf_server_body(lds, S, ld, ranges, Linv, info, sync, maxblk, local, start);
   if (start != 0) chain_end_signal(sync + kSyncEnd);
 }
-__global__ __launch_bounds__(256) void chain_start_kernel(int* sync_a, int n_a, int* sync_b, int n_b, int value) {
-  for (int i = threadIdx.x; i < n_a; i += 256) sync_a[i] = 0;
-  if (sync_b) for (int i = threadIdx.x; i < n_b; i += 256) sync_b[i] = 0;
+struct ChainStartArgs { int* sync[4]; int n[4]; };
+__global__ __launch_bounds__(256) void chain_start_kernel(ChainStartArgs a, int value) {
+  for (int f = 0; f < 4; ++f)
+    if (a.sync[f]) for (int i = threadIdx.x; i < a.n[f]; i += 256) a.sync[f][i] = 0;
   __syncthreads();
   if (threadIdx.x != 0) return;
   __builtin_amdgcn_fence(__ATOMIC_RELEASE, "agent");
-  __hip_atomic_store(sync_a + kSyncStart, value, __ATOMIC_RELAXED, __HIP_MEMORY_SCOPE_AGENT);
-  if (sync_b) __hip_atomic_store(sync_b + kSyncStart, value, __ATOMIC_RELAXED, __HIP_MEMORY_SCOPE_AGENT);
+  for (int f = 0; f < 4; ++f)
+    if (a.sync[f]) __hip_atomic_store(a.sync[f] + kSyncStart, value, __ATOMIC_RELAXED, __HIP_MEMORY_SCOPE_AGENT);
 }
 struct ServerArgs { double* S; long ld; ChainRanges ranges; double* Linv; int* sync; int maxblk; };
-struct ServerPair { ServerArgs f[2]; };
-__global__ __launch_bounds__(256, 1) void potrf_server_pair_kernel(ServerPair pair, int* info, int local, int start) {
+struct ServerGroup { ServerArgs f[kMaxGroupFronts]; };
+__global__ __launch_bounds__(256, 1) void potrf_server_pair_kernel(ServerGroup pair, int* info, int local, int start) {
   extern __shared__ __attribute__((aligned(16))) double lds[];
   const ServerArgs& p = pair.f[blockIdx.x];
   potrf_server_body(lds, p.S, p.ld, p.ranges, p.Linv, info, p.sync, p.maxblk, local, start);
@@ -1086,8 +1088,8 @@
   chain_column_body((int)blockIdx.x, S, ld, j, Linv_j, tiles_m, main_t, jump_t, ncrit, Xs, sync, maxblk, syrk_need, column_need, info, do_next, wait_first, ncand);
 }
 struct ColumnArgs { double* S; long ld; int j; const double* Linv_j; int tiles_m, main_t, jump_t, ncrit; double* Xs; int* sync; int maxblk, syrk_need, column_need, grid, ncand; };
-struct ColumnPair { ColumnArgs f[2]; };
-__global__ __launch_bounds__(256, 2) void chain_column_pair_kernel(ColumnPair pair, int* info) {
+struct ColumnGroup { ColumnArgs f[kMaxGroupFronts]; };
+__global__ __launch_bounds__(256, 2) void chain_column_pair_kernel(ColumnGroup pair, int* info) {
   const ColumnArgs& p = pair.f[blockIdx.y];
   if ((int)blockIdx.x >= p.grid) return;
   chain_column_body((int)blockIdx.x, p.S, p.ld, p.j, p.Linv_j, p.tiles_m, p.main_t, p.jump_t, p.ncrit, p.Xs, p.sync, p.maxblk, p.syrk_need, p.column_need, info, 1, 0, p.ncand);
@@ -1330,6 +1332,44 @@
   } else {
     const int j = b - own;
     if (j < p.f[0].janitors) { front = 0; blk = nA + j; } else { front = 1; blk = nB + (j - p.f[0].janitors); }
+  }
+  bs_resident_body(p.f[front], p.env[front], blk);
+}
+
+constexpr int kBsGroupMaxBlocks = 224;
+struct BsTopQuarter { unsigned short top[kBsGroupMaxBlocks]; unsigned short tail[kBsGroupMaxBlocks]; };
+struct BsGroup { BsArgs f[kMaxGroupFronts]; BsTopQuarter env[kMaxGroupFronts]; int nf; };
+static_assert(sizeof(BsGroup) <= 4096, "the kernel-argument segment");
+__global__ __launch_bounds__(1024, 1) void bs_resident_group_kernel(BsGroup p) {
+  const int b = (int)blockIdx.x;
+  if (p.f[0].jan_parts > 0) {
+    const int g = b >> 3, slot = b & 7, front = slot >> 1;
+    if (front >= p.nf) return;
+    const int nown = p.f[front].nown;
+    if (g >= nown) return;
+    bs_resident_body(p.f[front], p.env[front], (slot & 1) == 0 ? g : nown + g);
+    return;
+  }
+  int own = 0;
+  for (int f = 0; f < p.nf; ++f) own += p.f[f].nown;
+  int front = 0, blk = 0;
+  if (b < own) {
+    int rem = b;
+    for (int r = 0;; ++r) {
+      int live = 0;
+      for (int f = 0; f < p.nf; ++f) live += p.f[f].nown > r ? 1 : 0;
+      if (rem < live) {
+        for (int f = 0; f < p.nf; ++f) if (p.f[f].nown > r && rem-- == 0) { front = f; break; }
+        blk = r;
+        break;
+      }
+      rem -= live;
+    }
+  } else {
+    int j = b - own;
+    while (front < p.nf - 1 && j >= p.f[front].janitors) { j -= p.f[front].janitors; ++front; }
+    if (j >= p.f[front].janitors) return;
+    blk = p.f[front].nown + j;
   }
   bs_resident_body(p.f[front], p.env[front], blk);
 }
@@ -1411,7 +1451,7 @@
   int queue_choice = -1;
   std::atomic<bool> tuning{false};
   std::atomic<int> chain_server{1};
-  std::atomic<int> pair_users{0};
+  std::atomic<int> group_server_cus{0};
   hipStream_t fork = nullptr;
   hipStream_t plain[2] = {nullptr, nullptr};
   std::mutex enqueue_mutex[2];
@@ -1796,13 +1836,15 @@
   ctx->dq->chain_server = 0;
 }
 bool cholesky_chain_enabled(const CholeskyContext* ctx) { return ctx && ctx->dq && ctx->server && ctx->resident && ctx->dq->chain_server; }
-bool cholesky_claim_pair_servers(CholeskyContext* ctx) {
-  if (!ctx || !ctx->dq) return false;
-  if (ctx->dq->pair_users.fetch_add(1) < 4) return true;
-  ctx->dq->pair_users.fetch_sub(1);
+bool cholesky_claim_group_servers(CholeskyContext* ctx, int fronts) {
+  if (!ctx || !ctx->dq || fronts < 2 || fronts > kMaxGroupFronts) return false;
+  if (ctx->dq->group_server_cus.fetch_add(fronts) + fronts <= 8) return true;
+  ctx->dq->group_server_cus.fetch_sub(fronts);
   return false;
 }
-void cholesky_release_pair_servers(CholeskyContext* ctx) { if (ctx && ctx->dq) ctx->dq->pair_users.fetch_sub(1); }
+void cholesky_release_group_servers(CholeskyContext* ctx, int fronts) { if (ctx && ctx->dq) ctx->dq->group_server_cus.fetch_sub(fronts); }
+bool cholesky_claim_pair_servers(CholeskyContext* ctx) { return cholesky_claim_group_servers(ctx, 2); }
+void cholesky_release_pair_servers(CholeskyContext* ctx) { cholesky_release_group_servers(ctx, 2); }
 
 void cholesky_prepare(CholeskyContext* ctx, hipStream_t s) {
   if (!ctx || !ctx->dq || !ctx->server || ctx->prepared) return;
@@ -1815,7 +1857,7 @@
 }
 
 void cholesky_factor(double* S, long ld, int npad, double* Linv, int* info, int group, hipStream_t s, CholeskyContext* ctx,
-                     KernelTimer* kt, const int* last, bool allow_chain, int ncols, int tail_rows, const CholeskyPartner* partner, const int* tail) {
+                     KernelTimer* kt, const int* last, bool allow_chain, int ncols, int tail_rows, const CholeskyPartner* partner, const int* tail, int npartners) {
   const int nblk = npad / 128;
   if (ncols < 0 || ncols > nblk) ncols = nblk;
   if (tail_rows < 1 || ncols > nblk - tail_rows) tail_rows = 1;
@@ -1931,9 +1973,12 @@
     bool on = false; CholeskyPlan plan; int nblk = 0, ncols = 0, tail0 = 0, start_at = 0, maxblk = 0; const int* last = nullptr; const int* tail = nullptr;
     double* S = nullptr; long ld = 0; double* Linv = nullptr; int* sync = nullptr; double* xs = nullptr;
     int next = 0, seq = 0, col_seq = 0;
-  } pb;
+  } pbs[kMaxGroupFronts - 1];
+  int npb = 0;
+  if (!partner) npartners = 0;
+  npartners = std::max(0, std::min(npartners, kMaxGroupFronts - 1));
   struct PartnerStep { ColumnArgs col; ThinSyrkArgs syrk; int Tb; bool next_resident, by_column; };
-  auto partner_step = [&](int kB) {
+  auto partner_step = [&](const PartnerState& pb, int kB) {
     PartnerStep st;
     auto lm = [&](int c) { return pb.last ? (pb.last[c] < pb.nblk - 1 ? pb.last[c] : pb.nblk - 1) : pb.nblk - 1; };
     auto rf = [&](int first_row, int last_row) {
@@ -1957,7 +2002,7 @@
                            4 * rs.main, 4 * rs.jump, rs.main, rs.jump, st.by_column ? pb.sync + kSyncSyrkColumn : (int*)nullptr, st.Tb > 0 ? 2 * st.Tb * (st.Tb + 1) : 0};
     return st;
   };
-  auto partner_advance = [&](const PartnerStep& st, hipStream_t bulk_stream) {
+  auto partner_advance = [&](PartnerState& pb, const PartnerStep& st, hipStream_t bulk_stream) {
     if (st.Tb > 0) {
       if (st.by_column) pb.col_seq += 4 * st.Tb;
       else if (st.next_resident) { ++pb.seq; hipLaunchKernelGGL(chain_marker_kernel, dim3(1), dim3(1), 0, bulk_stream, pb.sync + kSyncSyrkSeq, pb.seq); }
@@ -1973,19 +2018,27 @@
     if (hipStreamIsCapturing(s, &capturing) != hipSuccess) { (void)hipGetLastError(); capturing = hipStreamCaptureStatusActive; }
     const bool early = dev_knobs().chain_early_server != 0 && capturing == hipStreamCaptureStatusNone;
     if (!early) (void)hipMemsetAsync(sync, 0, sizeof(int) * (size_t)(kSyncHeader + kSyncArrays * maxblk), s);
-    if (partner && partner->ncols > 0 && partner->ctx && !(kt && kt->times_all())) {
-      pb.plan = cholesky_plan(partner->nblk, group, partner->last, true, partner->ncols, partner->tail_rows, partner->tail);
-      bool all = (int)pb.plan.resident.size() >= partner->ncols;
-      for (int j = 0; all && j < partner->ncols; ++j) all = pb.plan.resident[j] && !pb.plan.paired[j];
+    for (int ip = 0; ip < npartners; ++ip) partner[ip].taken = false;
+    for (int ip = 0; ip < npartners; ++ip) {
+      const CholeskyPartner* pt = partner + ip;
+      if (!(pt->ncols > 0 && pt->ctx && !(kt && kt->times_all()))) continue;
+      bool own_counters = pt->ctx != ctx;
+      for (int q = 0; q < ip; ++q) own_counters = own_counters && !(partner[q].taken && partner[q].ctx == pt->ctx);
+      if (!own_counters) continue;
+      PartnerState& pb = pbs[npb];
+      pb.plan = cholesky_plan(pt->nblk, group, pt->last, true, pt->ncols, pt->tail_rows, pt->tail);
+      bool all = (int)pb.plan.resident.size() >= pt->ncols;
+      for (int j = 0; all && j < pt->ncols; ++j) all = pb.plan.resident[j] && !pb.plan.paired[j];
       int start = 0;
       while (start < ncols && !(plan.resident[start] && !plan.paired[start])) ++start;
-      int* sb_sync = all && start < ncols ? partner->ctx->sync_for(partner->nblk) : nullptr;
-      if (sb_sync && partner->ctx->xs) {
-        pb.on = true; pb.start_at = start; pb.sync = sb_sync; pb.maxblk = partner->ctx->sync_blk; pb.xs = partner->ctx->xs;
-        pb.nblk = partner->nblk; pb.ncols = partner->ncols; pb.tail0 = partner->nblk - std::max(1, std::min(partner->tail_rows, partner->nblk - partner->ncols));
-        pb.last = partner->last; pb.tail = partner->tail; pb.S = partner->S; pb.ld = partner->ld; pb.Linv = partner->Linv;
+      int* sb_sync = all && start < ncols ? pt->ctx->sync_for(pt->nblk) : nullptr;
+      if (sb_sync && pt->ctx->xs) {
+        pb.on = true; pb.start_at = start; pb.sync = sb_sync; pb.maxblk = pt->ctx->sync_blk; pb.xs = pt->ctx->xs;
+        pb.nblk = pt->nblk; pb.ncols = pt->ncols; pb.tail0 = pt->nblk - std::max(1, std::min(pt->tail_rows, pt->nblk - pt->ncols));
+        pb.last = pt->last; pb.tail = pt->tail; pb.S = pt->S; pb.ld = pt->ld; pb.Linv = pt->Linv;
         if (!early) (void)hipMemsetAsync(pb.sync, 0, sizeof(int) * (size_t)(kSyncHeader + kSyncArrays * pb.maxblk), s);
-        partner->taken = true;
+        pt->taken = true;
+        ++npb;
       }
     }
     start_ev = ctx->event(ev++);
@@ -1993,17 +2046,22 @@
     if (early) {
       static std::atomic<int> epoch{0};
       start_value = 1 + (epoch.fetch_add(1) & 0x3fffffff);
-      hipLaunchKernelGGL(chain_start_kernel, dim3(1), dim3(256), 0, s, sync, kSyncHeader + kSyncArrays * maxblk, pb.on ? pb.sync : (int*)nullptr,
-                         pb.on ? kSyncHeader + kSyncArrays * pb.maxblk : 0, start_value);
+      ChainStartArgs sa{};
+      sa.sync[0] = sync; sa.n[0] = kSyncHeader + kSyncArrays * maxblk;
+      for (int ip = 0; ip < npb; ++ip) { sa.sync[1 + ip] = pbs[ip].sync; sa.n[1 + ip] = kSyncHeader + kSyncArrays * pbs[ip].maxblk; }
+      hipLaunchKernelGGL(chain_start_kernel, dim3(1), dim3(256), 0, s, sa, start_value);
     } else {
       (void)hipStreamWaitEvent(srv, start_ev, 0);
     }
-    if (pb.on) {
-      ServerPair sp2;
+    if (npb > 0) {
+      ServerGroup sp2{};
       sp2.f[0] = ServerArgs{S, ld, ranges, Linv, sync, maxblk};
-      ChainRanges rb; rb.n = 1; rb.begin[0] = 0; rb.end[0] = pb.ncols;
-      sp2.f[1] = ServerArgs{pb.S, pb.ld, rb, pb.Linv, pb.sync, pb.maxblk};
-      hipLaunchKernelGGL(potrf_server_pair_kernel, dim3(2), dim3(256), potrf128_lds_bytes(), srv, sp2, info, local, start_value);
+      for (int ip = 0; ip < npb; ++ip) {
+        const PartnerState& pb = pbs[ip];
+        ChainRanges rb; rb.n = 1; rb.begin[0] = 0; rb.end[0] = pb.ncols;
+        sp2.f[1 + ip] = ServerArgs{pb.S, pb.ld, rb, pb.Linv, pb.sync, pb.maxblk};
+      }
+      hipLaunchKernelGGL(potrf_server_pair_kernel, dim3(1 + npb), dim3(256), potrf128_lds_bytes(), srv, sp2, info, local, start_value);
     } else {
       hipLaunchKernelGGL(potrf_server_kernel, dim3(1), dim3(256), potrf128_lds_bytes(), srv, S, ld, ranges, Linv, info, sync, maxblk, local, start_value);
     }
@@ -2025,7 +2083,8 @@
     if (k0 >= ncols) break;
     const int K = (k1 - k0) * 128;
     bool with_partner = false;
-    PartnerStep pst{};
+    PartnerStep pst[kMaxGroupFronts - 1] = {};
+    int live[kMaxGroupFronts - 1] = {0, 0, 0}, nlive = 0;
     const bool resident = is_resident(k0);
     const bool next_resident = is_resident(k1);
     const bool pair = plan.paired[k0] == 1 && k1 - k0 == 2;
@@ -2056,14 +2115,19 @@
       const int T = rn.main + rn.extra;
       const int ncrit = (rn.main > 0 || rn.jump == 0) ? 16 : 0;
       const int ncand = ncrit && local && !after_pair ? kCritCandidates : ncrit;
-      with_partner = pb.on && k0 >= pb.start_at && pb.next < pb.ncols && !after_pair && Tb <= g_thin_syrk_tiles && ctx->early_tiles > g_thin_syrk_tiles;
-      if (with_partner) pst = partner_step(pb.next);
-      hipEvent_t col_done = (Tb > 0 || (with_partner && pst.Tb > 0)) ? ctx->event(ev++) : nullptr;
+      nlive = 0;
+      if (npb > 0 && k0 >= pbs[0].start_at && !after_pair && Tb <= g_thin_syrk_tiles && ctx->early_tiles > g_thin_syrk_tiles)
+        for (int ip = 0; ip < npb; ++ip) if (pbs[ip].next < pbs[ip].ncols) { live[nlive] = ip; pst[nlive] = partner_step(pbs[ip], pbs[ip].next); ++nlive; }
+      with_partner = nlive > 0;
+      bool any_syrk = Tb > 0;
+      for (int q = 0; q < nlive; ++q) any_syrk = any_syrk || pst[q].Tb > 0;
+      hipEvent_t col_done = any_syrk ? ctx->event(ev++) : nullptr;
       if (with_partner) {
-        ColumnPair cp;
+        ColumnGroup cp{};
         cp.f[0] = ColumnArgs{S, ld, k0, Linv + (long)k0 * 128 * 128, 4 * T, 4 * rn.main, 4 * rn.jump, ncrit, ctx->xs, sync, maxblk, seq, col_seq, column_grid(ncrit, T, ncand), ncand};
-        cp.f[1] = pst.col;
-        hipExtLaunchKernelGGL(chain_column_pair_kernel, dim3(std::max(cp.f[0].grid, cp.f[1].grid), 2), dim3(256), 0, sp, nullptr, col_done, 0, cp, info);
+        int gx = cp.f[0].grid;
+        for (int q = 0; q < nlive; ++q) { cp.f[1 + q] = pst[q].col; gx = std::max(gx, pst[q].col.grid); }
+        hipExtLaunchKernelGGL(chain_column_pair_kernel, dim3(gx, 1 + nlive), dim3(256), 0, sp, nullptr, col_done, 0, cp, info);
       } else {
         hipExtLaunchKernelGGL(chain_column_kernel, dim3(column_grid(ncrit, T, ncand)), dim3(256), 0, sp, nullptr, col_done, 0, S, ld, k0,
                               (const double*)(Linv + (long)k0 * 128 * 128), 4 * T, 4 * rn.main, 4 * rn.jump, ncrit, ctx->xs, sync, maxblk, seq, col_seq, info, 1, after_pair ? 1 : 0, ncand);
@@ -2082,20 +2146,20 @@
 #ifdef SK_TESTING
       if (next_resident && Tb > 0 && !ctx->dq->tuning) { int want = k1; withheld = want >= 0 && g_test_withhold.compare_exchange_strong(want, -1); }
 #endif
-      ThinSyrkPair tp;
+      ThinSyrkGroup tp{};
       tp.f[0] = ThinSyrkArgs{S + (long)(k1 + 1) * 128 * ld + (long)(k1 + 1) * 128, ld, S + (long)(k1 + 1) * 128 * ld + (long)k0 * 128, ld, 128, 4 * Tb, 4 * rs.main, 4 * rs.jump,
                              rs.main, rs.jump, by_col && !withheld ? sync + kSyncSyrkColumn : (int*)nullptr, Tb > 0 ? 2 * Tb * (Tb + 1) : 0};
-      tp.f[1] = pst.syrk;
-      const int gx = std::max(tp.f[0].grid, tp.f[1].grid);
+      int gx = tp.f[0].grid;
+      for (int q = 0; q < nlive; ++q) { tp.f[1 + q] = pst[q].syrk; gx = std::max(gx, pst[q].syrk.grid); }
       hipEvent_t t_start = nullptr, t_stop = nullptr;
       if (kt && gx > 0) kt->pair("gemm_syrk", &t_start, &t_stop);
       hipEvent_t stop_ev = t_stop ? t_stop : ctx->event(ev++);
-      if (gx > 0) hipExtLaunchKernelGGL(syrk_trailing_thin_pair_f64_kernel, dim3(gx, 2), dim3(256), 0, sb, t_start, stop_ev, 0, tp);
+      if (gx > 0) hipExtLaunchKernelGGL(syrk_trailing_thin_pair_f64_kernel, dim3(gx, 1 + nlive), dim3(256), 0, sb, t_start, stop_ev, 0, tp);
       if (Tb > 0) {
         if (by_col) col_seq += 4 * Tb;
         else if (next_resident) { ++seq; if (!withheld) hipLaunchKernelGGL(chain_marker_kernel, dim3(1), dim3(1), 0, sb, sync + kSyncSyrkSeq, seq); }
       }
-      partner_advance(pst, sb);
+      for (int q = 0; q < nlive; ++q) partner_advance(pbs[live[q]], pst[q], sb);
       if (gx > 0 && !next_resident) syrk_done = stop_ev;
       syrk_done2 = syrk_any;
       syrk_any = gx > 0 ? stop_ev : nullptr;
@@ -2147,24 +2211,27 @@
       }
     }
   }
-  while (pb.on && pb.next < pb.ncols) {
-    const PartnerStep st = partner_step(pb.next);
-    hipEvent_t col_done = st.Tb > 0 ? ctx->event(ev++) : nullptr;
-    ColumnPair cp;
-    cp.f[0] = st.col; cp.f[1] = st.col; cp.f[1].grid = 0;
-    hipExtLaunchKernelGGL(chain_column_pair_kernel, dim3(st.col.grid, 1), dim3(256), 0, sp, nullptr, col_done, 0, cp, info);
-    if (st.Tb > 0) {
+  for (;;) {
+    PartnerStep st[kMaxGroupFronts - 1];
+    int live[kMaxGroupFronts - 1], nlive = 0;
+    for (int ip = 0; ip < npb; ++ip) if (pbs[ip].next < pbs[ip].ncols) { live[nlive] = ip; st[nlive] = partner_step(pbs[ip], pbs[ip].next); ++nlive; }
+    if (nlive == 0) break;
+    int gx = 0, gs = 0;
+    ColumnGroup cp{};
+    ThinSyrkGroup tp{};
+    for (int q = 0; q < nlive; ++q) { cp.f[q] = st[q].col; tp.f[q] = st[q].syrk; gx = std::max(gx, st[q].col.grid); gs = std::max(gs, st[q].syrk.grid); }
+    hipEvent_t col_done = gs > 0 ? ctx->event(ev++) : nullptr;
+    hipExtLaunchKernelGGL(chain_column_pair_kernel, dim3(gx, nlive), dim3(256), 0, sp, nullptr, col_done, 0, cp, info);
+    if (gs > 0) {
       (void)hipStreamWaitEvent(ctx->bulk, col_done, 0);
-      ThinSyrkPair tp;
-      tp.f[0] = st.syrk; tp.f[1] = st.syrk; tp.f[1].grid = 0;
       hipEvent_t t_start = nullptr, t_stop = nullptr;
       if (kt) kt->pair("gemm_syrk", &t_start, &t_stop);
-      hipExtLaunchKernelGGL(syrk_trailing_thin_pair_f64_kernel, dim3(st.syrk.grid, 1), dim3(256), 0, ctx->bulk, t_start, t_stop, 0, tp);
-    }
-    partner_advance(st, ctx->bulk);
+      hipExtLaunchKernelGGL(syrk_trailing_thin_pair_f64_kernel, dim3(gs, nlive), dim3(256), 0, ctx->bulk, t_start, t_stop, 0, tp);
+    }
+    for (int q = 0; q < nlive; ++q) partner_advance(pbs[live[q]], st[q], ctx->bulk);
   }
   if (chain && start_value != 0) {
-    int expected = pb.on ? 2 : 1;
+    int expected = 1 + npb;
     for (hipStream_t q : {sp, ctx->bulk, used_bulk_early ? ctx->bulk_early : (hipStream_t) nullptr})
       if (q && q != s) { hipLaunchKernelGGL(chain_end_marker_kernel, dim3(1), dim3(64), 0, q, sync + kSyncEnd); ++expected; }
     hipLaunchKernelGGL(chain_gate_kernel, dim3(1), dim3(64), 0, s, (const int*)(sync + kSyncEnd), expected, info);
@@ -2274,6 +2341,29 @@
   }
 }
 
+__global__ __launch_bounds__(1024) void bs_border_step_kernel(const double* __restrict__ Lrow, long ld, const double* __restrict__ yb, double* __restrict__ w,
+                                                               int col0, int ncols) {
+  __shared__ double ykb[128], red[16 * 64];
+  const int t = threadIdx.x, cl = t & 63, rg = t >> 6;
+  const int col = col0 + blockIdx.x * 64 + cl;
+  if (t < 128) ykb[t] = yb[t];
+  __syncthreads();
+  double s = 0.0;
+  if (col < ncols) {
+    const double* p = Lrow + (long)(rg * 8) * ld + col;
+#pragma unroll
+    for (int i = 0; i < 8; ++i) s += p[(long)i * ld] * ykb[rg * 8 + i];
+  }
+  red[rg * 64 + cl] = s;
+  __syncthreads();
+  if (t < 64 && col < ncols) {
+    double u = 0.0;
+#pragma unroll
+    for (int g = 0; g < 16; ++g) u += red[g * 64 + t];
+    w[col] -= u;
+  }
+}
+
 __global__ void gather_map_kernel(const double* __restrict__ src, const int* __restrict__ map, double* __restrict__ dst, int m) {
   const int i = blockIdx.x * blockDim.x + threadIdx.x;
   if (i < m) dst[i] = map ? (map[i] >= 0 ? src[map[i]] : 0.0) : src[i];
@@ -2304,7 +2394,7 @@
 
 void cholesky_backsolve_front(double* S, long ld, int nblk, int ncols, int rhs_row, const double* Linv, const double* yb, double* w, double* y,
                               hipStream_t s, const int* last, bool spike, int tail_rows, int* info, bool zero_after, const int* tail, const int* yb_map, int resident,
-                              bool prefilled) {
+                              bool prefilled, bool border_by_blocks) {
   const int ni = ncols * 128, m = (nblk - ncols) * 128;
   if (ncols <= 0) return;
   const bool res = info && (resident < 0 ? g_bs_resident.load() != 0 : resident != 0) && nblk <= kBsMaxBlocks;
@@ -2337,8 +2427,12 @@
     }
   const int bfirst = first[ncols < nblk - 1 ? ncols : nblk - 1];
   const int bcol0 = (spike || tail) ? 0 : std::min(bfirst, ncols) * 128;
-  if (ni > bcol0)
+  if (ni > bcol0 && border_by_blocks) {
+    for (int r = nblk - 1; r >= ncols; --r)
+      hipLaunchKernelGGL(bs_border_step_kernel, dim3((ni - bcol0 + 63) / 64), dim3(1024), 0, s, S + (long)r * 128 * ld, ld, yb + (long)(r - ncols) * 128, w, bcol0, ni);
+  } else if (ni > bcol0) {
     hipLaunchKernelGGL(bs_border_kernel, dim3((ni - bcol0 + 63) / 64), dim3(1024), 0, s, S + (long)ncols * 128 * ld, ld, m, yb, w, bcol0, ni);
+  }
   for (int kb = ncols - 1; kb >= 0; --kb) {
     const int nc = kb * 128, col0 = first[kb] * 128;
     const int grid = nc > col0 ? (nc - col0 + 63) / 64 : 1;
@@ -2453,6 +2547,105 @@
   hipLaunchKernelGGL(gather_map_kernel, dim3((m + 255) / 256), dim3(256), 0, s, src, map, dst, m);
 }
 
+static thread_local int g_tree_fronts_taken = 0;
+int cholesky_tree_fronts_taken() { return g_tree_fronts_taken; }
+static void tree_factor_level(const TreeNode* nodes, int n, CholeskyContext* const* lend, int* info, int group, hipStream_t s, CholeskyContext* ctx, KernelTimer* kt,
+                              bool allow_chain) {
+  int lead = -1;
+  for (int k = 0; k < n && lead < 0; ++k) if (nodes[k].v.ncols > 0) lead = k;
+  if (lead < 0) return;
+  CholeskyPartner pt[3];
+  int idx[3], np = 0;
+  for (int k = lead + 1; k < n; ++k) {
+    const FrontView& F = nodes[k].v;
+    if (F.ncols <= 0) continue;
+    pt[np] = CholeskyPartner{F.S, F.ld, F.nblk, F.ncols, F.tail_rows, F.last, F.Linv, ctx && allow_chain ? lend[np] : nullptr, F.tail};
+    idx[np++] = k;
+  }
+  const FrontView& A = nodes[lead].v;
+  cholesky_factor(A.S, A.ld, A.nblk * 128, A.Linv, info, group, s, ctx, kt, A.last, allow_chain, A.ncols, A.tail_rows, np ? pt : nullptr, A.tail, np);
+  for (int q = 0; q < np; ++q)
+    if (pt[q].taken) {
+      ++g_tree_fronts_taken;
+    } else {
+      const FrontView& F = nodes[idx[q]].v;
+      cholesky_factor(F.S, F.ld, F.nblk * 128, F.Linv, info, group, s, ctx, kt, F.last, allow_chain, F.ncols, F.tail_rows, nullptr, F.tail);
+    }
+}
+
+void cholesky_tree_factor(const DissectionTree& t, int* info, int group, hipStream_t s, CholeskyContext* ctx, KernelTimer* kt, bool allow_chain) {
+  g_tree_fronts_taken = 0;
+  tree_factor_level(t.leaf, t.nleaves, t.lend, info, group, s, ctx, kt, allow_chain);
+  for (int k = 0; k < t.nleaves; ++k) {
+    const TreeNode& c = t.leaf[k];
+    if (c.v.ncols <= 0) continue;
+    const FrontView& P = c.parent >= 0 ? t.mid[c.parent].v : t.root;
+    cholesky_border_add(P.S, P.ld, c.v.S, c.v.ld, c.v.ncols, c.v.nblk - c.v.ncols, c.map, s);
+  }
+  tree_factor_level(t.mid, t.nmid, t.lend, info, group, s, ctx, kt, allow_chain);
+  for (int k = 0; k < t.nmid; ++k) {
+    const TreeNode& c = t.mid[k];
+    if (c.v.ncols > 0) cholesky_border_add(t.root.S, t.root.ld, c.v.S, c.v.ld, c.v.ncols, c.v.nblk - c.v.ncols, c.map, s);
+  }
+  cholesky_factor(t.root.S, t.root.ld, t.root.nblk * 128, t.root.Linv, info, group, s, ctx, kt, t.root.last, allow_chain, -1, 1, nullptr, t.root.tail);
+}
+
+static void tree_backsolve_level(const DissectionTree& t, const TreeNode* nodes, int n, hipStream_t s, int* info, bool zero_after, int resident, bool prefilled) {
+  int live[4], nl = 0;
+  bool fits = true;
+  for (int k = 0; k < n; ++k) if (nodes[k].v.ncols > 0) { live[nl++] = k; fits = fits && nodes[k].v.nblk <= kBsGroupMaxBlocks; }
+  if (nl == 0) return;
+  const bool res = info && resident != 0;
+  auto parent_y = [&](const TreeNode& c) { return c.parent >= 0 ? (const double*)t.mid[c.parent].y : (const double*)t.yR; };
+  if (res && nl > 1 && fits && t.level_launches && dev_knobs().bs_pair != 0) {
+    BsGroup p{};
+    p.nf = nl;
+    const bool spread = zero_after && dev_knobs().bs_spread != 0;
+    int grid = 0, jan = 0, most = 0;
+    for (int q = 0; q < nl; ++q) {
+      const TreeNode& c = nodes[live[q]];
+      const FrontView& F = c.v;
+      const int tail_rows = F.tail_rows >= 1 && F.tail_rows <= F.nblk - F.ncols ? F.tail_rows : 1;
+      for (int col = 0; col < F.nblk; ++col) {
+        p.env[q].top[col] = (unsigned short)(F.last ? std::min(std::max(F.last[col], col), F.nblk - 1) : F.nblk - 1);
+        p.env[q].tail[col] = (unsigned short)(F.tail ? std::min(std::max(F.tail[col], 0), F.nblk - 1) : F.nblk - tail_rows);
+      }
+      const int janitors = spread ? F.ncols : (zero_after ? bs_janitors(F.ncols) : 0);
+      p.f[q] = BsArgs{F.Linv, F.S, F.ld, (const double*)(F.S + (long)F.rhs_row * F.ld), F.ncols * 128, c.y, F.nblk, info, F.ncols, parent_y(c), janitors, c.ymap,
+                      spread ? 1 : 0, spread ? 1 : 0};
+      if (!prefilled) (void)hipMemsetAsync(c.y, 0xff, sizeof(double) * (size_t)F.ncols * 128, s);
+      grid += F.ncols; jan += janitors; most = std::max(most, F.ncols);
+    }
+    if (spread) { grid = 8 * most; jan = 0; }
+    hipLaunchKernelGGL(bs_resident_group_kernel, dim3(grid + jan), dim3(1024), 0, s, p);
+    return;
+  }
+  for (int q = 0; q < nl; ++q) {
+    const TreeNode& c = nodes[live[q]];
+    const FrontView& F = c.v;
+    const int m = (F.nblk - F.ncols) * 128;
+    const bool mapped = res && F.nblk <= kBsMaxBlocks;
+    double* yb = c.w + (long)F.ncols * 128;
+    if (!mapped) cholesky_gather_map(parent_y(c), c.ymap, yb, m, s);
+    cholesky_backsolve_front(F.S, F.ld, F.nblk, F.ncols, F.rhs_row, F.Linv, mapped ? parent_y(c) : (const double*)yb, c.w, c.y, s, F.last, F.spike, F.tail_rows, info, zero_after,
+                             F.tail, mapped ? c.ymap : nullptr, resident, prefilled, true);
+  }
+}
+
+void cholesky_tree_backsolve(const DissectionTree& t, hipStream_t s, KernelTimer* kt, int* info, bool zero_after, int resident, bool prefilled) {
+  if (resident < 0) resident = g_bs_resident.load() != 0 ? 1 : 0;
+  cholesky_backsolve(t.root.S, t.root.ld, t.n_root, t.root.nblk * 128, t.root.rhs_row, t.root.Linv, t.wR, t.yR, s, nullptr, t.root.last, info, t.root.tail, zero_after, resident,
+                     prefilled);
+  if (kt) kt->begin("backsolve", s);
+  tree_backsolve_level(t, t.mid, t.nmid, s, info, zero_after, resident, prefilled);
+  for (int k = 0; k < t.nmid; ++k) {
+    const FrontView& F = t.mid[k].v;
+    if (F.nblk > F.ncols) cholesky_gather_map(t.yR, t.mid[k].ymap, t.mid[k].y + (long)F.ncols * 128, (F.nblk - F.ncols) * 128, s);
+  }
+  tree_backsolve_level(t, t.leaf, t.nleaves, s, info, zero_after, resident, prefilled);
+  if (kt) kt->end("backsolve", s);
+}
+
 void launch_syrk_gram(double* H, long ldh, const double* A, long lda, int Kc, int nslabs, double* slabs, int tiles, hipStream_t s,
                       KernelTimer* kt) {
   if (tiles <= 0) return;
diff --git a/skeres_amd/csrc/chol_kernels.hpp b/skeres_amd/csrc/chol_kernels.hpp
--- a/skeres_amd/csrc/chol_kernels.hpp
+++ b/skeres_amd/csrc/chol_kernels.hpp
@@ -162,12 +162,14 @@
 };
 void cholesky_factor(double* S, long ld, int npad, double* Linv, int* info, int group, hipStream_t s, CholeskyContext* ctx,
                      KernelTimer* kt, const int* last = nullptr, bool allow_chain = false, int ncols = -1, int tail_rows = 1,
-                     const CholeskyPartner* partner = nullptr, const int* tail = nullptr);
+                     const CholeskyPartner* partner = nullptr, const int* tail = nullptr, int npartners = 1);
 void cholesky_prepare(CholeskyContext* ctx, hipStream_t s);
 bool cholesky_note_info(CholeskyContext* ctx, int info);
 bool cholesky_chain_enabled(const CholeskyContext* ctx);
 bool cholesky_claim_pair_servers(CholeskyContext* ctx);
 void cholesky_release_pair_servers(CholeskyContext* ctx);
+bool cholesky_claim_group_servers(CholeskyContext* ctx, int fronts);
+void cholesky_release_group_servers(CholeskyContext* ctx, int fronts);
 void cholesky_disable_chain(CholeskyContext* ctx);
 void cholesky_backsolve(double* S, long ld, int n, int npad, int rhs_row, const double* Linv, double* w, double* y,
                         hipStream_t s, KernelTimer* kt, const int* last = nullptr, int* info = nullptr, const int* tail = nullptr, bool zero_after = false, int resident = -1,
@@ -193,11 +195,32 @@
                                KernelTimer* kt, KernelTimer* ktB, bool allow_chain);
 void cholesky_dissected_backsolve(const DissectedSystem& d, int n_root, double* wR, double* yR, double* wA, double* yA, double* wB, double* yB, double* ybB,
                                   hipStream_t s, CholeskyContext* ctxB, KernelTimer* kt, int* info = nullptr, bool zero_after = false, int resident = -1, bool prefilled = false);
+struct TreeNode {
+  FrontView v;
+  int parent = -1;
+  const int* map = nullptr;
+  const int* ymap = nullptr;
+  double* y = nullptr;
+  double* w = nullptr;
+};
+struct DissectionTree {
+  int nleaves = 0, nmid = 0;
+  TreeNode leaf[4], mid[2];
+  FrontView root;
+  int n_root = 0;
+  double *yR = nullptr, *wR = nullptr;
+  CholeskyContext* lend[3] = {nullptr, nullptr, nullptr};
+  bool level_launches = true;
+};
+void cholesky_tree_factor(const DissectionTree& t, int* info, int group, hipStream_t s, CholeskyContext* ctx, KernelTimer* kt, bool allow_chain);
+int cholesky_tree_fronts_taken();
+void cholesky_tree_backsolve(const DissectionTree& t, hipStream_t s, KernelTimer* kt, int* info = nullptr, bool zero_after = false, int resident = -1, bool prefilled = false);
 void cholesky_border_add(double* root, long ld_r, const double* front, long ld_f, int ncols, int border_blocks, const int* map, hipStream_t s);
 void cholesky_backsolve_front(double* S, long ld, int nblk, int ncols, int rhs_row, const double* Linv, const double* yb, double* w, double* y,
                               hipStream_t s, const int* last, bool spike = false, int tail_rows = 1, int* info = nullptr, bool zero_after = false, const int* tail = nullptr,
                               const int* yb_map = nullptr,
-                              int resident = -1, bool prefilled = false);
+                              int resident = -1, bool prefilled = false,
+                              bool border_by_blocks = false);
 void cholesky_gather_map(const double* src, const int* map, double* dst, int m, hipStream_t s);
 void launch_syrk_gram(double* H, long ldh, const double* A, long lda, int Kc, int nslabs, double* slabs, int tiles, hipStream_t s,
                       KernelTimer* kt);
diff --git a/skeres_amd/csrc/chol_solve.hip b/skeres_amd/csrc/chol_solve.hip
--- a/skeres_amd/csrc/chol_solve.hip
+++ b/skeres_amd/csrc/chol_solve.hip
@@ -39,6 +39,8 @@
 hipError_t download(std::vector<double>& h, const double* d, hipStream_t s) { return hipMemcpyAsync(h.data(), d, h.size() * sizeof(double), hipMemcpyDeviceToHost, s); }
 
 const int* envelope_of(const std::vector<int>& last) { return last.empty() ? nullptr : last.data(); }
+
+constexpr int kTreeGroupFronts = 4;
 
 }
 
@@ -165,4 +167,77 @@
   return SK_OK;
 }
 
-}
+int cholesky_tree_fronts_in_lock_step() { return cholesky_tree_fronts_taken(); }
+long cholesky_tree_factor_doubles(int n, int num_segments, const int* cuts, int border_begin) { return tree_factor_doubles(n, num_segments, cuts, border_begin); }
+
+int cholesky_solve_tree(int n, const double* A, const double* b, double* x, int num_segments, const int* cuts, int border_begin, int group, int automatic_plan, int lock_step,
+                        double* factors, long factor_doubles) {
+  const std::string why = tree_check(n, A, num_segments, cuts, border_begin);
+  if (!why.empty()) { set_error("%s", why.c_str()); return SK_ERR_INVALID_ARGUMENT; }
+  if (factors && factor_doubles != tree_factor_doubles(n, num_segments, cuts, border_begin)) { set_error("invalid argument"); return SK_ERR_INVALID_ARGUMENT; }
+  SolveDevice dev;
+  if (const int rc = dev.open(true)) return rc;
+  hipStream_t s = dev.stream.s;
+  group = group_or_automatic(group, automatic_plan);
+  const bool chain = dev.chain(automatic_plan);
+  TreeFronts f = tree_fronts(n, A, b, num_segments, cuts, border_begin);
+  struct Front { TreeFrontHost* h; DevBuf<double> F, Linv, w, y; DevBuf<int> map, ymap, last; };
+  std::vector<std::unique_ptr<Front>> fronts;
+  for (int k = 0; k < f.nleaves + f.nmid + 1; ++k) {
+    std::unique_ptr<Front> fr(new Front());
+    fr->h = k < f.nleaves ? &f.leaf[k] : k < f.nleaves + f.nmid ? &f.mid[k - f.nleaves] : &f.root;
+    const HostFront& h = fr->h->h;
+    SK_HIP_TRY(fr->F.upload(h.F, s));
+    SK_HIP_TRY(fr->Linv.alloc((size_t)std::max(h.ncols, 1) * 128 * 128)); SK_HIP_TRY(fr->Linv.zero(s));
+    SK_HIP_TRY(fr->w.alloc(h.dim)); SK_HIP_TRY(fr->y.alloc(h.dim)); SK_HIP_TRY(fr->y.zero(s));
+    if (!fr->h->map.empty()) { SK_HIP_TRY(fr->map.upload(fr->h->map, s)); SK_HIP_TRY(fr->ymap.upload(fr->h->ymap, s)); }
+    fronts.push_back(std::move(fr));
+  }
+  DevBuf<int> dinfo;
+  SK_HIP_TRY(dinfo.alloc(1)); SK_HIP_TRY(dinfo.zero(s));
+  auto view = [](const Front& fr) {
+    const HostFront& h = fr.h->h;
+    FrontView v;
+    v.S = fr.F.p; v.ld = (long)h.dim; v.nblk = h.nblk; v.ncols = h.ncols; v.last = envelope_of(h.last); v.Linv = fr.Linv.p; v.rhs_row = h.rhs_row;
+    v.tail_rows = fr.h->tail_rows; v.spike = true;
+    return v;
+  };
+  auto node = [&view](const Front& fr) {
+    TreeNode nd;
+    nd.v = view(fr); nd.parent = fr.h->parent; nd.map = fr.map.p; nd.ymap = fr.ymap.p; nd.y = fr.y.p; nd.w = fr.w.p;
+    return nd;
+  };
+  DissectionTree t;
+  t.nleaves = f.nleaves; t.nmid = f.nmid;
+  for (int k = 0; k < f.nleaves; ++k) t.leaf[k] = node(*fronts[k]);
+  for (int k = 0; k < f.nmid; ++k) t.mid[k] = node(*fronts[f.nleaves + k]);
+  const Front& R = *fronts.back();
+  t.root = view(R); t.root.tail_rows = 1; t.root.spike = false;
+  t.n_root = f.root.interior_n; t.yR = R.y.p; t.wR = R.w.p;
+  CholeskyContext lend[3];
+  const bool group_ok = lock_step != 0 && chain && cholesky_claim_group_servers(dev.context(), kTreeGroupFronts);
+  if (group_ok) {
+    int most = 0;
+    for (const auto& fr : fronts) most = std::max(most, fr->h->h.nblk);
+    for (int k = 0; k < 3; ++k) { t.lend[k] = &lend[k]; (void)lend[k].sync_for(most); }
+  }
+  t.level_launches = lock_step != 0;
+  cholesky_tree_factor(t, dinfo.p, group, s, dev.context(), nullptr, chain);
+  cholesky_tree_backsolve(t, s, nullptr, dinfo.p);
+  const int rc = dev.close(dinfo.p);
+  if (group_ok) cholesky_release_group_servers(dev.context(), kTreeGroupFronts);
+  if (rc) return rc;
+  long at = 0;
+  for (auto& fr : fronts) {
+    const TreeFrontHost& h = *fr->h;
+    std::vector<double> y(h.h.dim);
+    SK_HIP_TRY(download(y, fr->y.p, s));
+    if (factors) SK_HIP_TRY(hipMemcpyAsync(factors + at, fr->F.p, h.h.dim * h.h.dim * sizeof(double), hipMemcpyDeviceToHost, s));
+    SK_HIP_TRY(hipStreamSynchronize(s));
+    tree_scatter(h, y.data(), x);
+    at += (long)(h.h.dim * h.h.dim);
+  }
+  return SK_OK;
+}
+
+}
diff --git a/skeres_amd/csrc/chol_solve.hpp b/skeres_amd/csrc/chol_solve.hpp
--- a/skeres_amd/csrc/chol_solve.hpp
+++ b/skeres_amd/csrc/chol_solve.hpp
@@ -5,5 +5,9 @@
 int cholesky_solve_single(int n, const double* A, const double* b, double* x, double* L, int group, const int* last, int automatic_plan, int border_begin_row);
 int cholesky_solve_two_way(int n, const double* A, const double* b, double* x, int head, int tail_begin, int group, int automatic_plan);
 int cholesky_solve_multi_way(int n, const double* A, const double* b, double* x, int num_segments, const int* cuts, int group, int automatic_plan);
+int cholesky_solve_tree(int n, const double* A, const double* b, double* x, int num_segments, const int* cuts, int border_begin, int group, int automatic_plan, int lock_step,
+                        double* factors, long factor_doubles);
+int cholesky_tree_fronts_in_lock_step();
+long cholesky_tree_factor_doubles(int n, int num_segments, const int* cuts, int border_begin);
 
 }
```
